# GreatV/oar-ocr

Measured on AMD Instinct MI355X. Metric: images/sec end-to-end PP-OCRv6 det+rec, higher is better.
Workload: dtype f32; 1 GPU; PP-OCRv6-tiny-class det+rec (synthetic-weight graphs: det 447089 params, rec 1135700 params, V=6906), batch=32 synthetic 960x960 pages per GPU, 40 text lines/page; timed region = u8 pages in pageable HOST memory -> oar_ocr_predict -> oar_ocr_decode -> sorted boxes + texts + scores on the host; image_batch_size=32, region_batch_size=256, parallelism=image-parallel x1

## Files before the change

### include/oar_mi355x.h

```cpp
#ifndef OAR_MI355X_H
#define OAR_MI355X_H

#include <stddef.h>
#include <stdint.h>

#ifdef __cplusplus
extern "C" {
#endif

typedef enum {
    OAR_OK = 0,
    OAR_INVALID_INPUT = 1,
    OAR_MODEL_LOAD = 2,
    OAR_UNSUPPORTED_OP = 3,
    OAR_SHAPE_MISMATCH = 4,
    OAR_DEVICE = 5,
    OAR_OOM = 6,
    OAR_INTERNAL = 7
} oar_status;

size_t oar_last_error(char* buf, size_t cap);
size_t oar_version(char* buf, size_t cap);
int oar_device_count(void);

// ... 170 lines not shown
    float* ctc_probs;
    float* page_angle;
    uint8_t* page_rectified;
    float* line_angle;
    uint32_t n_points;
    uint32_t* point_offsets;
} oar_ocr_result;

oar_status oar_ocr_create(const uint8_t* det_onnx, size_t det_len, const uint8_t* rec_onnx, size_t rec_len,
                          const oar_ocr_cfg* cfg, oar_ocr** out);
void oar_ocr_destroy(oar_ocr* o);
oar_status oar_ocr_predict(oar_ocr* o, const uint8_t* const* rgb, const uint32_t* widths, const uint32_t* heights,
                           uint32_t n_images, oar_ocr_result* out);
oar_status oar_ocr_predict_device(oar_ocr* o, const uint8_t* const* d_rgb, const uint32_t* widths,
                                  const uint32_t* heights, uint32_t n_images, oar_ocr_result* out);
void oar_ocr_result_free(oar_ocr_result* r);
oar_status oar_ocr_predict_async(oar_ocr* o, const uint8_t* const* rgb, const uint32_t* widths, const uint32_t* heights, uint32_t n_images,
                                 int32_t device_pages, uint64_t* ticket);
oar_status oar_ocr_wait(oar_ocr* o, uint64_t ticket, oar_ocr_result* out);
oar_status oar_ocr_decode(const oar_ctc_dict* dict, const oar_ocr_result* res, float score_threshold, oar_text_result* out);

oar_status oar_ctc_word_boxes(const float* line_pts_xy, uint32_t n_points, const char* text_utf8, size_t text_len, const uint32_t* col_indices,
                              uint32_t n_cols, uint32_t seq_len, float wh_ratio, float max_wh_ratio, float* boxes, uint32_t cap_boxes, uint32_t* n_boxes);
oar_status oar_char_positions_to_word_boxes(const float* line_pts_xy, uint32_t n_points, const float* char_positions, uint32_t n_positions,
                                            uint32_t char_count, float* boxes, uint32_t cap_boxes, uint32_t* n_boxes);
typedef struct {
    uint32_t n_regions;
    uint64_t* box_offsets;
    float* boxes;
} oar_word_boxes;
oar_status oar_ocr_word_boxes(const oar_ocr_result* res, const oar_text_result* txt, oar_word_boxes* out);
void oar_word_boxes_free(oar_word_boxes* w);

typedef struct {
    uint32_t n_images, n_regions;
    uint32_t* region_offsets;
    float* points;
    float* scores;
    uint64_t* text_offsets;
    char* utf8;
} oar_packed_pages;
oar_status oar_shard_range(uint64_t n_items, uint32_t world_size, uint32_t rank, uint64_t* begin, uint64_t* end);
oar_status oar_ocr_pack(const oar_ocr_result* res, const oar_text_result* txt, uint8_t** blob, size_t* len);
void oar_blob_free(uint8_t* blob);
oar_status oar_packed_merge(const uint8_t* const* blobs, const size_t* lens, uint32_t n_blobs, oar_packed_pages* out);
void oar_packed_pages_free(oar_packed_pages* p);

typedef struct oar_cls oar_cls;
typedef struct {
    int32_t device_id;
    uint32_t input_h, input_w;
    uint32_t resize_short;
    uint32_t topk;
    uint32_t batch;
} oar_cls_cfg;
typedef struct {
    uint32_t n_images, topk, n_classes;
    int32_t* class_ids;
    float* scores;
} oar_cls_result;
oar_status oar_cls_create(const uint8_t* onnx, size_t onnx_len, const oar_cls_cfg* cfg, oar_cls** out);
void oar_cls_destroy(oar_cls* c);
oar_status oar_cls_run(oar_cls* c, const uint8_t* const* rgb, const uint32_t* widths, const uint32_t* heights, uint32_t n_images,
                       oar_cls_result* out);
void oar_cls_result_free(oar_cls_result* r);
oar_status oar_cls_preprocess(oar_cls* c, const uint8_t* const* rgb, const uint32_t* widths, const uint32_t* heights, uint32_t n_images,
                              float* out_nchw);

typedef struct oar_rect oar_rect;
#define OAR_RECT_NATIVE_SIZE 0xFFFFFFFFu
typedef struct { int32_t device_id; uint32_t target_h, target_w; } oar_rect_cfg;
oar_status oar_rect_create(const uint8_t* onnx, size_t onnx_len, const oar_rect_cfg* cfg, oar_rect** out);
void oar_rect_destroy(oar_rect* r);
oar_status oar_rect_run(oar_rect* r, const uint8_t* rgb, uint32_t width, uint32_t height, uint8_t* out_rgb);

oar_status oar_ocr_attach(oar_ocr* o, oar_cls* doc_orientation, oar_rect* rectifier, oar_cls* line_orientation);

oar_status oar_k_rotate_rgb(const uint8_t* rgb, uint32_t w, uint32_t h, int32_t quarter, uint8_t* out);
oar_status oar_k_bgr_planes_to_rgb(const float* planes, uint64_t plane, float scale, uint8_t* out);
oar_status oar_host_rotate_back_points(float* pts, uint32_t n_points, float angle, uint32_t rotated_w, uint32_t rotated_h);

typedef struct oar_layout oar_layout;
typedef struct {
    int32_t device_id;
    uint32_t input_h, input_w;
    int32_t resize_filter;
    int32_t color_bgr;
    float scale;
    float mean[3], std[3];
    uint32_t num_classes;
    int32_t model_type;
    float score_threshold;
    float nms_threshold;
    uint32_t max_detections;
} oar_layout_cfg;
typedef struct {
    uint32_t n_images, n_boxes;
    uint32_t* box_offsets;
    float* boxes;
    int32_t* classes;
    float* scores;
    uint32_t feature_dim;
} oar_layout_result;
oar_status oar_layout_create(const uint8_t* onnx, size_t onnx_len, const oar_layout_cfg* cfg, oar_layout** out);
void oar_layout_destroy(oar_layout* l);
oar_status oar_layout_run(oar_layout* l, const uint8_t* const* rgb, const uint32_t* widths, const uint32_t* heights, uint32_t n_images, oar_layout_result* out);
void oar_layout_result_free(oar_layout_result* r);
oar_status oar_layout_preprocess(oar_layout* l, const uint8_t* rgb, uint32_t width, uint32_t height, float* out_chw);
oar_status oar_k_resize_filter(const uint8_t* rgb, uint32_t w, uint32_t h, uint32_t nw, uint32_t nh, int32_t filter, uint8_t* out);
oar_status oar_k_layout_postprocess(const float* pred, uint32_t n_images, uint32_t rows, uint32_t feat, const float* src_wh, uint32_t num_classes, int32_t model_type,
                                    float score_threshold, float nms_threshold, uint32_t max_detections, oar_layout_result* out);
typedef struct {
    float score_threshold;
    const float* class_thresholds;
    int32_t layout_nms;
    int32_t image_class_id;
    int32_t formula_class_id;
    const int32_t* class_merge_modes;
} oar_ppdoc_cfg;
oar_status oar_layout_run_ppdoc(oar_layout* l, const uint8_t* const* rgb, const uint32_t* widths, const uint32_t* heights, uint32_t n_images, const oar_ppdoc_cfg* cfg,
                                oar_layout_result* out);
oar_status oar_k_ppdoc_postprocess(const float* pred, uint32_t n_images, uint32_t rows, uint32_t feat, const float* src_wh, uint32_t num_classes, const oar_ppdoc_cfg* cfg,
                                   oar_layout_result* out);
int32_t oar_host_nms_with_merge(const float* boxes, const int32_t* classes, const float* scores, uint32_t n, const int32_t* mode_of_class, uint32_t num_classes,
                                float nms_threshold, uint32_t max_detections, float* out_boxes, int32_t* out_classes, float* out_scores);

oar_status oar_dev_alloc(int32_t device_id, size_t bytes, void** out);
oar_status oar_dev_upload(void* dst, const void* src, size_t bytes);
oar_status oar_dev_download(void* dst, const void* src, size_t bytes);
void oar_dev_free(void* p);
oar_status oar_dev_synchronize(int32_t device_id);

oar_status oar_k_normalize(const uint8_t* rgb, uint32_t w, uint32_t h, const int32_t src_channels[3],
                           const float alpha[3], const float beta[3], int32_t hwc_layout, float* out);
oar_status oar_k_rec_preprocess(const uint8_t* const* rgb, const uint32_t* widths, const uint32_t* heights,
                                uint32_t n, uint32_t img_h, uint32_t img_w, uint32_t max_img_w,
                                float* out_nchw, uint32_t* tensor_width);
oar_status oar_k_rec_preprocess_flip(const uint8_t* const* rgb, const uint32_t* widths, const uint32_t* heights, const uint8_t* flips,
                                     uint32_t n, uint32_t img_h, uint32_t img_w, uint32_t max_img_w,
                                     float* out_nchw, uint32_t* tensor_width);
oar_status oar_k_resize_triangle(const uint8_t* rgb, uint32_t w, uint32_t h, uint32_t nw, uint32_t nh, uint8_t* out);
oar_status oar_k_threshold(const float* pred, size_t n, float thresh, uint8_t* mask);
oar_status oar_k_dilate(const uint8_t* mask, uint32_t height, uint32_t width, uint8_t* out);
oar_status oar_k_poly_scores(const float* pred, uint32_t height, uint32_t width, const float* pts_xy, const uint32_t* counts,
                             uint32_t n_polys, float* scores);
oar_status oar_k_contours(const uint8_t* mask, uint32_t width, uint32_t height, uint32_t max_contours, int32_t* n_contours,
                          int64_t* offsets, int32_t* pts_xy, int32_t* types, int64_t cap_points);
oar_status oar_k_ctc_argmax(const float* probs, size_t rows, size_t vocab, int64_t* idx, float* prob);
oar_status oar_k_unclip(const float* boxes, uint32_t n_boxes, float ratio, int32_t* counts, float* pts_xy, uint32_t cap_points);
oar_status oar_k_box_scores(const float* pred, uint32_t height, uint32_t width, const float* boxes,
                            uint32_t n_boxes, float* scores);
oar_status oar_k_rotate_crop(const uint8_t* rgb, uint32_t w, uint32_t h, const float box[8], uint8_t* out,
                             size_t cap, uint32_t* out_w, uint32_t* out_h);

oar_status oar_image_decode(const uint8_t* bytes, size_t len, uint8_t** rgb, uint32_t* width, uint32_t* height);
void oar_image_free(uint8_t* rgb);
oar_status oar_image_decode_device(const uint8_t* bytes, size_t len, int32_t device_id, void** dev_rgb, uint32_t* width, uint32_t* height);

int32_t oar_host_candidates(const uint8_t* mask, uint32_t width, uint32_t height, uint32_t max_candidates, int32_t max_bands,
                            float* boxes8, int32_t cap);
int32_t oar_host_contours(const uint8_t* mask, uint32_t width, uint32_t height, uint32_t max_contours, int32_t max_bands,
                          int64_t* offsets, int32_t* pts_xy, int32_t* types, int64_t cap_points);
int32_t oar_host_contours_bits(const uint8_t* mask, uint32_t width, uint32_t height, uint32_t max_contours, int32_t max_bands,
                               int64_t* offsets, int32_t* pts_xy, int32_t* types, int64_t cap_points);
int32_t oar_host_unclip(const float box8[8], float ratio, float* out_xy, int32_t cap_points);
int32_t oar_host_approx_poly_dp(const float* xy, int32_t n_points, float epsilon, float* out_xy, int32_t cap_points);
float oar_host_perimeter(const float* xy, int32_t n_points);
int32_t oar_host_unclip_poly(const float* xy, int32_t n_points, float ratio, float* out_xy, int32_t cap_points);
int32_t oar_host_offset_ring(const int64_t* xy, int32_t n_points, double radius, int64_t* out_xy, int32_t cap_points);
int32_t oar_host_ring_outline(const int64_t* xy, int32_t n_points, int32_t negative, int64_t* out_xy, int32_t cap_points);
void oar_host_sort_poly_boxes(const float* pts_xy, const uint32_t* offsets, int32_t n, int32_t* order);
int32_t oar_host_mini_box(const float* xy, int32_t n_points, float box8[8], float* min_side);
int32_t oar_host_convex_hull(const float* xy, int32_t n_points, float* out_xy, int32_t cap_points);
void oar_host_sort_quad_boxes(const float* boxes8, int32_t n, int32_t* order);
int32_t oar_host_pool_selftest(int32_t threads, int32_t jobs);
void oar_host_plan_crop(uint32_t img_w, uint32_t img_h, const float box8[8], int32_t plan[8], float inv[9]);

oar_status oar_debug_inject_failure(const char* site, int32_t count);

typedef struct {
    char name[48];
    uint64_t launches;
    double total_ms;
    double alg_bytes;
    double alg_flops;
} oar_prof_entry;
void oar_prof_reset(void);
void oar_prof_enable(int32_t on);
void oar_prof_filter(const char* class_name);
void oar_prof_sampling(int32_t stride, int32_t phase);
int32_t oar_prof_snapshot(oar_prof_entry* entries, int32_t cap);

#ifdef __cplusplus
}
#endif
#endif
```

### oar_ocr_amd/api.py

```python
from __future__ import annotations

import ctypes as C
import os
from dataclasses import dataclass, field
from pathlib import Path
from typing import List, Optional, Sequence

import numpy as np

_HERE = Path(__file__).resolve().parent
LIB_PATH = _HERE / "lib" / "libOarMi355x.so"
_lib = None

OAR_OK, OAR_INVALID_INPUT, OAR_MODEL_LOAD, OAR_UNSUPPORTED_OP, OAR_SHAPE_MISMATCH, OAR_DEVICE, OAR_OOM, OAR_INTERNAL = range(8)


class OCRError(RuntimeError):

    def __init__(self, code: int, message: str):
        super().__init__(f"[oar_status {code}] {message}")
        self.code = code
        self.message = message


class EngineCfg(C.Structure):
    _fields_ = [("device_id", C.c_int32), ("use_hip_graph", C.c_int32), ("profile", C.c_int32), ("precision", C.c_int32), ("stream", C.c_void_p)]


PRECISION_F32 = 0


class Tensor(C.Structure):
    _fields_ = [("rank", C.c_int32), ("dims", C.c_int64 * 8), ("data", C.POINTER(C.c_float)), ("name", C.c_char * 64),
                ("dtype", C.c_int32), ("reserved", C.c_int32), ("data_i64", C.POINTER(C.c_int64))]


class Input(C.Structure):
    _fields_ = [("name", C.c_char_p), ("data", C.POINTER(C.c_float)), ("dims", C.POINTER(C.c_int64)), ("rank", C.c_int32),
                ("reserved", C.c_int32)]


class IoInfo(C.Structure):
    _fields_ = [("name", C.c_char * 64), ("dtype", C.c_int32), ("rank", C.c_int32), ("dims", C.c_int64 * 8)]


OUTPUT_VIEW_FN = C.CFUNCTYPE(C.c_int32, C.c_void_p, C.POINTER(C.c_int64), C.c_int32, C.POINTER(C.c_float))


class DetCfg(C.Structure):
    _fields_ = [("device_id", C.c_int32), ("limit_side_len", C.c_uint32), ("limit_type", C.c_int32), ("max_side_limit", C.c_uint32),
                ("max_candidates", C.c_uint32), ("use_hip_graph", C.c_int32), ("profile", C.c_int32), ("host_threads", C.c_int32),
                ("box_type", C.c_int32), ("score_mode", C.c_int32), ("use_dilation", C.c_int32), ("gpu_contours", C.c_int32)]


class DetResult(C.Structure):
    _fields_ = [("n_images", C.c_uint32), ("n_boxes", C.c_uint32), ("box_offsets", C.POINTER(C.c_uint32)),
                ("points", C.POINTER(C.c_float)), ("scores", C.POINTER(C.c_float)), ("n_points", C.c_uint32), ("point_offsets", C.POINTER(C.c_uint32))]


class RecCfg(C.Structure):
    _fields_ = [("device_id", C.c_int32), ("rec_image_shape", C.c_uint32 * 3), ("max_img_w", C.c_uint32), ("use_hip_graph", C.c_int32),
                ("profile", C.c_int32), ("reserved", C.c_int32)]


class RecResult(C.Structure):
    _fields_ = [("batch", C.c_uint32), ("seq_len", C.c_uint32), ("vocab", C.c_uint32), ("tensor_width", C.c_uint32),
                ("indices", C.POINTER(C.c_int64)), ("probs", C.POINTER(C.c_float))]


class OcrCfg(C.Structure):
    _fields_ = [("det", DetCfg), ("rec", RecCfg), ("det_thresh", C.c_float), ("det_box_thresh", C.c_float), ("det_unclip_ratio", C.c_float),
                ("image_batch_size", C.c_uint32), ("region_batch_size", C.c_uint32), ("max_pooled_crops", C.c_uint32), ("box_sort", C.c_int32), ("lanes", C.c_uint32)]


class OcrResult(C.Structure):
    _fields_ = [("n_images", C.c_uint32), ("n_regions", C.c_uint32), ("region_offsets", C.POINTER(C.c_uint32)),
                ("points", C.POINTER(C.c_float)), ("det_scores", C.POINTER(C.c_float)), ("crop_wh", C.POINTER(C.c_uint32)),
                ("seq_len", C.POINTER(C.c_uint32)), ("max_wh_ratio", C.POINTER(C.c_float)), ("ctc_offsets", C.POINTER(C.c_uint64)),
                ("ctc_indices", C.POINTER(C.c_int64)), ("ctc_probs", C.POINTER(C.c_float)),
                ("page_angle", C.POINTER(C.c_float)), ("page_rectified", C.POINTER(C.c_uint8)), ("line_angle", C.POINTER(C.c_float)),
                ("n_points", C.c_uint32), ("point_offsets", C.POINTER(C.c_uint32))]


class ClsCfg(C.Structure):
    _fields_ = [("device_id", C.c_int32), ("input_h", C.c_uint32), ("input_w", C.c_uint32), ("resize_short", C.c_uint32),
                ("topk", C.c_uint32), ("batch", C.c_uint32)]


class ClsResult(C.Structure):
    _fields_ = [("n_images", C.c_uint32), ("topk", C.c_uint32), ("n_classes", C.c_uint32), ("class_ids", C.POINTER(C.c_int32)),
                ("scores", C.POINTER(C.c_float))]


class RectCfg(C.Structure):
    _fields_ = [("device_id", C.c_int32), ("target_h", C.c_uint32), ("target_w", C.c_uint32)]


class TextResult(C.Structure):
    _fields_ = [("n", C.c_uint32), ("text_offsets", C.POINTER(C.c_uint64)), ("utf8", C.POINTER(C.c_char)), ("scores", C.POINTER(C.c_float)),
                ("char_offsets", C.POINTER(C.c_uint64)), ("char_cols", C.POINTER(C.c_uint32)), ("char_positions", C.POINTER(C.c_float)),
                ("seq_len", C.POINTER(C.c_uint32)), ("kept", C.POINTER(C.c_uint8))]


class WordBoxes(C.Structure):
    _fields_ = [("n_regions", C.c_uint32), ("box_offsets", C.POINTER(C.c_uint64)), ("boxes", C.POINTER(C.c_float))]


class LayoutCfg(C.Structure):
    _fields_ = [("device_id", C.c_int32), ("input_h", C.c_uint32), ("input_w", C.c_uint32), ("resize_filter", C.c_int32), ("color_bgr", C.c_int32), ("scale", C.c_float),
                ("mean", C.c_float * 3), ("std", C.c_float * 3), ("num_classes", C.c_uint32), ("model_type", C.c_int32), ("score_threshold", C.c_float),
                ("nms_threshold", C.c_float), ("max_detections", C.c_uint32)]


class LayoutResult(C.Structure):
    _fields_ = [("n_images", C.c_uint32), ("n_boxes", C.c_uint32), ("box_offsets", C.POINTER(C.c_uint32)), ("boxes", C.POINTER(C.c_float)),
                ("classes", C.POINTER(C.c_int32)), ("scores", C.POINTER(C.c_float)), ("feature_dim", C.c_uint32)]


class ProfEntry(C.Structure):
    _fields_ = [("name", C.c_char * 48), ("launches", C.c_uint64), ("total_ms", C.c_double), ("alg_bytes", C.c_double), ("alg_flops", C.c_double)]


class DecodeStats(C.Structure):
    _fields_ = [("steps_limit", C.c_int64), ("steps_enqueued", C.c_int64), ("steps_executed", C.c_int64), ("lookahead", C.c_int64)]

    def __repr__(self):
        return f"DecodeStats(steps_limit={self.steps_limit}, steps_enqueued={self.steps_enqueued}, steps_executed={self.steps_executed}, lookahead={self.lookahead})"


EXPORTS = [
    "oar_last_error", "oar_version", "oar_device_count", "oar_engine_create", "oar_engine_destroy", "oar_engine_input_name",
    "oar_engine_run", "oar_engine_run_named", "oar_engine_run_first_f32", "oar_engine_io", "oar_tensor_free", "oar_engine_cost", "oar_det_create", "oar_det_destroy", "oar_det_run", "oar_det_result_free",
    "oar_db_postprocess", "oar_rec_create", "oar_rec_destroy", "oar_rec_run", "oar_rec_result_free", "oar_ocr_create", "oar_ocr_destroy",
    "oar_ocr_predict", "oar_ocr_predict_device", "oar_ocr_result_free", "oar_dev_alloc", "oar_dev_upload", "oar_dev_download",
    "oar_dev_free", "oar_dev_synchronize", "oar_k_normalize", "oar_k_rec_preprocess", "oar_k_resize_triangle", "oar_k_threshold",
    "oar_k_ctc_argmax", "oar_k_box_scores", "oar_k_rotate_crop", "oar_prof_reset", "oar_prof_enable", "oar_prof_filter", "oar_prof_sampling", "oar_prof_snapshot",
    "oar_host_candidates", "oar_host_unclip", "oar_host_mini_box", "oar_host_convex_hull", "oar_host_sort_quad_boxes", "oar_host_pool_selftest", "oar_host_plan_crop",
    "oar_cls_create", "oar_cls_destroy", "oar_cls_run", "oar_cls_result_free", "oar_cls_preprocess", "oar_rect_create", "oar_rect_destroy",
    "oar_rect_run", "oar_ocr_attach", "oar_k_rotate_rgb", "oar_k_bgr_planes_to_rgb", "oar_host_rotate_back_points",
    "oar_engine_cache_stats", "oar_onnx_inspect", "oar_host_contours", "oar_ctc_dict_create", "oar_ctc_dict_destroy", "oar_ctc_dict_classes",
    "oar_ctc_decode", "oar_ocr_decode", "oar_text_result_free", "oar_db_postprocess_ex", "oar_k_dilate", "oar_k_poly_scores", "oar_debug_inject_failure", "oar_k_contours", "oar_host_contours_bits",
    "oar_k_unclip", "oar_k_rec_preprocess_flip", "oar_layout_create", "oar_layout_destroy", "oar_layout_run", "oar_layout_result_free", "oar_layout_preprocess", "oar_k_resize_filter", "oar_k_layout_postprocess", "oar_layout_run_ppdoc", "oar_k_ppdoc_postprocess", "oar_host_nms_with_merge", "oar_image_decode_device", "oar_ocr_predict_async", "oar_ocr_wait", "oar_ctc_word_boxes", "oar_char_positions_to_word_boxes", "oar_ocr_word_boxes", "oar_word_boxes_free", "oar_image_decode", "oar_image_free", "oar_host_approx_poly_dp", "oar_host_perimeter", "oar_host_unclip_poly", "oar_host_offset_ring", "oar_host_ring_outline", "oar_host_sort_poly_boxes",
    "oar_engine_set_decode_stop", "oar_engine_decode_stats",
]


def lib():
    global _lib
    if _lib is not None:
        return _lib
    if not LIB_PATH.exists():
        raise OCRError(OAR_DEVICE, f"{LIB_PATH} is missing: run `python -c 'import __graft_entry__ as g; g.build()'` "
                                   "(the MI355X path has no CPU fallback)")
    L = C.CDLL(str(LIB_PATH))
    vp, u8pp, u32p, f32p = C.c_void_p, C.POINTER(C.c_void_p), C.POINTER(C.c_uint32), C.POINTER(C.c_float)
    L.oar_last_error.restype = C.c_size_t
    L.oar_last_error.argtypes = [C.c_char_p, C.c_size_t]
    L.oar_version.restype = C.c_size_t
    L.oar_version.argtypes = [C.c_char_p, C.c_size_t]
    L.oar_device_count.restype = C.c_int
    L.oar_engine_create.argtypes = [vp, C.c_size_t, C.POINTER(EngineCfg), C.POINTER(vp)]
    L.oar_engine_destroy.argtypes = [vp]
    L.oar_engine_destroy.restype = None
    L.oar_engine_input_name.argtypes = [vp, C.c_char_p, C.c_size_t]
    L.oar_engine_run.argtypes = [vp, vp, C.POINTER(C.c_int64), C.c_int32, C.POINTER(Tensor), C.c_int32, C.POINTER(C.c_int32)]
    L.oar_engine_run_named.argtypes = [vp, C.POINTER(Input), C.c_int32, C.POINTER(Tensor), C.c_int32, C.POINTER(C.c_int32)]
    L.oar_engine_run_first_f32.argtypes = [vp, C.POINTER(Input), C.c_int32, OUTPUT_VIEW_FN, vp]
    L.oar_engine_io.argtypes = [vp, C.POINTER(IoInfo), C.c_int32, C.POINTER(C.c_int32), C.POINTER(IoInfo), C.c_int32, C.POINTER(C.c_int32)]
    L.oar_tensor_free.argtypes = [C.POINTER(Tensor)]
    L.oar_tensor_free.restype = None
    L.oar_engine_cost.argtypes = [vp, C.POINTER(C.c_int64), C.c_int32, C.POINTER(C.c_double), C.POINTER(C.c_double), C.POINTER(C.c_int32)]
    L.oar_engine_cache_stats.argtypes = [vp, C.POINTER(C.c_uint64), C.POINTER(C.c_uint64)]
    L.oar_engine_set_decode_stop.argtypes = [vp, C.c_int64]
    L.oar_engine_decode_stats.argtypes = [vp, C.POINTER(DecodeStats)]
    L.oar_onnx_inspect.argtypes = [vp, C.c_size_t, C.c_char_p, C.c_size_t]
    L.oar_det_create.argtypes = [vp, C.c_size_t, C.POINTER(DetCfg), C.POINTER(vp)]
    L.oar_det_destroy.argtypes = [vp]
    L.oar_det_destroy.restype = None
    L.oar_det_run.argtypes = [vp, u8pp, u32p, u32p, C.c_uint32, C.c_float, C.c_float, C.c_float, C.POINTER(DetResult)]
    L.oar_det_result_free.argtypes = [C.POINTER(DetResult)]
    L.oar_det_result_free.restype = None
    L.oar_db_postprocess.argtypes = [vp, C.c_uint32, C.c_uint32, C.c_uint32, C.c_uint32, C.c_float, C.c_float, C.c_float, C.c_uint32, C.POINTER(DetResult)]
    L.oar_db_postprocess_ex.argtypes = [vp, C.c_uint32, C.c_uint32, C.c_uint32, C.c_uint32, C.c_float, C.c_float, C.c_float, C.c_uint32, C.c_int32, C.c_int32,
                                        C.c_int32, C.POINTER(DetResult)]
    L.oar_debug_inject_failure.argtypes = [C.c_char_p, C.c_int32]
    L.oar_k_dilate.argtypes = [vp, C.c_uint32, C.c_uint32, vp]
    L.oar_k_poly_scores.argtypes = [vp, C.c_uint32, C.c_uint32, vp, u32p, C.c_uint32, vp]
    L.oar_rec_create.argtypes = [vp, C.c_size_t, C.POINTER(RecCfg), C.POINTER(vp)]
    L.oar_rec_destroy.argtypes = [vp]
    L.oar_rec_destroy.restype = None
    L.oar_rec_run.argtypes = [vp, u8pp, u32p, u32p, C.c_uint32, C.POINTER(RecResult)]
    L.oar_rec_result_free.argtypes = [C.POINTER(RecResult)]
    L.oar_rec_result_free.restype = None
    L.oar_ocr_create.argtypes = [vp, C.c_size_t, vp, C.c_size_t, C.POINTER(OcrCfg), C.POINTER(vp)]
    L.oar_ocr_destroy.argtypes = [vp]
    L.oar_ocr_destroy.restype = None
    L.oar_ocr_predict.argtypes = [vp, u8pp, u32p, u32p, C.c_uint32, C.POINTER(OcrResult)]
    L.oar_ocr_predict_device.argtypes = [vp, u8pp, u32p, u32p, C.c_uint32, C.POINTER(OcrResult)]
    L.oar_ocr_result_free.argtypes = [C.POINTER(OcrResult)]
    L.oar_ocr_result_free.restype = None
    L.oar_dev_alloc.argtypes = [C.c_int32, C.c_size_t, C.POINTER(vp)]
    L.oar_dev_upload.argtypes = [vp, vp, C.c_size_t]
    L.oar_dev_download.argtypes = [vp, vp, C.c_size_t]
    L.oar_dev_free.argtypes = [vp]
    L.oar_dev_free.restype = None
    L.oar_dev_synchronize.argtypes = [C.c_int32]
    L.oar_k_normalize.argtypes = [vp, C.c_uint32, C.c_uint32, C.POINTER(C.c_int32), f32p, f32p, C.c_int32, vp]
    L.oar_k_rec_preprocess.argtypes = [u8pp, u32p, u32p, C.c_uint32, C.c_uint32, C.c_uint32, C.c_uint32, vp, u32p]
    L.oar_ctc_word_boxes.argtypes = [vp, C.c_uint32, C.c_char_p, C.c_size_t, vp, C.c_uint32, C.c_uint32, C.c_float, C.c_float, vp, C.c_uint32, u32p]
    L.oar_char_positions_to_word_boxes.argtypes = [vp, C.c_uint32, vp, C.c_uint32, C.c_uint32, vp, C.c_uint32, u32p]
    L.oar_ocr_word_boxes.argtypes = [vp, vp, vp]
    L.oar_word_boxes_free.argtypes = [vp]
    L.oar_word_boxes_free.restype = None
    L.oar_k_rec_preprocess_flip.argtypes = [u8pp, u32p, u32p, vp, C.c_uint32, C.c_uint32, C.c_uint32, C.c_uint32, vp, u32p]
    L.oar_k_resize_triangle.argtypes = [vp, C.c_uint32, C.c_uint32, C.c_uint32, C.c_uint32, vp]
    L.oar_k_threshold.argtypes = [vp, C.c_size_t, C.c_float, vp]
    L.oar_k_ctc_argmax.argtypes = [vp, C.c_size_t, C.c_size_t, vp, vp]
    L.oar_k_box_scores.argtypes = [vp, C.c_uint32, C.c_uint32, vp, C.c_uint32, vp]
    L.oar_k_unclip.argtypes = [vp, C.c_uint32, C.c_float, vp, vp, C.c_uint32]
    L.oar_image_decode.argtypes = [vp, C.c_size_t, C.POINTER(C.POINTER(C.c_uint8)), C.POINTER(C.c_uint32), C.POINTER(C.c_uint32)]
    L.oar_image_free.argtypes = [C.POINTER(C.c_uint8)]
    L.oar_layout_create.argtypes = [vp, C.c_size_t, vp, C.POINTER(C.c_void_p)]
    L.oar_layout_destroy.argtypes = [vp]
    L.oar_layout_destroy.restype = None
    L.oar_layout_run.argtypes = [vp, u8pp, u32p, u32p, C.c_uint32, vp]
    L.oar_layout_result_free.argtypes = [vp]
    L.oar_layout_result_free.restype = None
    L.oar_layout_preprocess.argtypes = [vp, vp, C.c_uint32, C.c_uint32, vp]
    L.oar_k_resize_filter.argtypes = [vp, C.c_uint32, C.c_uint32, C.c_uint32, C.c_uint32, C.c_int32, vp]
    L.oar_k_layout_postprocess.argtypes = [vp, C.c_uint32, C.c_uint32, C.c_uint32, vp, C.c_uint32, C.c_int32, C.c_float, C.c_float, C.c_uint32, vp]
    L.oar_ocr_predict_async.argtypes = [vp, u8pp, u32p, u32p, C.c_uint32, C.c_int32, C.POINTER(C.c_uint64)]
    L.oar_ocr_wait.argtypes = [vp, C.c_uint64, vp]
    L.oar_image_decode_device.argtypes = [vp, C.c_size_t, C.c_int32, C.POINTER(C.c_void_p), C.POINTER(C.c_uint32), C.POINTER(C.c_uint32)]
    L.oar_image_free.restype = None
    L.oar_k_rotate_crop.argtypes = [vp, C.c_uint32, C.c_uint32, f32p, vp, C.c_size_t, u32p, u32p]
    L.oar_host_candidates.argtypes = [vp, C.c_uint32, C.c_uint32, C.c_uint32, C.c_int32, vp, C.c_int32]
    L.oar_host_candidates.restype = C.c_int32
    L.oar_host_contours.argtypes = [vp, C.c_uint32, C.c_uint32, C.c_uint32, C.c_int32, vp, vp, vp, C.c_int64]
    L.oar_host_contours.restype = C.c_int32
    L.oar_host_unclip.argtypes = [vp, C.c_float, vp, C.c_int32]
    L.oar_host_unclip.restype = C.c_int32
    L.oar_host_approx_poly_dp.argtypes = [vp, C.c_int32, C.c_float, vp, C.c_int32]
    L.oar_host_approx_poly_dp.restype = C.c_int32
    L.oar_host_perimeter.argtypes = [vp, C.c_int32]
    L.oar_host_perimeter.restype = C.c_float
    L.oar_host_unclip_poly.argtypes = [vp, C.c_int32, C.c_float, vp, C.c_int32]
    L.oar_host_unclip_poly.restype = C.c_int32
    L.oar_host_offset_ring.argtypes = [vp, C.c_int32, C.c_double, vp, C.c_int32]
    L.oar_host_offset_ring.restype = C.c_int32
    L.oar_host_ring_outline.argtypes = [vp, C.c_int32, C.c_int32, vp, C.c_int32]
    L.oar_host_ring_outline.restype = C.c_int32
    L.oar_host_sort_poly_boxes.argtypes = [vp, vp, C.c_int32, vp]
    L.oar_host_sort_poly_boxes.restype = None
    L.oar_host_mini_box.argtypes = [vp, C.c_int32, vp, f32p]
    L.oar_host_mini_box.restype = C.c_int32
    L.oar_host_convex_hull.argtypes = [vp, C.c_int32, vp, C.c_int32]
    L.oar_host_convex_hull.restype = C.c_int32
    L.oar_host_sort_quad_boxes.argtypes = [vp, C.c_int32, vp]
    L.oar_host_sort_quad_boxes.restype = None
    L.oar_host_plan_crop.argtypes = [C.c_uint32, C.c_uint32, vp, vp, vp]
    L.oar_host_plan_crop.restype = None
    L.oar_cls_create.argtypes = [vp, C.c_size_t, C.POINTER(ClsCfg), C.POINTER(vp)]
    L.oar_cls_destroy.argtypes = [vp]
    L.oar_cls_destroy.restype = None
    L.oar_cls_run.argtypes = [vp, u8pp, u32p, u32p, C.c_uint32, C.POINTER(ClsResult)]
    L.oar_cls_result_free.argtypes = [C.POINTER(ClsResult)]
    L.oar_cls_result_free.restype = None
    L.oar_cls_preprocess.argtypes = [vp, u8pp, u32p, u32p, C.c_uint32, vp]
    L.oar_rect_create.argtypes = [vp, C.c_size_t, C.POINTER(RectCfg), C.POINTER(vp)]
    L.oar_rect_destroy.argtypes = [vp]
    L.oar_rect_destroy.restype = None
    L.oar_rect_run.argtypes = [vp, vp, C.c_uint32, C.c_uint32, vp]
    L.oar_ocr_attach.argtypes = [vp, vp, vp, vp]
    L.oar_k_rotate_rgb.argtypes = [vp, C.c_uint32, C.c_uint32, C.c_int32, vp]
    L.oar_k_bgr_planes_to_rgb.argtypes = [vp, C.c_uint64, C.c_float, vp]
    L.oar_host_rotate_back_points.argtypes = [vp, C.c_uint32, C.c_float, C.c_uint32, C.c_uint32]
    L.oar_ctc_dict_create.argtypes = [C.c_char_p, C.c_size_t, C.c_int32, C.POINTER(vp)]
    L.oar_ctc_dict_destroy.argtypes = [vp]
    L.oar_ctc_dict_destroy.restype = None
    L.oar_ctc_dict_classes.argtypes = [vp]
    L.oar_ctc_dict_classes.restype = C.c_uint32
    L.oar_ctc_decode.argtypes = [vp, vp, vp, C.c_uint32, C.c_uint32, C.c_float, C.POINTER(TextResult)]
    L.oar_ocr_decode.argtypes = [vp, C.POINTER(OcrResult), C.c_float, C.POINTER(TextResult)]
    L.oar_text_result_free.argtypes = [C.POINTER(TextResult)]
    L.oar_text_result_free.restype = None
    L.oar_prof_reset.restype = None
    L.oar_prof_enable.argtypes = [C.c_int32]
    L.oar_prof_enable.restype = None
    L.oar_prof_filter.argtypes = [C.c_char_p]
    L.oar_prof_filter.restype = None
    L.oar_prof_sampling.argtypes = [C.c_int32, C.c_int32]
    L.oar_prof_sampling.restype = None
    L.oar_prof_snapshot.argtypes = [C.POINTER(ProfEntry), C.c_int32]
    L.oar_prof_snapshot.restype = C.c_int32
    _lib = L
    return L


def _check(st: int):
    if st != OAR_OK:
        buf = C.create_string_buffer(4096)
        lib().oar_last_error(buf, 4096)
        raise OCRError(st, buf.value.decode(errors="replace"))


DEFAULT_PARALLEL_THRESHOLD = 4


def load_image_from_memory(data: bytes) -> np.ndarray:
    buf = (C.c_char * len(data)).from_buffer_copy(data) if len(data) else (C.c_char * 1)()
    out = C.POINTER(C.c_uint8)()
    w, h = C.c_uint32(0), C.c_uint32(0)
    _check(lib().oar_image_decode(C.cast(buf, C.c_void_p), len(data), C.byref(out), C.byref(w), C.byref(h)))
    try:
        return np.ctypeslib.as_array(out, shape=(h.value, w.value, 3)).copy()
    finally:
        lib().oar_image_free(out)


def load_image_to_device(data: bytes, device_id: int = 0):
    buf = (C.c_char * len(data)).from_buffer_copy(data) if len(data) else (C.c_char * 1)()
    ptr = C.c_void_p()
    w, h = C.c_uint32(0), C.c_uint32(0)
    _check(lib().oar_image_decode_device(C.cast(buf, C.c_void_p), len(data), device_id, C.byref(ptr), C.byref(w), C.byref(h)))
    holder = DeviceBuffer.__new__(DeviceBuffer)
    holder.ptr, holder.nbytes = ptr, w.value * h.value * 3
    return holder, w.value, h.value


def load_image(path) -> np.ndarray:
    with open(path, "rb") as f:
        return load_image_from_memory(f.read())


def load_images(paths, parallel_threshold: Optional[int] = None) -> List[np.ndarray]:
    paths = list(paths)
    thr = DEFAULT_PARALLEL_THRESHOLD if parallel_threshold is None else parallel_threshold
    if len(paths) > thr:
        from concurrent.futures import ThreadPoolExecutor
        with ThreadPoolExecutor(max_workers=min(len(paths), os.cpu_count() or 4)) as ex:
            return list(ex.map(load_image, paths))
    return [load_image(p) for p in paths]


def version() -> str:
    buf = C.create_string_buffer(256)
    lib().oar_version(buf, 256)
    return buf.value.decode()


def onnx_inspect(model: bytes) -> str:
    buf = C.create_string_buffer(8192)
    b = (C.c_char * max(len(model), 1)).from_buffer_copy(model or b"\0")
    st = lib().oar_onnx_inspect(C.cast(b, C.c_void_p), len(model), buf, 8192)
    _check(st)
    return buf.value.decode()


def debug_inject_failure(site: str, count: int):
    _check(lib().oar_debug_inject_failure(site.encode(), count))


def device_count() -> int:
    return int(lib().oar_device_count())


def _p(a: np.ndarray):
    return a.ctypes.data_as(C.c_void_p)


def _img_arrays(images: Sequence[np.ndarray]):
    imgs = [np.ascontiguousarray(im, dtype=np.uint8) for im in images]
    for im in imgs:
        if im.ndim != 3 or im.shape[2] != 3:
            raise OCRError(OAR_INVALID_INPUT, "images must be HxWx3 uint8 (RgbImage)")
    ptrs = (C.c_void_p * max(len(imgs), 1))(*[im.ctypes.data for im in imgs])
    ws = (C.c_uint32 * max(len(imgs), 1))(*[im.shape[1] for im in imgs])
    hs = (C.c_uint32 * max(len(imgs), 1))(*[im.shape[0] for im in imgs])
    return imgs, ptrs, ws, hs


class OrtInfer:

    def __init__(self, model: bytes, device_id: int = 0, profile: bool = False, precision: int = PRECISION_F32, stream: Optional[int] = None):
        self._h = C.c_void_p()
        cfg = EngineCfg(device_id, 0, int(profile), int(precision), C.c_void_p(stream) if stream else None)
        buf = (C.c_char * len(model)).from_buffer_copy(model)
        _check(lib().oar_engine_create(C.cast(buf, C.c_void_p), len(model), C.byref(cfg), C.byref(self._h)))
# ... 1027 lines not shown
        raise OCRError(OAR_INVALID_INPUT, "oar_host_nms_with_merge failed")
    return ob[:k].copy(), oc[:k].copy(), os_[:k].copy()


def k_resize_filter(rgb, nw, nh, filter="lanczos3"):
    rgb = np.ascontiguousarray(rgb, np.uint8)
    h, w, _ = rgb.shape
    out = np.empty((nh, nw, 3), np.uint8)
    _check(lib().oar_k_resize_filter(_p(rgb), w, h, nw, nh, LAYOUT_FILTERS[filter], _p(out)))
    return out


def k_layout_postprocess(pred, src_wh, num_classes, score_threshold=0.5, nms_threshold=0.5, max_detections=100, model_type="picodet"):
    pred = np.ascontiguousarray(pred, np.float32)
    n, rows, feat = pred.shape
    wh = np.ascontiguousarray(src_wh, np.float32).reshape(n, 2)
    res = LayoutResult()
    _check(lib().oar_k_layout_postprocess(_p(pred) if pred.size else None, n, rows, feat, _p(wh), num_classes, LAYOUT_MODEL_TYPES.get(model_type, 0), C.c_float(score_threshold),
                                          C.c_float(nms_threshold), max_detections, C.byref(res)))
    try:
        return _unpack_layout(res)
    finally:
        lib().oar_layout_result_free(C.byref(res))


class DeviceBuffer:
    def __init__(self, data: np.ndarray, device_id: int = 0):
        data = np.ascontiguousarray(data)
        self.nbytes = data.nbytes
        self.ptr = C.c_void_p()
        _check(lib().oar_dev_alloc(device_id, self.nbytes, C.byref(self.ptr)))
        _check(lib().oar_dev_upload(self.ptr, _p(data), self.nbytes))

    def free(self):
        if self.ptr:
            lib().oar_dev_free(self.ptr)
            self.ptr = C.c_void_p()

    def __del__(self):
        try:
            self.free()
        except Exception:
            pass


def prof_enable(on: bool = True):
    lib().oar_prof_enable(int(on))


def prof_filter(name: str = ""):
    lib().oar_prof_filter(name.encode() if name else None)


def prof_sampling(stride: int = 1, phase: int = 0):
    lib().oar_prof_sampling(stride, phase)


def prof_reset():
    lib().oar_prof_reset()


def prof_snapshot(max_entries: int = 512):
    arr = (ProfEntry * max_entries)()
    n = lib().oar_prof_snapshot(arr, max_entries)
    return [{"name": arr[i].name.decode(), "launches": int(arr[i].launches), "total_ms": arr[i].total_ms,
             "alg_bytes": arr[i].alg_bytes, "alg_flops": arr[i].alg_flops} for i in range(min(n, max_entries))]


def k_normalize(rgb, alpha, beta, src=(0, 1, 2), layout="chw"):
    rgb = np.ascontiguousarray(rgb, np.uint8)
    h, w, _ = rgb.shape
    out = np.empty((3, h, w) if layout == "chw" else (h, w, 3), np.float32)
    a, b = np.ascontiguousarray(alpha, np.float32), np.ascontiguousarray(beta, np.float32)
    s = (C.c_int32 * 3)(*src)
    _check(lib().oar_k_normalize(_p(rgb), w, h, s, a.ctypes.data_as(C.POINTER(C.c_float)), b.ctypes.data_as(C.POINTER(C.c_float)),
                                 0 if layout == "chw" else 1, _p(out)))
    return out


def k_rec_preprocess(crops, img_h=48, img_w=320, max_img_w=3200, flips=None):
    imgs, ptrs, ws, hs = _img_arrays(crops)
    tw = C.c_uint32(0)
    fl = None if flips is None else np.ascontiguousarray(np.asarray(flips, bool).astype(np.uint8))
    _check(lib().oar_k_rec_preprocess_flip(ptrs, ws, hs, None if fl is None else _p(fl), len(imgs), img_h, img_w, max_img_w, None, C.byref(tw)))
    out = np.empty((len(imgs), 3, img_h, tw.value), np.float32)
    _check(lib().oar_k_rec_preprocess_flip(ptrs, ws, hs, None if fl is None else _p(fl), len(imgs), img_h, img_w, max_img_w, _p(out), C.byref(tw)))
    return out


def k_resize_triangle(rgb, nw, nh):
    rgb = np.ascontiguousarray(rgb, np.uint8)
    h, w, _ = rgb.shape
    out = np.empty((nh, nw, 3), np.uint8)
    _check(lib().oar_k_resize_triangle(_p(rgb), w, h, nw, nh, _p(out)))
    return out


def k_threshold(pred, thresh):
    pred = np.ascontiguousarray(pred, np.float32)
    out = np.empty(pred.shape, np.uint8)
    _check(lib().oar_k_threshold(_p(pred), pred.size, thresh, _p(out)))
    return out


def k_dilate(mask):
    mask = np.ascontiguousarray(mask, np.uint8)
    out = np.empty_like(mask)
    _check(lib().oar_k_dilate(_p(mask), mask.shape[0], mask.shape[1], _p(out)))
    return out


def k_poly_scores(pred, polys):
    pred = np.ascontiguousarray(pred, np.float32)
    h, w = pred.shape
    pts = np.ascontiguousarray(np.concatenate([np.asarray(p, np.float32).reshape(-1, 2) for p in polys]) if polys else np.zeros((0, 2), np.float32))
    counts = (C.c_uint32 * max(len(polys), 1))(*[len(p) for p in polys])
    out = np.zeros(len(polys), np.float32)
    _check(lib().oar_k_poly_scores(_p(pred), h, w, _p(pts), counts, len(polys), _p(out)))
    return out


def k_ctc_argmax(probs):
    probs = np.ascontiguousarray(probs, np.float32)
    v = probs.shape[-1]
    rows = probs.size // v if v else 0
    idx = np.zeros(rows, np.int64)
    p = np.zeros(rows, np.float32)
    _check(lib().oar_k_ctc_argmax(_p(probs), rows, v, _p(idx), _p(p)))
    return idx, p


def k_box_scores(pred, boxes):
    pred = np.ascontiguousarray(pred, np.float32)
    boxes = np.ascontiguousarray(boxes, np.float32).reshape(-1, 8)
    h, w = pred.shape
    out = np.zeros(boxes.shape[0], np.float32)
    _check(lib().oar_k_box_scores(_p(pred), h, w, _p(boxes), boxes.shape[0], _p(out)))
    return out


def k_rotate_crop(img, box):
    img = np.ascontiguousarray(img, np.uint8)
    h, w, _ = img.shape
    box = np.ascontiguousarray(box, np.float32).reshape(8)
    cap = 3 * (w + h + 8) ** 2
    out = np.empty(cap, np.uint8)
    ow, oh = C.c_uint32(0), C.c_uint32(0)
    _check(lib().oar_k_rotate_crop(_p(img), w, h, box.ctypes.data_as(C.POINTER(C.c_float)), _p(out), cap, C.byref(ow), C.byref(oh)))
    if ow.value == 0:
        return None
    return out[:ow.value * oh.value * 3].reshape(oh.value, ow.value, 3).copy()


def host_candidates(mask, max_candidates=1000, max_bands=1):
    mask = np.ascontiguousarray(mask, np.uint8)
    h, w = mask.shape
    out = np.zeros((max_candidates, 4, 2), np.float32)
    n = lib().oar_host_candidates(_p(mask), w, h, max_candidates, max_bands, _p(out), max_candidates)
    if n < 0:
        raise OCRError(OAR_INTERNAL, "oar_host_candidates failed")
    return out[:n].copy()


def host_contours(mask, max_contours=100000, max_bands=1, bits=False):
    mask = np.ascontiguousarray(mask, np.uint8)
    h, w = mask.shape
    cap = 4 * h * w + 16
    offs = np.zeros(max_contours + 1, np.int64)
    pts = np.zeros((cap, 2), np.int32)
    types = np.zeros(max_contours, np.int32)
    fn = lib().oar_host_contours_bits if bits else lib().oar_host_contours
    n = fn(_p(mask), w, h, max_contours, max_bands, _p(offs), _p(pts), _p(types), cap)
    if n < 0:
        raise OCRError(OAR_INTERNAL, "oar_host_contours failed")
    return [(pts[offs[i]:offs[i + 1]].copy(), int(types[i])) for i in range(n)]


def k_contours(mask, max_contours=100000):
    mask = np.ascontiguousarray(mask, np.uint8)
    h, w = mask.shape
    cap = 4 * h * w + 16
    offs = np.zeros(max_contours + 1, np.int64)
    pts = np.zeros((cap, 2), np.int32)
    types = np.zeros(max_contours, np.int32)
    n = C.c_int32(0)
    _check(lib().oar_k_contours(_p(mask), w, h, max_contours, C.byref(n), _p(offs), _p(pts), _p(types), cap))
    return [(pts[offs[i]:offs[i + 1]].copy(), int(types[i])) for i in range(n.value)]


def k_unclip(boxes, ratio, cap_points=96):
    b = np.ascontiguousarray(boxes, np.float32).reshape(-1, 8)
    n = len(b)
    counts = np.zeros(max(n, 1), np.int32)
    pts = np.zeros((max(n, 1), cap_points, 2), np.float32)
    _check(lib().oar_k_unclip(_p(b), n, C.c_float(ratio), _p(counts), _p(pts), cap_points))
    return [None if counts[i] < 0 else pts[i, :counts[i]].copy() for i in range(n)]


def host_unclip(box, ratio):
    box = np.ascontiguousarray(box, np.float32).reshape(8)
    out = np.zeros((1024, 2), np.float32)
    n = lib().oar_host_unclip(_p(box), ratio, _p(out), 1024)
    return out[:max(n, 0)].copy()


def host_approx_poly_dp(points, epsilon):
    pts = np.ascontiguousarray(points, np.float32).reshape(-1, 2)
    out = np.zeros((max(len(pts), 1), 2), np.float32)
    n = lib().oar_host_approx_poly_dp(_p(pts), pts.shape[0], C.c_float(epsilon), _p(out), out.shape[0])
    return out[:max(n, 0)].copy()


def host_perimeter(points) -> float:
    pts = np.ascontiguousarray(points, np.float32).reshape(-1, 2)
    return float(lib().oar_host_perimeter(_p(pts), pts.shape[0]))


def host_unclip_poly(points, ratio):
    pts = np.ascontiguousarray(points, np.float32).reshape(-1, 2)
    cap = 64 * len(pts) + 1024
    out = np.zeros((cap, 2), np.float32)
    n = lib().oar_host_unclip_poly(_p(pts), pts.shape[0], C.c_float(ratio), _p(out), cap)
    if n < 0:
        raise RuntimeError("oar_host_unclip_poly failed")
    return out[:n].copy()


def host_offset_ring(ring, radius):
    r = np.ascontiguousarray(ring, np.int64).reshape(-1, 2)
    cap = 64 * len(r) + 1024
    out = np.zeros((cap, 2), np.int64)
    n = lib().oar_host_offset_ring(_p(r), r.shape[0], C.c_double(radius), _p(out), cap)
    return out[:max(n, 0)].copy()


def host_ring_outline(raw, negative=False):
    r = np.ascontiguousarray(raw, np.int64).reshape(-1, 2)
    cap = 4 * len(r) + 64
    out = np.zeros((cap, 2), np.int64)
    n = lib().oar_host_ring_outline(_p(r), r.shape[0], 1 if negative else 0, _p(out), cap)
    return out[:n].copy() if n > 0 else None


def host_sort_poly_boxes(polys):
    if not polys:
        return np.zeros(0, np.int32)
    offs = np.zeros(len(polys) + 1, np.uint32)
    offs[1:] = np.cumsum([len(p) for p in polys])
    pts = np.ascontiguousarray(np.concatenate([np.asarray(p, np.float32).reshape(-1, 2) for p in polys] + [np.zeros((0, 2), np.float32)]), np.float32)
    if len(pts) == 0:
        pts = np.zeros((1, 2), np.float32)
    order = np.zeros(len(polys), np.int32)
    lib().oar_host_sort_poly_boxes(_p(pts), _p(offs), len(polys), _p(order))
    return order


def host_mini_box(points):
    pts = np.ascontiguousarray(points, np.float32).reshape(-1, 2)
    out = np.zeros((4, 2), np.float32)
    ms = C.c_float(0)
    ok = lib().oar_host_mini_box(_p(pts), pts.shape[0], _p(out), C.byref(ms))
    return (out, float(ms.value)) if ok == 1 else None


def host_convex_hull(points):
    pts = np.ascontiguousarray(points, np.float32).reshape(-1, 2)
    out = np.zeros((max(pts.shape[0], 1), 2), np.float32)
    n = lib().oar_host_convex_hull(_p(pts), pts.shape[0], _p(out), out.shape[0])
    if n < 0:
        raise OCRError(1, "oar_host_convex_hull failed")
    return out[:n].copy()


def host_sort_quad_boxes(boxes):
    b = np.ascontiguousarray(boxes, np.float32).reshape(-1, 8)
    order = np.zeros(b.shape[0], np.int32)
    if b.shape[0]:
        lib().oar_host_sort_quad_boxes(_p(b), b.shape[0], _p(order))
    return order


def host_plan_crop(img_w, img_h, box):
    b = np.ascontiguousarray(box, np.float32).reshape(8)
    plan = np.zeros(8, np.int32)
    inv = np.zeros(9, np.float32)
    lib().oar_host_plan_crop(img_w, img_h, _p(b), _p(plan), _p(inv))
    return plan, inv


@dataclass
class Classification:
    class_id: int
    score: float


class ImageClassifier:

    def __init__(self, model: bytes, input_hw=(224, 224), resize_short: int = 256, topk: int = 1, device_id: int = 0, batch: int = 0):
        self._h = C.c_void_p()
        self.input_hw = tuple(input_hw)
        cfg = ClsCfg(device_id, input_hw[0], input_hw[1], resize_short or 0, topk, batch)
        buf = (C.c_char * len(model)).from_buffer_copy(model)
        _check(lib().oar_cls_create(C.cast(buf, C.c_void_p), len(model), C.byref(cfg), C.byref(self._h)))

    def predict(self, images: Sequence[np.ndarray]) -> List[List[Classification]]:
        if len(images) == 0:
# ... 376 lines not shown
```

### oar_ocr_amd/csrc/c_api.cc

```cpp
#include <condition_variable>
#include <cstdlib>
#include <cmath>
#include <cstring>
#include <deque>
#include <map>
#include <mutex>
#include <thread>

#include "engine.h"
#include "layout.h"
#include "pipeline.h"

namespace oar {
const std::string& last_error();
extern std::atomic<int> g_inject_batched_det_failures;
}
using namespace oar;

struct oar_engine { std::unique_ptr<Engine> e; PinBuf view; };
struct oar_det { std::unique_ptr<Detector> d; };
struct oar_rec { std::unique_ptr<Recognizer> r; };
struct OcrLane {
    std::unique_ptr<Ocr> o;
    std::thread worker;
// ... 990 lines not shown
oar_status oar_k_rec_preprocess(const uint8_t* const* rgb, const uint32_t* widths, const uint32_t* heights, uint32_t n, uint32_t img_h,
                                uint32_t img_w, uint32_t max_img_w, float* out_nchw, uint32_t* tensor_width) {
    return oar_k_rec_preprocess_flip(rgb, widths, heights, nullptr, n, img_h, img_w, max_img_w, out_nchw, tensor_width);
}

oar_status oar_k_rec_preprocess_flip(const uint8_t* const* rgb, const uint32_t* widths, const uint32_t* heights, const uint8_t* flips, uint32_t n,
                                     uint32_t img_h, uint32_t img_w, uint32_t max_img_w, float* out_nchw, uint32_t* tensor_width) {
    return guard([&] {
        OAR_CHECK(tensor_width && (n == 0 || (rgb && widths && heights)), OAR_INVALID_INPUT, "oar_k_rec_preprocess: bad arguments");
        require_device();
        std::vector<uint32_t> ws(widths, widths + n), hs(heights, heights + n);
        std::vector<int32_t> rws;
        int Wt = host::rec_tensor_width(ws, hs, (int)img_h, (int)img_w, (int)max_img_w, rws);
        *tensor_width = (uint32_t)Wt;
        if (!out_nchw || n == 0) return;
        size_t stage = 0;
        for (uint32_t i = 0; i < n; ++i) stage += ((size_t)ws[i] * hs[i] * 3 + 63) & ~(size_t)63;
        DevBuf dc, dd, dout;
        dc.reserve(stage); dd.reserve(n * sizeof(pp::CropDesc)); dout.reserve((size_t)n * 3 * img_h * Wt * 4);
        std::vector<pp::CropDesc> descs(n);
        size_t off = 0;
        for (uint32_t i = 0; i < n; ++i) {
            size_t bytes = (size_t)ws[i] * hs[i] * 3;
            OAR_HIP(hipMemcpy(dc.as<uint8_t>() + off, rgb[i], bytes, hipMemcpyHostToDevice));
            descs[i].src = dc.as<uint8_t>() + off; descs[i].w = (int)ws[i]; descs[i].h = (int)hs[i]; descs[i].rw = rws[i]; descs[i].flip = flips && flips[i] ? 1 : 0;
            off += (bytes + 63) & ~(size_t)63;
        }
        OAR_HIP(hipMemcpy(dd.p, descs.data(), n * sizeof(pp::CropDesc), hipMemcpyHostToDevice));
        pp::rec_pack(nullptr, dd.as<pp::CropDesc>(), (int)n, (int)img_h, Wt, dout.as<float>(), 1);
        OAR_HIP(hipMemcpy(out_nchw, dout.p, (size_t)n * 3 * img_h * Wt * 4, hipMemcpyDeviceToHost));
    });
}

oar_status oar_k_resize_triangle(const uint8_t* rgb, uint32_t w, uint32_t h, uint32_t nw, uint32_t nh, uint8_t* out) {
    return guard([&] {
        OAR_CHECK(rgb && out && w && h && nw && nh, OAR_INVALID_INPUT, "oar_k_resize_triangle: bad arguments");
        require_device();
        DevBuf din, dout;
        din.reserve((size_t)w * h * 3); dout.reserve((size_t)nw * nh * 3);
        OAR_HIP(hipMemcpy(din.p, rgb, (size_t)w * h * 3, hipMemcpyHostToDevice));
        pp::resize_triangle(nullptr, din.as<uint8_t>(), (int)w, (int)h, dout.as<uint8_t>(), (int)nw, (int)nh);
        OAR_HIP(hipMemcpy(out, dout.p, (size_t)nw * nh * 3, hipMemcpyDeviceToHost));
    });
}

oar_status oar_k_threshold(const float* pred, size_t n, float thresh, uint8_t* mask) {
    return guard([&] {
        OAR_CHECK((pred && mask) || n == 0, OAR_INVALID_INPUT, "oar_k_threshold: bad arguments");
        require_device();
        if (n == 0) return;
        DevBuf din, dout;
        din.reserve(n * 4); dout.reserve(n + 4);
        OAR_HIP(hipMemcpy(din.p, pred, n * 4, hipMemcpyHostToDevice));
        pp::threshold(nullptr, din.as<float>(), dout.as<uint8_t>(), (int64_t)n, thresh);
        OAR_HIP(hipMemcpy(mask, dout.p, n, hipMemcpyDeviceToHost));
    });
}

oar_status oar_k_dilate(const uint8_t* mask, uint32_t height, uint32_t width, uint8_t* out) {
    return guard([&] {
        OAR_CHECK(mask && out && height && width, OAR_INVALID_INPUT, "oar_k_dilate: bad arguments");
        require_device();
        const size_t n = (size_t)height * width;
        DevBuf din, dout;
        din.reserve(n); dout.reserve(n);
        OAR_HIP(hipMemcpy(din.p, mask, n, hipMemcpyHostToDevice));
        pp::dilate3x3(nullptr, din.as<uint8_t>(), dout.as<uint8_t>(), 1, (int)height, (int)width);
        OAR_HIP(hipMemcpy(out, dout.p, n, hipMemcpyDeviceToHost));
    });
}

oar_status oar_k_poly_scores(const float* pred, uint32_t height, uint32_t width, const float* pts_xy, const uint32_t* counts, uint32_t n_polys,
                             float* scores) {
    return guard([&] {
        OAR_CHECK(pred && height && width && (n_polys == 0 || (pts_xy && counts && scores)), OAR_INVALID_INPUT, "oar_k_poly_scores: bad arguments");
        require_device();
        if (n_polys == 0) return;
        std::vector<pp::PolyDesc> pd(n_polys);
        size_t at = 0;
        for (uint32_t i = 0; i < n_polys; ++i) { pd[i] = pp::PolyDesc{(int32_t)at, (int32_t)counts[i], 0, 0}; at += counts[i]; }
        const size_t hw = (size_t)height * width;
        DevBuf dpred, dpts, dpd, dsc;
        dpred.reserve(hw * 4); dpts.reserve(at * 8 + 8); dpd.reserve(pd.size() * sizeof(pp::PolyDesc)); dsc.reserve((size_t)n_polys * 4);
        OAR_HIP(hipMemcpy(dpred.p, pred, hw * 4, hipMemcpyHostToDevice));
        if (at) OAR_HIP(hipMemcpy(dpts.p, pts_xy, at * 8, hipMemcpyHostToDevice));
        OAR_HIP(hipMemcpy(dpd.p, pd.data(), pd.size() * sizeof(pp::PolyDesc), hipMemcpyHostToDevice));
        pp::poly_scores(nullptr, dpred.as<float>(), (int)height, (int)width, dpts.as<float>(), dpd.as<pp::PolyDesc>(), (int)n_polys, dsc.as<float>());
        OAR_HIP(hipMemcpy(scores, dsc.p, (size_t)n_polys * 4, hipMemcpyDeviceToHost));
    });
}

oar_status oar_k_ctc_argmax(const float* probs, size_t rows, size_t vocab, int64_t* idx, float* prob) {
    return guard([&] {
        require_device();
        if (rows == 0 || vocab == 0) return;
        OAR_CHECK(probs && idx && prob, OAR_INVALID_INPUT, "oar_k_ctc_argmax: bad arguments");
        DevBuf din, di, dp;
        din.reserve(rows * vocab * 4); di.reserve(rows * 8); dp.reserve(rows * 4);
        OAR_HIP(hipMemcpy(din.p, probs, rows * vocab * 4, hipMemcpyHostToDevice));
        pp::ctc_argmax(nullptr, din.as<float>(), (int64_t)rows, (int)vocab, di.as<int64_t>(), dp.as<float>());
        OAR_HIP(hipMemcpy(idx, di.p, rows * 8, hipMemcpyDeviceToHost));
        OAR_HIP(hipMemcpy(prob, dp.p, rows * 4, hipMemcpyDeviceToHost));
    });
}

oar_status oar_k_unclip(const float* boxes, uint32_t n_boxes, float ratio, int32_t* counts, float* pts_xy, uint32_t cap_points) {
    return guard([&] {
        require_device();
        OAR_CHECK(n_boxes == 0 || (boxes && counts && pts_xy), OAR_INVALID_INPUT, "oar_k_unclip: bad arguments");
        if (n_boxes == 0) return;
        std::vector<pp::ScoreBox> sb(n_boxes);
        for (uint32_t i = 0; i < n_boxes; ++i) { std::memcpy(sb[i].pts, boxes + (size_t)i * 8, 32); sb[i].image = 0; sb[i].pad = 0; }
        DevBuf db, dout;
        db.reserve(n_boxes * sizeof(pp::ScoreBox)); dout.reserve(n_boxes * sizeof(pp::UnclipOut));
        OAR_HIP(hipMemcpy(db.p, sb.data(), n_boxes * sizeof(pp::ScoreBox), hipMemcpyHostToDevice));
        pp::unclip_quads(nullptr, db.as<pp::ScoreBox>(), (int)n_boxes, ratio, dout.as<pp::UnclipOut>());
        std::vector<pp::UnclipOut> ho(n_boxes);
        OAR_HIP(hipMemcpy(ho.data(), dout.p, n_boxes * sizeof(pp::UnclipOut), hipMemcpyDeviceToHost));
        for (uint32_t i = 0; i < n_boxes; ++i) {
            counts[i] = ho[i].n_pts;
            const int m = std::min<int>(std::max(ho[i].n_pts, 0), (int)cap_points);
            std::memcpy(pts_xy + (size_t)i * cap_points * 2, ho[i].pts, (size_t)m * 2 * sizeof(float));
        }
    });
}
oar_status oar_k_box_scores(const float* pred, uint32_t height, uint32_t width, const float* boxes, uint32_t n_boxes, float* scores) {
    return guard([&] {
        require_device();
        if (n_boxes == 0) return;
        OAR_CHECK(pred && boxes && scores && height && width, OAR_INVALID_INPUT, "oar_k_box_scores: bad arguments");
        size_t hw = (size_t)height * width;
        DevBuf dpred, db, ds;
        dpred.reserve(hw * 4); db.reserve(n_boxes * sizeof(pp::ScoreBox)); ds.reserve(n_boxes * 4);
        std::vector<pp::ScoreBox> sb(n_boxes);
        for (uint32_t i = 0; i < n_boxes; ++i) { std::memcpy(sb[i].pts, boxes + (size_t)i * 8, 32); sb[i].image = 0; sb[i].pad = 0; }
        OAR_HIP(hipMemcpy(dpred.p, pred, hw * 4, hipMemcpyHostToDevice));
        OAR_HIP(hipMemcpy(db.p, sb.data(), n_boxes * sizeof(pp::ScoreBox), hipMemcpyHostToDevice));
        pp::box_scores(nullptr, dpred.as<float>(), (int)height, (int)width, db.as<pp::ScoreBox>(), (int)n_boxes, ds.as<float>());
        OAR_HIP(hipMemcpy(scores, ds.p, n_boxes * 4, hipMemcpyDeviceToHost));
    });
}

oar_status oar_k_rotate_crop(const uint8_t* rgb, uint32_t w, uint32_t h, const float box[8], uint8_t* out, size_t cap, uint32_t* out_w,
                             uint32_t* out_h) {
    return guard([&] {
        OAR_CHECK(rgb && box && out_w && out_h && w && h, OAR_INVALID_INPUT, "oar_k_rotate_crop: bad arguments");
        require_device();
        host::CropPlan pl = host::plan_crop((int)w, (int)h, box);
        *out_w = *out_h = 0;
        if (pl.mode == 0) return;
        *out_w = (uint32_t)pl.out_w(); *out_h = (uint32_t)pl.out_h();
        size_t bytes = (size_t)pl.out_w() * pl.out_h() * 3;
        OAR_CHECK(out && cap >= bytes, OAR_INVALID_INPUT, "oar_k_rotate_crop: output buffer too small");
        DevBuf dpage, dd, dout;
        dpage.reserve((size_t)w * h * 3); dd.reserve(sizeof(pp::WarpDesc)); dout.reserve(bytes);
        OAR_HIP(hipMemcpy(dpage.p, rgb, (size_t)w * h * 3, hipMemcpyHostToDevice));
        pp::WarpDesc d;
        std::memset(&d, 0, sizeof d);
        d.page = dpage.as<uint8_t>(); d.page_w = (int)w; d.page_h = (int)h;
        d.left = pl.left; d.top = pl.top; d.cw = pl.cw; d.ch = pl.ch; d.ow = pl.ow; d.oh = pl.oh; d.rot = pl.rot; d.mode = pl.mode;
        std::memcpy(d.inv, pl.inv, sizeof d.inv);
        d.out_off = 0;
        OAR_HIP(hipMemcpy(dd.p, &d, sizeof d, hipMemcpyHostToDevice));
        pp::rotate_crops(nullptr, dd.as<pp::WarpDesc>(), 1, dout.as<uint8_t>(), pl.out_w() * pl.out_h());
        OAR_HIP(hipMemcpy(out, dout.p, bytes, hipMemcpyDeviceToHost));
    });
}

int32_t oar_host_candidates(const uint8_t* mask, uint32_t width, uint32_t height, uint32_t max_candidates, int32_t max_bands,
                            float* boxes8, int32_t cap) {
    try {
        const int row_bytes = ((int)width + 7) / 8;
        std::vector<uint8_t> bits((size_t)row_bytes * height, 0);
        for (uint32_t y = 0; y < height; ++y)
            for (uint32_t x = 0; x < width; ++x)
                if (mask[(size_t)y * width + x]) bits[(size_t)y * row_bytes + (x >> 3)] |= (uint8_t)(1u << (x & 7));
        std::vector<int> cuts = host::blank_row_bands_bits(bits.data(), row_bytes, (int)height, max_bands < 1 ? 1 : max_bands);
        std::vector<host::Contour> cs;
        for (size_t i = 0; i + 1 < cuts.size(); ++i) {
            auto part = host::find_contours_band_bits(bits.data(), row_bytes, (int)width, cuts[i], cuts[i + 1], max_candidates, true);
            for (auto& c : part) { if (cs.size() >= max_candidates) break; cs.push_back(std::move(c)); }
        }
        int32_t n = 0;
        for (auto& c : cs) {
            host::Pt mb[4];
            float ms = 0.f;
            if (!host::contour_mini_box(c, mb, ms) || ms < 3.0f) continue;
            if (n < cap) for (int k = 0; k < 4; ++k) { boxes8[n * 8 + k * 2] = mb[k].x; boxes8[n * 8 + k * 2 + 1] = mb[k].y; }
            ++n;
        }
        return n;
    } catch (...) { return -1; }
}
int32_t oar_host_contours_bits(const uint8_t* mask, uint32_t width, uint32_t height, uint32_t max_contours, int32_t max_bands, int64_t* offsets,
                               int32_t* pts_xy, int32_t* types, int64_t cap_points) {
    try {
        const int row_bytes = ((int)width + 7) / 8;
        std::vector<uint8_t> bits((size_t)row_bytes * height, 0);
        for (uint32_t y = 0; y < height; ++y)
            for (uint32_t x = 0; x < width; ++x)
                if (mask[(size_t)y * width + x]) bits[(size_t)y * row_bytes + (x >> 3)] |= (uint8_t)(1u << (x & 7));
        std::vector<int> cuts = host::blank_row_bands_bits(bits.data(), row_bytes, (int)height, max_bands < 1 ? 1 : max_bands);
        int32_t n = 0;
        int64_t np = 0;
        if (offsets) offsets[0] = 0;
        for (size_t i = 0; i + 1 < cuts.size(); ++i) {
            auto part = host::find_contours_band_bits(bits.data(), row_bytes, (int)width, cuts[i], cuts[i + 1], max_contours);
            for (auto& c : part) {
                if ((uint32_t)n >= max_contours) break;
                for (auto& q : c.pts) {
                    if (pts_xy && np < cap_points) { pts_xy[np * 2] = (int32_t)q.x; pts_xy[np * 2 + 1] = (int32_t)q.y; }
                    ++np;
                }
                if (types) types[n] = c.hole ? 1 : 0;
                ++n;
                if (offsets) offsets[n] = np;
            }
        }
        return n;
    } catch (...) { return -1; }
}
int32_t oar_host_contours(const uint8_t* mask, uint32_t width, uint32_t height, uint32_t max_contours, int32_t max_bands, int64_t* offsets,
                          int32_t* pts_xy, int32_t* types, int64_t cap_points) {
    try {
        std::vector<int32_t> scratch((size_t)width * height);
        std::vector<int> cuts = host::blank_row_bands(mask, (int)width, (int)height, max_bands < 1 ? 1 : max_bands);
        int32_t n = 0;
        int64_t np = 0;
        if (offsets) offsets[0] = 0;
        for (size_t i = 0; i + 1 < cuts.size(); ++i) {
            auto part = host::find_contours_band(mask, (int)width, (int)height, cuts[i], cuts[i + 1], max_contours, scratch.data());
            for (auto& c : part) {
                if ((uint32_t)n >= max_contours) break;
                for (auto& q : c.pts) {
                    if (pts_xy && np < cap_points) { pts_xy[np * 2] = (int32_t)q.x; pts_xy[np * 2 + 1] = (int32_t)q.y; }
                    ++np;
                }
                if (types) types[n] = c.hole ? 1 : 0;
                ++n;
                if (offsets) offsets[n] = np;
            }
        }
        return n;
    } catch (...) { return -1; }
}

oar_status oar_k_contours(const uint8_t* mask, uint32_t width, uint32_t height, uint32_t max_contours, int32_t* n_contours, int64_t* offsets,
                          int32_t* pts_xy, int32_t* types, int64_t cap_points) {
    return guard([&] {
        OAR_CHECK(mask && width > 0 && height > 0 && n_contours, OAR_INVALID_INPUT, "oar_k_contours: bad arguments");
        int ndev = 0;
        if (hipGetDeviceCount(&ndev) != hipSuccess || ndev <= 0) fail(OAR_DEVICE, "no HIP device visible: libOarMi355x has no CPU fallback");
        DevBuf dm;
        const size_t hw = (size_t)width * height;
        dm.reserve(hw);
        OAR_HIP(hipMemcpy(dm.p, mask, hw, hipMemcpyHostToDevice));
        std::vector<host::Contour> cs = Detector::trace_device_mask(dm.as<uint8_t>(), (int)height, (int)width, max_contours);
        int64_t np = 0;
        if (offsets) offsets[0] = 0;
        int32_t n = 0;
        for (auto& c : cs) {
            for (auto& q : c.pts) {
                if (pts_xy && np < cap_points) { pts_xy[np * 2] = (int32_t)q.x; pts_xy[np * 2 + 1] = (int32_t)q.y; }
                ++np;
            }
            if (types) types[n] = c.hole ? 1 : 0;
            ++n;
            if (offsets) offsets[n] = np;
        }
        *n_contours = n;
    });
}
int32_t oar_host_unclip(const float box8[8], float ratio, float* out_xy, int32_t cap_points) {
    try {
        host::Pt b[4];
        for (int k = 0; k < 4; ++k) b[k] = {box8[k * 2], box8[k * 2 + 1]};
        std::vector<host::Pt> r = host::unclip(b, ratio);
        for (size_t i = 0; i < r.size() && (int32_t)i < cap_points; ++i) { out_xy[i * 2] = r[i].x; out_xy[i * 2 + 1] = r[i].y; }
        return (int32_t)r.size();
    } catch (...) { return -1; }
}
oar_status oar_image_decode(const uint8_t* bytes, size_t len, uint8_t** rgb, uint32_t* width, uint32_t* height) {
    return guard([&] {
        OAR_CHECK(bytes && rgb && width && height, OAR_INVALID_INPUT, "oar_image_decode: bad arguments");
        *rgb = nullptr; *width = *height = 0;
        if (img::is_jpeg(bytes, len)) {
            img::JpegImage ji;
            img::jpeg_entropy_decode(bytes, len, ji);
            std::vector<uint8_t> px;
            img::jpeg_render_host(ji, px);
            uint8_t* out = cmalloc<uint8_t>(px.size());
            std::memcpy(out, px.data(), px.size());
            *rgb = out; *width = ji.w; *height = ji.h;
            return;
        }
        std::vector<uint8_t> px;
        uint32_t w = 0, h = 0;
        if (!img::is_png(bytes, len)) {
            if (!img::decode_misc(bytes, len, px, w, h)) {
                const char* what = img::sniff(bytes, len);
                if (what) fail(OAR_UNSUPPORTED_OP, std::string("image load: ") + what + " is not decoded by this library (PNG, JPEG, BMP, PNM, TIFF and GIF are); use the reference's loader for it");
                fail(OAR_INVALID_INPUT, "image load: unrecognised image format");
            }
        } else {
            img::decode_png(bytes, len, px, w, h);
        }
        uint8_t* out = cmalloc<uint8_t>(px.size());
        std::memcpy(out, px.data(), px.size());
        *rgb = out; *width = w; *height = h;
    });
}
void oar_image_free(uint8_t* rgb) { std::free(rgb); }

oar_status oar_image_decode_device(const uint8_t* bytes, size_t len, int32_t device_id, void** dev_rgb, uint32_t* width, uint32_t* height) {
    return guard([&] {
        OAR_CHECK(bytes && dev_rgb && width && height, OAR_INVALID_INPUT, "oar_image_decode_device: bad arguments");
        *dev_rgb = nullptr; *width = *height = 0;
        require_device();
// ... 282 lines not shown
```

### oar_ocr_amd/csrc/pipeline.cc

```cpp
#include "pipeline.h"

#include <algorithm>
#include <map>
#include <string>
#include <cmath>
#include <chrono>
#include <cstdlib>
#include <cstring>
#include <sched.h>

namespace oar {

namespace {
struct PhaseTimer {
    bool on;
    std::chrono::steady_clock::time_point t0;
    std::vector<std::pair<const char*, double>> marks;
    PhaseTimer() {
        static const bool en = [] { const char* e = getenv("OAR_TIMING"); return e && (e[0] == '1' || e[0] == '2'); }();
        on = en;
        t0 = std::chrono::steady_clock::now();
    }
    void mark(const char* name) {
        if (!on) return;
// ... 876 lines not shown
            OAR_HIP(hipMemcpyAsync(sl.scores_host.p, sl.scores_dev.p, total * sizeof(float), hipMemcpyDeviceToHost, score_stream_));
            OAR_HIP(hipEventRecord(score_done_[sb], score_stream_));
        } else if (total) {
            sl.boxes_host.reserve(total * sizeof(pp::ScoreBox)); sl.scores_host.reserve(total * sizeof(float));
            sl.boxes_dev.reserve(total * sizeof(pp::ScoreBox)); sl.scores_dev.reserve(total * sizeof(float));
            pp::ScoreBox* sbx = sl.boxes_host.as<pp::ScoreBox>();
            for (int k = 0; k < nb; ++k)
                for (size_t i = 0; i < cands[b0 + k].size(); ++i) {
                    pp::ScoreBox& x = sbx[sl.base[k] + i];
                    std::memcpy(x.pts, cands[b0 + k][i].pts, sizeof x.pts);
                    x.image = b0 + k; x.pad = 0;
                }
            OAR_HIP(hipMemcpyAsync(sl.boxes_dev.p, sbx, total * sizeof(pp::ScoreBox), hipMemcpyHostToDevice, score_stream_));
            pp::box_scores(score_stream_, probs, H, W, sl.boxes_dev.as<pp::ScoreBox>(), (int)total, sl.scores_dev.as<float>());
            OAR_HIP(hipMemcpyAsync(sl.scores_host.p, sl.scores_dev.p, total * sizeof(float), hipMemcpyDeviceToHost, score_stream_));
            static const int gpu_unclip_env = [] { const char* e = getenv("OAR_GPU_UNCLIP"); return e && (e[0] == '0' || e[0] == '1') ? e[0] - '0' : -1; }();
            const bool gpu_unclip = gpu_unclip_env >= 0 ? gpu_unclip_env == 1 : gpu_contours;
            sl.unclipped = gpu_unclip;
            if (gpu_unclip) {
                sl.unclip_dev.reserve(total * sizeof(pp::UnclipOut)); sl.unclip_host.reserve(total * sizeof(pp::UnclipOut));
                pp::unclip_quads(score_stream_, sl.boxes_dev.as<pp::ScoreBox>(), (int)total, unclip, sl.unclip_dev.as<pp::UnclipOut>());
                OAR_HIP(hipMemcpyAsync(sl.unclip_host.p, sl.unclip_dev.p, total * sizeof(pp::UnclipOut), hipMemcpyDeviceToHost, score_stream_));
            }
            OAR_HIP(hipEventRecord(score_done_[sb], score_stream_));
        }
        tmark("box_scores_enqueue");
        if (sb > 0 && !finished_prev) finish(sb - 1);
    };
    static const int depth = [] { const char* e = getenv("OAR_DET_DEPTH"); int v = e ? atoi(e) : 1; return v < 1 ? 1 : v > 8 ? 8 : v; }();
    if (helper_enqueues) {
        struct Enqueuer {
            std::thread th;
            std::atomic<int> done{0};
            std::atomic<bool> failed{false};
            std::exception_ptr err;
            ~Enqueuer() { if (th.joinable()) th.join(); }
        } enq;
        const int device = eng_->device();
        enq.th = std::thread([&, device] {
            try {
                OAR_HIP(hipSetDevice(device));
                for (int q = 0; q < nsub; ++q) { enqueue(q); enq.done.store(q + 1, std::memory_order_release); }
            } catch (...) {
                enq.err = std::current_exception();
                enq.failed.store(true, std::memory_order_release);
            }
        });
        for (int sb = 0; sb < nsub; ++sb) {
            wait_for_thread([&] { return enq.done.load(std::memory_order_acquire) > sb || enq.failed.load(std::memory_order_acquire); });
            if (enq.failed.load(std::memory_order_acquire)) { enq.th.join(); std::rethrow_exception(enq.err); }
            host_stage(sb);
        }
        finish(nsub - 1);
        enq.th.join();
        if (enq.failed.load(std::memory_order_acquire)) std::rethrow_exception(enq.err);
    } else {
        int queued = 0;
        for (; queued < std::min(depth, nsub); ++queued) enqueue(queued);
        for (int sb = 0; sb < nsub; ++sb) {
            if (queued < nsub) enqueue(queued++);
            host_stage(sb);
        }
        finish(nsub - 1);
    }
    if (Profiler::get().enabled) Profiler::get().flush();
}

std::vector<host::Contour> Detector::trace_device_mask(const uint8_t* d_mask, int H, int W, uint32_t max_contours, bool gpu_contours) {
    const size_t hw = (size_t)H * W;
    std::vector<uint8_t> mask;
    auto fetch = [&]() -> const uint8_t* {
        if (mask.empty()) { mask.resize(hw); OAR_HIP(hipMemcpy(mask.data(), d_mask, hw, hipMemcpyDeviceToHost)); }
        return mask.data();
    };
    if (!gpu_contours) return host::find_contours(fetch(), W, H, max_contours);
    ContourBufs tb;
    tb.reserve(1, 1, H, W, 1);
    pp::trace_contours(nullptr, d_mask, 1, H, W, tb.rows.as<uint8_t>(), tb.band_y.as<int32_t>(), tb.n_bands.as<int32_t>(), tb.lists.as<uint32_t>(),
                       ContourBufs::kSegsPerPage, tb.scratch.as<uint32_t>(), tb.packed.as<uint32_t>(), (uint32_t)std::min<size_t>(tb.packed_words_per_page, 0xffffffffu),
                       tb.ctrl.as<uint32_t>(), tb.ctrl_host.as<uint32_t>(), tb.table_dev.as<pp::SegRec>(), tb.table.as<pp::SegRec>(), ContourBufs::kSegsPerPage);
    OAR_HIP(hipStreamSynchronize(nullptr));
    const uint32_t* ctrl = tb.ctrl_host.as<uint32_t>();
    const uint32_t n_rec = ctrl[pp::kTraceCtlSegments];
    if (ctrl[pp::kTraceCtlOverflow] || n_rec > ContourBufs::kSegsPerPage) return host::find_contours(fetch(), W, H, max_contours);
    std::vector<std::pair<uint32_t, host::Contour>> items;
    for (uint32_t i = 0; i < n_rec; ++i) {
        const pp::SegRec& r = tb.table.as<pp::SegRec>()[i];
        OAR_CHECK(r.page == 0 && r.y0 >= 0 && r.y0 < r.y1 && r.y1 <= H && r.x0 >= 0 && r.x0 < r.x1 && r.x1 <= W, OAR_INTERNAL, "contour tracer: corrupt segment record");
        if (r.flags) trace_record_on_host(r, fetch(), H, W, max_contours, items);
        else parse_traced_record(r, tb.packed.as<uint32_t>(), items);
    }
    std::vector<host::Contour> out;
    merge_traced_page(items, max_contours, out);
    return out;
}

void Detector::postprocess_host(const float* pred, int H, int W, uint32_t src_w, uint32_t src_h, float thresh, float box_thresh,
                                float unclip, uint32_t max_candidates, DetBoxes& out, int score_mode, int use_dilation, int box_type) {
    int ndev = 0;
    if (hipGetDeviceCount(&ndev) != hipSuccess || ndev <= 0) fail(OAR_DEVICE, "no HIP device visible: libOarMi355x has no CPU fallback");
    const size_t hw = (size_t)H * W;
    DevBuf dpred, dmask, dmask2, dboxes, dscores, dpts;
    dpred.reserve(hw * 4); dmask.reserve(hw);
    OAR_HIP(hipMemcpy(dpred.p, pred, hw * 4, hipMemcpyHostToDevice));
    pp::threshold(nullptr, dpred.as<float>(), dmask.as<uint8_t>(), (int64_t)hw, thresh);
    const uint8_t* traced = dmask.as<uint8_t>();
    if (use_dilation) { dmask2.reserve(hw); pp::dilate3x3(nullptr, traced, dmask2.as<uint8_t>(), 1, H, W); traced = dmask2.as<uint8_t>(); }
    std::vector<Candidate> cands;
    const int kind = box_type == 1 ? kCandPoly : score_mode == 1 ? kCandSlow : kCandFast;
    {
        std::vector<host::Contour> cs = Detector::trace_device_mask(traced, H, W, max_candidates ? max_candidates : 1000);
        for (auto& c : cs) {
            Candidate cd;
            if (contour_candidate(c, cd, kind)) cands.push_back(std::move(cd));
        }
    }
    std::vector<float> scores(cands.size(), 0.f);
    if (!cands.empty() && kind != kCandFast) {
        std::vector<float> pts;
        std::vector<pp::PolyDesc> pd;
        for (auto& c : cands) {
            pd.push_back(pp::PolyDesc{(int32_t)(pts.size() / 2), (int32_t)c.contour.size(), 0, 0});
            for (auto& p : c.contour) { pts.push_back(p.x); pts.push_back(p.y); }
        }
        dpts.reserve(pts.size() * 4 + 8); dboxes.reserve(pd.size() * sizeof(pp::PolyDesc)); dscores.reserve(pd.size() * 4);
        OAR_HIP(hipMemcpy(dpts.p, pts.data(), pts.size() * 4, hipMemcpyHostToDevice));
        OAR_HIP(hipMemcpy(dboxes.p, pd.data(), pd.size() * sizeof(pp::PolyDesc), hipMemcpyHostToDevice));
        pp::poly_scores(nullptr, dpred.as<float>(), H, W, dpts.as<float>(), dboxes.as<pp::PolyDesc>(), (int)pd.size(), dscores.as<float>());
        OAR_HIP(hipMemcpy(scores.data(), dscores.p, pd.size() * 4, hipMemcpyDeviceToHost));
    } else if (!cands.empty()) {
        std::vector<pp::ScoreBox> sb(cands.size());
        for (size_t i = 0; i < cands.size(); ++i) { std::memcpy(sb[i].pts, cands[i].pts, sizeof sb[i].pts); sb[i].image = 0; sb[i].pad = 0; }
        dboxes.reserve(sb.size() * sizeof(pp::ScoreBox)); dscores.reserve(sb.size() * 4);
        OAR_HIP(hipMemcpy(dboxes.p, sb.data(), sb.size() * sizeof(pp::ScoreBox), hipMemcpyHostToDevice));
        pp::box_scores(nullptr, dpred.as<float>(), H, W, dboxes.as<pp::ScoreBox>(), (int)sb.size(), dscores.as<float>());
        OAR_HIP(hipMemcpy(scores.data(), dscores.p, sb.size() * 4, hipMemcpyDeviceToHost));
    }
    if (box_type == 1) finish_polys(cands, scores.data(), H, W, src_w, src_h, box_thresh, unclip, out);
    else finish_boxes(cands, scores.data(), H, W, src_w, src_h, box_thresh, unclip, out);
}

Recognizer::Recognizer(const uint8_t* onnx, size_t len, const oar_rec_cfg& cfg, const std::vector<hipStream_t>& lane_streams) : cfg_(cfg) {
    if (cfg_.rec_image_shape[0] == 0) { cfg_.rec_image_shape[0] = 3; cfg_.rec_image_shape[1] = 48; cfg_.rec_image_shape[2] = 320; }
    if (cfg_.max_img_w == 0) cfg_.max_img_w = 3200;
    eng_.reset(new Engine(onnx, len, cfg_.device_id, lane_streams.empty() ? nullptr : lane_streams[0]));
    const int n_lanes = [] { const char* e = getenv("OAR_REC_LANES"); int v = e ? atoi(e) : 2; return v < 1 ? 1 : v > 4 ? 4 : v; }();
    for (int i = 1; i < n_lanes; ++i) {
        lanes_.emplace_back(new Engine(onnx, len, cfg_.device_id, i < (int)lane_streams.size() ? lane_streams[i] : nullptr));
        lane_in_.emplace_back(new DevBuf());
        hipEvent_t ev;
        OAR_HIP(hipEventCreateWithFlags(&ev, hipEventDisableTiming));
        lane_done_.push_back(ev);
    }
    if (n_lanes > 1) {
        std::vector<hipStream_t> ls{eng_->stream()};
        for (auto& l : lanes_) ls.push_back(l->stream());
        Profiler::get().add_lanes(this, ls);
    }
}
Recognizer::~Recognizer() {
    if (!lanes_.empty()) Profiler::get().remove_lanes(this);
    for (auto& l : lanes_) (void)hipStreamSynchronize(l->stream());
    for (hipEvent_t e : lane_done_) (void)hipEventDestroy(e);
}

const float* Recognizer::pack(const std::vector<Crop>& crops, int& Wt, bool nchw, size_t desc_slot, size_t stage_slot, int lane) {
    hipStream_t s = lane_engine(lane).stream();
    DevBuf& in_buf = lane == 0 ? input_f32_ : *lane_in_[lane - 1];
    const int n = (int)crops.size();
    const int img_h = (int)cfg_.rec_image_shape[1], img_w = (int)cfg_.rec_image_shape[2];
    std::vector<uint32_t> ws(n), hs(n);
    size_t stage = 0;
    for (int i = 0; i < n; ++i) {
        OAR_CHECK(crops[i].w > 0 && crops[i].h > 0 && (crops[i].host || crops[i].dev), OAR_INVALID_INPUT, "recognizer: empty crop");
        ws[i] = crops[i].w; hs[i] = crops[i].h;
        if (!crops[i].dev) stage += ((size_t)crops[i].w * crops[i].h * 3 + 63) & ~(size_t)63;
    }
    std::vector<int32_t> rws;
    Wt = host::rec_tensor_width(ws, hs, img_h, img_w, (int)cfg_.max_img_w, rws);
    size_t need_in = (size_t)n * 3 * img_h * Wt * sizeof(float);
    size_t need_desc = (desc_slot + n) * sizeof(pp::CropDesc), need_stage = stage_slot + stage;
    if (need_stage > crops_dev_.cap || need_in > in_buf.cap || need_desc > descs_dev_.cap) {
        OAR_HIP(hipStreamSynchronize(s));
        OAR_CHECK(desc_slot == 0 && stage_slot == 0, OAR_INTERNAL, "recognizer staging buffers must be pre-sized for multi-batch runs");
        crops_dev_.reserve(need_stage); in_buf.reserve(need_in); descs_dev_.reserve(need_desc);
    }
    if (need_desc > descs_host_.cap || need_stage > stage_host_.cap) {
        OAR_CHECK(desc_slot == 0 && stage_slot == 0, OAR_INTERNAL, "recognizer pinned buffers must be pre-sized for multi-batch runs");
        descs_host_.reserve(need_desc); stage_host_.reserve(need_stage);
    }
    pp::CropDesc* dh = descs_host_.as<pp::CropDesc>() + desc_slot;
    pp::CropDesc* dd = descs_dev_.as<pp::CropDesc>() + desc_slot;
    size_t off = stage_slot;
    for (int i = 0; i < n; ++i) {
        const uint8_t* d = crops[i].dev;
        if (!d) {
            size_t bytes = (size_t)crops[i].w * crops[i].h * 3;
            std::memcpy(stage_host_.as<uint8_t>() + off, crops[i].host, bytes);
            d = crops_dev_.as<uint8_t>() + off;
            off += (bytes + 63) & ~(size_t)63;
        }
        dh[i].src = d; dh[i].w = (int)crops[i].w; dh[i].h = (int)crops[i].h; dh[i].rw = rws[i]; dh[i].flip = crops[i].flip ? 1 : 0;
    }
    if (stage) OAR_HIP(hipMemcpyAsync(crops_dev_.as<uint8_t>() + stage_slot, stage_host_.as<uint8_t>() + stage_slot, stage, hipMemcpyHostToDevice, s));
    OAR_HIP(hipMemcpyAsync(dd, dh, (size_t)n * sizeof(pp::CropDesc), hipMemcpyHostToDevice, s));
    pp::rec_pack(s, dd, n, img_h, Wt, in_buf.as<float>(), nchw ? 1 : 0);
    return in_buf.as<float>();
}

static_assert(sizeof(pp::ResizedImg) == sizeof(k::StemImg) && sizeof(pp::ResizedImg) == 16, "one table for pp::rec_resize_u8 and k::conv_smallcin_u8");

const pp::ResizedImg* Recognizer::pack_u8(const std::vector<Crop>& crops, int& Wt, size_t desc_slot, size_t stage_slot, int lane) {
    hipStream_t s = lane_engine(lane).stream();
    DevBuf& in_buf = lane == 0 ? input_f32_ : *lane_in_[lane - 1];
    const int n = (int)crops.size();
    const int img_h = (int)cfg_.rec_image_shape[1], img_w = (int)cfg_.rec_image_shape[2];
    std::vector<uint32_t> ws(n), hs(n);
    size_t stage = 0;
    for (int i = 0; i < n; ++i) {
        OAR_CHECK(crops[i].w > 0 && crops[i].h > 0 && (crops[i].host || crops[i].dev), OAR_INVALID_INPUT, "recognizer: empty crop");
        ws[i] = crops[i].w; hs[i] = crops[i].h;
        if (!crops[i].dev) stage += ((size_t)crops[i].w * crops[i].h * 3 + 63) & ~(size_t)63;
    }
    std::vector<int32_t> rws;
    Wt = host::rec_tensor_width(ws, hs, img_h, img_w, (int)cfg_.max_img_w, rws);
    size_t need_in = 0;
    int max_rw = 0;
    for (int i = 0; i < n; ++i) { need_in += ((size_t)img_h * rws[i] * 3 + 63) & ~(size_t)63; max_rw = std::max(max_rw, (int)rws[i]); }
    const size_t need_desc = (desc_slot + n) * sizeof(pp::CropDesc), need_stage = stage_slot + stage, need_imgs = (desc_slot + n) * sizeof(pp::ResizedImg);
    OAR_CHECK(need_stage <= crops_dev_.cap && need_in <= in_buf.cap && need_desc <= descs_dev_.cap && need_imgs <= imgs_dev_.cap && need_desc <= descs_host_.cap &&
                  need_stage <= stage_host_.cap && need_imgs <= imgs_host_.cap, OAR_INTERNAL, "recognizer staging buffers must be pre-sized (run_batches)");
    pp::CropDesc* dh = descs_host_.as<pp::CropDesc>() + desc_slot;
    pp::CropDesc* dd = descs_dev_.as<pp::CropDesc>() + desc_slot;
    pp::ResizedImg* ih = imgs_host_.as<pp::ResizedImg>() + desc_slot;
    pp::ResizedImg* id = imgs_dev_.as<pp::ResizedImg>() + desc_slot;
    size_t off = stage_slot, roff = 0;
    for (int i = 0; i < n; ++i) {
        const uint8_t* d = crops[i].dev;
        if (!d) {
            const size_t bytes = (size_t)crops[i].w * crops[i].h * 3;
            std::memcpy(stage_host_.as<uint8_t>() + off, crops[i].host, bytes);
            d = crops_dev_.as<uint8_t>() + off;
            off += (bytes + 63) & ~(size_t)63;
        }
        dh[i].src = d; dh[i].w = (int)crops[i].w; dh[i].h = (int)crops[i].h; dh[i].rw = rws[i]; dh[i].flip = crops[i].flip ? 1 : 0;
        ih[i].ptr = in_buf.as<uint8_t>() + roff; ih[i].w = rws[i]; ih[i].pad = 0;
        roff += ((size_t)img_h * rws[i] * 3 + 63) & ~(size_t)63;
    }
    if (stage) OAR_HIP(hipMemcpyAsync(crops_dev_.as<uint8_t>() + stage_slot, stage_host_.as<uint8_t>() + stage_slot, stage, hipMemcpyHostToDevice, s));
    OAR_HIP(hipMemcpyAsync(dd, dh, (size_t)n * sizeof(pp::CropDesc), hipMemcpyHostToDevice, s));
    OAR_HIP(hipMemcpyAsync(id, ih, (size_t)n * sizeof(pp::ResizedImg), hipMemcpyHostToDevice, s));
    pp::rec_resize_u8(s, dd, id, n, img_h, max_rw);
    return id;
}

void Recognizer::pack_only(const std::vector<Crop>& crops, std::vector<float>& nchw, uint32_t& Wt_out) {
    std::lock_guard<std::mutex> lk(mu_);
    OAR_HIP(hipSetDevice(eng_->device()));
    nchw.clear(); Wt_out = 0;
    if (crops.empty()) return;
    int Wt = 0;
    const float* d = pack(crops, Wt, true);
    size_t cnt = crops.size() * 3 * (size_t)cfg_.rec_image_shape[1] * Wt;
    nchw.resize(cnt);
    OAR_HIP(hipMemcpyAsync(nchw.data(), d, cnt * 4, hipMemcpyDeviceToHost, eng_->stream()));
    OAR_HIP(hipStreamSynchronize(eng_->stream()));
    Wt_out = (uint32_t)Wt;
}

void Recognizer::run(const std::vector<Crop>& crops, RecOut& out) {
    std::vector<std::vector<Crop>> b(1, crops);
    std::vector<RecOut> o;
    run_batches(b, o);
    out = std::move(o[0]);
}

void Recognizer::run_batches(const std::vector<std::vector<Crop>>& batches, std::vector<RecOut>& outs) {
    std::lock_guard<std::mutex> lk(mu_);
    outs.assign(batches.size(), RecOut());
    OAR_HIP(hipSetDevice(eng_->device()));
    hipStream_t s = eng_->stream();
    const int img_h = (int)cfg_.rec_image_shape[1], img_w = (int)cfg_.rec_image_shape[2];
    size_t total_crops = 0, total_stage = 0, max_in = 0;
    for (auto& b : batches) {
        std::vector<uint32_t> ws, hs;
        for (auto& c : b) {
            ws.push_back(c.w); hs.push_back(c.h);
            OAR_CHECK(c.w > 0 && c.h > 0 && (c.host || c.dev), OAR_INVALID_INPUT, "recognizer: empty crop");
            if (!c.dev) total_stage += ((size_t)c.w * c.h * 3 + 63) & ~(size_t)63;
        }
        if (b.empty()) continue;
        std::vector<int32_t> rws;
        int Wt = host::rec_tensor_width(ws, hs, img_h, img_w, (int)cfg_.max_img_w, rws);
        max_in = std::max(max_in, (size_t)b.size() * 3 * img_h * Wt * sizeof(float));
        total_crops += b.size();
    }
    if (total_crops == 0) return;
    if (total_stage > crops_dev_.cap || max_in > input_f32_.cap || total_crops * sizeof(pp::CropDesc) > descs_dev_.cap) {
        OAR_HIP(hipStreamSynchronize(s));
        crops_dev_.reserve(total_stage); input_f32_.reserve(max_in); descs_dev_.reserve(total_crops * sizeof(pp::CropDesc));
    }
    for (auto& lb : lane_in_)
        if (max_in > lb->cap) { for (auto& le : lanes_) OAR_HIP(hipStreamSynchronize(le->stream())); lb->reserve(max_in); }
    descs_host_.reserve(total_crops * sizeof(pp::CropDesc));
    stage_host_.reserve(total_stage);
    const char* fuse_env = getenv("OAR_REC_FUSE_STEM");
    const bool fuse_stem = !(fuse_env && fuse_env[0] == '0') && eng_->stem_fusable();
    if (fuse_stem) {
        if (total_crops * sizeof(pp::ResizedImg) > imgs_dev_.cap) { OAR_HIP(hipStreamSynchronize(s)); for (auto& le : lanes_) OAR_HIP(hipStreamSynchronize(le->stream())); imgs_dev_.reserve(total_crops * sizeof(pp::ResizedImg)); }
        imgs_host_.reserve(total_crops * sizeof(pp::ResizedImg));
    }

    struct Pending { size_t row0, rows; };
    std::vector<Pending> pend(batches.size(), Pending{0, 0});
    size_t desc_slot = 0, stage_slot = 0, row_total = 0;
    std::vector<int> Wts(batches.size(), 0);
    std::vector<char> fuse_tail(batches.size(), 0);
    for (size_t bi = 0; bi < batches.size(); ++bi) {
        const auto& b = batches[bi];
        if (b.empty()) continue;
        std::vector<uint32_t> ws, hs;
        for (auto& c : b) { ws.push_back(c.w); hs.push_back(c.h); }
        std::vector<int32_t> rws;
        Wts[bi] = host::rec_tensor_width(ws, hs, img_h, img_w, (int)cfg_.max_img_w, rws);
        const Plan& probe = eng_->plan_for({(int64_t)b.size(), 3, img_h, Wts[bi]}, true, false, nullptr, fuse_stem);
        OAR_CHECK(!probe.outputs.empty(), OAR_INTERNAL, "CRNN: no output returned from inference");
        fuse_tail[bi] = probe.outputs[0].dims.size() == 3 && probe.outputs[0].dims[2] > 1024;
        const Plan& plan = fuse_tail[bi] ? eng_->plan_for({(int64_t)b.size(), 3, img_h, Wts[bi]}, true, true, nullptr, fuse_stem) : probe;
        const PlanOutput& po = plan.outputs[0];
        OAR_CHECK(po.dims.size() == 3, OAR_SHAPE_MISMATCH, "CRNN: expected 3D output (batch, time, vocab)");
        OAR_CHECK(po.dims[0] == (int64_t)b.size(), OAR_SHAPE_MISMATCH, "CRNN: output batch differs from input batch");
        outs[bi].T = (uint32_t)po.dims[1]; outs[bi].V = (uint32_t)po.dims[2]; outs[bi].Wt = (uint32_t)Wts[bi];
        pend[bi].row0 = row_total; pend[bi].rows = (size_t)b.size() * po.dims[1];
        if (po.dims[2] == 0) pend[bi].rows = 0;
        row_total += pend[bi].rows;
    }
    if (row_total * 8 > idx_dev_.cap || row_total * 4 > prob_dev_.cap) {
        OAR_HIP(hipStreamSynchronize(s));
        idx_dev_.reserve(row_total * 8); prob_dev_.reserve(row_total * 4);
    }
    idx_host_.reserve(row_total * 8); prob_host_.reserve(row_total * 4);
    const int n_lanes = 1 + (int)lanes_.size();
    std::vector<char> lane_used(n_lanes, 0);
    int next_lane = 0;
    for (size_t bi = 0; bi < batches.size(); ++bi) {
        const auto& b = batches[bi];
        if (b.empty()) continue;
        const int lane = next_lane;
        next_lane = (next_lane + 1) % n_lanes;
        lane_used[lane] = 1;
        Engine& eng = lane_engine(lane);
        hipStream_t sl = eng.stream();
        int Wt = 0;
        const float* in = nullptr;
        const pp::ResizedImg* imgs = nullptr;
        if (fuse_stem) imgs = pack_u8(b, Wt, desc_slot, stage_slot, lane);
        else in = pack(b, Wt, false, desc_slot, stage_slot, lane);
        desc_slot += b.size();
        for (auto& c : b) if (!c.dev) stage_slot += ((size_t)c.w * c.h * 3 + 63) & ~(size_t)63;
        k::StemU8 st{};
        if (fuse_stem) {
            st.src[0] = 2; st.src[1] = 1; st.src[2] = 0;
            st.dev = reinterpret_cast<const k::StemImg*>(imgs);
        }
        const Plan& plan = fuse_stem ? eng.run_stem(st, {(int64_t)b.size(), 3, img_h, Wt}, fuse_tail[bi] != 0)
                                     : eng.run(in, {(int64_t)b.size(), 3, img_h, Wt}, true, fuse_tail[bi] != 0);
        if (pend[bi].rows == 0) continue;
        const PlanOutput& po = plan.outputs[0];
        if (plan.skipped_softmax && plan.ctc_part.kind != Loc::NONE)
            k::ctc_combine(sl, eng.out_ptr(plan.ctc_part), (int64_t)pend[bi].rows, plan.ctc_tiles, idx_dev_.as<int64_t>() + pend[bi].row0,
                           prob_dev_.as<float>() + pend[bi].row0);
        else if (plan.skipped_softmax)
            k::softmax_argmax(sl, eng.out_ptr(po.loc), (int64_t)pend[bi].rows, plan.logits_valid > 0 ? plan.logits_valid : (int)po.dims[2], (int)po.dims[2],
                              idx_dev_.as<int64_t>() + pend[bi].row0, prob_dev_.as<float>() + pend[bi].row0);
        else
            pp::ctc_argmax(sl, eng.out_ptr(po.loc), (int64_t)pend[bi].rows, (int)po.dims[2], idx_dev_.as<int64_t>() + pend[bi].row0,
                           prob_dev_.as<float>() + pend[bi].row0);
    }
    for (int lane = 1; lane < n_lanes; ++lane) {
        if (!lane_used[lane]) continue;
        OAR_HIP(hipEventRecord(lane_done_[lane - 1], lanes_[lane - 1]->stream()));
        OAR_HIP(hipStreamWaitEvent(s, lane_done_[lane - 1], 0));
    }
    if (row_total) {
        OAR_HIP(hipMemcpyAsync(idx_host_.p, idx_dev_.p, row_total * 8, hipMemcpyDeviceToHost, s));
        OAR_HIP(hipMemcpyAsync(prob_host_.p, prob_dev_.p, row_total * 4, hipMemcpyDeviceToHost, s));
    }
    OAR_HIP(hipStreamSynchronize(s));
    for (size_t bi = 0; bi < batches.size(); ++bi) {
        if (pend[bi].rows == 0) continue;
        outs[bi].idx.assign(idx_host_.as<int64_t>() + pend[bi].row0, idx_host_.as<int64_t>() + pend[bi].row0 + pend[bi].rows);
        outs[bi].prob.assign(prob_host_.as<float>() + pend[bi].row0, prob_host_.as<float>() + pend[bi].row0 + pend[bi].rows);
    }
    if (Profiler::get().enabled) Profiler::get().flush();
}

Classifier::Classifier(const uint8_t* onnx, size_t len, const ClsCfg& cfg) : cfg_(cfg) {
    if (cfg_.input_h == 0 || cfg_.input_w == 0) { cfg_.input_h = 224; cfg_.input_w = 224; }
    if (cfg_.topk == 0) cfg_.topk = 1;
    if (cfg_.batch == 0) cfg_.batch = 64;
    eng_.reset(new Engine(onnx, len, cfg_.device_id));
}

const float* Classifier::pack(const std::vector<Image>& images, size_t i0, size_t n, bool nchw) {
    hipStream_t s = eng_->stream();
    const int ch = (int)cfg_.input_h, cw = (int)cfg_.input_w;
    size_t stage = 0;
    for (size_t i = 0; i < n; ++i) {
        const Image& im = images[i0 + i];
        OAR_CHECK(im.w > 0 && im.h > 0 && (im.host || im.dev), OAR_INVALID_INPUT, "classifier: empty image");
        if (!im.dev) stage += ((size_t)im.w * im.h * 3 + 255) & ~(size_t)255;
    }
    const size_t need_in = n * 3 * (size_t)ch * cw * sizeof(float), need_desc = n * sizeof(pp::ClsDesc);
    if (stage > stage_dev_.cap || need_in > input_f32_.cap || need_desc > descs_dev_.cap) {
        OAR_HIP(hipStreamSynchronize(s));
        stage_dev_.reserve(stage); input_f32_.reserve(need_in); descs_dev_.reserve(need_desc);
    } else {
        OAR_HIP(hipStreamSynchronize(s));
    }
    stage_host_.reserve(stage); descs_host_.reserve(need_desc);
    pp::ClsDesc* dh = descs_host_.as<pp::ClsDesc>();
    size_t off = 0;
    for (size_t i = 0; i < n; ++i) {
        const Image& im = images[i0 + i];
        const uint8_t* d = im.dev;
        if (!d) {
            const size_t bytes = (size_t)im.w * im.h * 3;
            std::memcpy(stage_host_.as<uint8_t>() + off, im.host, bytes);
            d = stage_dev_.as<uint8_t>() + off;
            off += (bytes + 255) & ~(size_t)255;
        }
        pp::ClsDesc& c = dh[i];
        c.src = d; c.w = (int)im.w; c.h = (int)im.h; c.pad = 0;
        if (cfg_.resize_short == 0) {
            c.nw = cw; c.nh = ch; c.x1 = 0; c.y1 = 0;
        } else {
            const float shortf = (float)std::min(im.w, im.h);
            const float scale = (float)cfg_.resize_short / shortf;
            const uint32_t nw = (uint32_t)std::max(std::round((float)im.w * scale), (float)cw);
            const uint32_t nh = (uint32_t)std::max(std::round((float)im.h * scale), (float)ch);
            c.nw = (int)nw; c.nh = (int)nh;
            c.x1 = (int)((nw > (uint32_t)cw ? nw - (uint32_t)cw : 0u) / 2);
            c.y1 = (int)((nh > (uint32_t)ch ? nh - (uint32_t)ch : 0u) / 2);
        }
    }
    if (stage) OAR_HIP(hipMemcpyAsync(stage_dev_.p, stage_host_.p, stage, hipMemcpyHostToDevice, s));
    OAR_HIP(hipMemcpyAsync(descs_dev_.p, descs_host_.p, need_desc, hipMemcpyHostToDevice, s));
    const float scale = 1.0f / 255.0f;
    const float mean[3] = {0.485f, 0.456f, 0.406f}, stdv[3] = {0.229f, 0.224f, 0.225f};
    float alpha[3], beta[3];
    for (int c = 0; c < 3; ++c) { alpha[c] = scale / stdv[c]; beta[c] = -mean[c] / stdv[c]; }
    pp::cls_pack(s, descs_dev_.as<pp::ClsDesc>(), (int)n, ch, cw, alpha, beta, input_f32_.as<float>(), nchw ? 1 : 0);
    return input_f32_.as<float>();
}

void Classifier::pack_only(const std::vector<Image>& images, std::vector<float>& nchw) {
    std::lock_guard<std::mutex> lk(mu_);
    OAR_HIP(hipSetDevice(eng_->device()));
    nchw.clear();
    if (images.empty()) return;
    const float* d = pack(images, 0, images.size(), true);
    nchw.resize(images.size() * 3 * (size_t)cfg_.input_h * cfg_.input_w);
    OAR_HIP(hipMemcpyAsync(nchw.data(), d, nchw.size() * 4, hipMemcpyDeviceToHost, eng_->stream()));
    OAR_HIP(hipStreamSynchronize(eng_->stream()));
}

void Classifier::run(const std::vector<Image>& images, ClsOut& out) {
    std::lock_guard<std::mutex> lk(mu_);
    OAR_HIP(hipSetDevice(eng_->device()));
    hipStream_t s = eng_->stream();
    out = ClsOut();
    out.topk = cfg_.topk;
    for (size_t i0 = 0; i0 < images.size(); i0 += cfg_.batch) {
        const size_t n = std::min<size_t>(cfg_.batch, images.size() - i0);
        const float* in = pack(images, i0, n, false);
        const Plan& plan = eng_->run(in, {(int64_t)n, 3, (int64_t)cfg_.input_h, (int64_t)cfg_.input_w}, true);
        OAR_CHECK(!plan.outputs.empty(), OAR_INTERNAL, "PP-LCNet: no output returned from inference");
        const PlanOutput& po = plan.outputs[0];
        OAR_CHECK(po.dims.size() == 2 && po.dims[0] == (int64_t)n, OAR_SHAPE_MISMATCH, "PP-LCNet: failed to convert output to 2D array");
        const int nc = (int)po.dims[1];
        out.n_classes = (uint32_t)nc;
        probs_host_.reserve(n * nc * sizeof(float));
        OAR_HIP(hipMemcpyAsync(probs_host_.p, eng_->out_ptr(po.loc), n * nc * sizeof(float), hipMemcpyDeviceToHost, s));
        OAR_HIP(hipStreamSynchronize(s));
        const float* pr = probs_host_.as<float>();
        const int k = std::min<int>((int)cfg_.topk, nc);
        for (size_t i = 0; i < n; ++i) {
            std::vector<int> order(nc);
            for (int c = 0; c < nc; ++c) order[c] = c;
            const float* row = pr + i * nc;
            std::stable_sort(order.begin(), order.end(), [&](int a, int b) { return row[a] > row[b]; });
            for (int t = 0; t < (int)cfg_.topk; ++t) {
                out.ids.push_back(t < k ? order[t] : -1);
                out.scores.push_back(t < k ? row[order[t]] : 0.0f);
            }
        }
    }
    if (Profiler::get().enabled) Profiler::get().flush();
}

Rectifier::Rectifier(const uint8_t* onnx, size_t len, const RectCfg& cfg) : cfg_(cfg) {
    eng_.reset(new Engine(onnx, len, cfg_.device_id));
}

void Rectifier::run_device(const uint8_t* src, uint32_t w, uint32_t h, uint8_t* dst) {
    std::lock_guard<std::mutex> lk(mu_);
    run_device_locked(src, w, h, dst);
}

void Rectifier::run_device_locked(const uint8_t* src, uint32_t w, uint32_t h, uint8_t* dst) {
// ... 179 lines not shown
                const float x = q[2 * k], y = q[2 * k + 1];
                if (a == 90) { q[2 * k] = (float)m.rotated_h - y; q[2 * k + 1] = x; }
                else if (a == 180) { q[2 * k] = (float)m.rotated_w - x; q[2 * k + 1] = (float)m.rotated_h - y; }
                else if (a == 270) { q[2 * k] = y; q[2 * k + 1] = (float)m.rotated_w - x; }
            }
        };
        for (auto& r : out[i]) {
            back(r.pts, 4);
            if (!r.poly.empty()) back(r.poly.data(), r.poly.size() / 2);
        }
    }
}

void Ocr::predict_core(const std::vector<PageRef>& pages, std::vector<std::vector<OcrRegion>>& out) {
    const int n = (int)pages.size();
    OAR_HIP(hipSetDevice(det_->engine().device()));
    hipStream_t s = det_->engine().stream();
    PhaseTimer timer;
    g_timer = &timer;
    struct TimerReset { ~TimerReset() { g_timer = nullptr; } } timer_reset;
    struct PoolItem { int img; int det_index; uint32_t w, h; float wh_ratio; size_t off; bool flip = false; };
    struct Slot { bool filled = false; OcrRegion r; };
    std::vector<std::vector<Slot>> per_image(n);
    std::vector<PoolItem> pool;
    size_t pool_bytes = 0;
    const float base_ratio = (float)cfg_.rec.rec_image_shape[2] > 0 ? (float)cfg_.rec.rec_image_shape[2] / (float)cfg_.rec.rec_image_shape[1] : 320.0f / 48.0f;

    auto flush = [&]() {
        if (pool.empty()) return;
        OAR_HIP(hipStreamSynchronize(s));
        std::vector<float> line_angle(pool.size(), -1.0f);
        if (line_cls_) {
            std::vector<Classifier::Image> imgs(pool.size());
            for (size_t i = 0; i < pool.size(); ++i) { imgs[i].dev = crop_pool_.as<uint8_t>() + pool[i].off; imgs[i].w = pool[i].w; imgs[i].h = pool[i].h; }
            ClsOut co;
            line_cls_->run(imgs, co);
            for (size_t i = 0; i < pool.size(); ++i) {
                const int c = co.ids[i * co.topk];
                if (c < 0) continue;
                line_angle[i] = (float)c * 180.0f;
                per_image[pool[i].img][pool[i].det_index].r.line_angle = line_angle[i];
                pool[i].flip = c == 1;
            }
        }
        std::vector<PoolItem> sorted = pool;
        std::stable_sort(sorted.begin(), sorted.end(), [](const PoolItem& a, const PoolItem& b) { return a.wh_ratio < b.wh_ratio; });
        const size_t bs = cfg_.region_batch_size;
        std::vector<std::vector<Recognizer::Crop>> batches;
        std::vector<float> chunk_max;
        for (size_t c0 = 0; c0 < sorted.size(); c0 += bs) {
            size_t c1 = std::min(sorted.size(), c0 + bs);
            std::vector<Recognizer::Crop> crops;
            float cm = base_ratio;
            for (size_t i = c0; i < c1; ++i) {
                Recognizer::Crop c;
                c.dev = crop_pool_.as<uint8_t>() + sorted[i].off; c.w = sorted[i].w; c.h = sorted[i].h; c.flip = sorted[i].flip;
                crops.push_back(c);
                if (sorted[i].wh_ratio > cm) cm = sorted[i].wh_ratio;
            }
            batches.push_back(std::move(crops));
            chunk_max.push_back(cm);
        }
        std::vector<RecOut> ros;
        tmark("rec_sort_batching");
        rec_->run_batches(batches, ros);
        tmark("rec_all_batches");
        for (size_t bi = 0; bi < batches.size(); ++bi) {
            const RecOut& ro = ros[bi];
            const size_t c0 = bi * bs;
            for (size_t k = 0; k < batches[bi].size(); ++k) {
                Slot& sl = per_image[sorted[c0 + k].img][sorted[c0 + k].det_index];
                sl.filled = true;
                sl.r.T = ro.T; sl.r.max_wh_ratio = chunk_max[bi];
                if (!ro.idx.empty()) {
                    sl.r.idx.assign(ro.idx.begin() + k * ro.T, ro.idx.begin() + (k + 1) * ro.T);
                    sl.r.prob.assign(ro.prob.begin() + k * ro.T, ro.prob.begin() + (k + 1) * ro.T);
                }
            }
        }
        pool.clear();
        pool_bytes = 0;
    };

    int flush_count = 0;
    bool planning_failed = false;
    auto run_chunk = [&](int start, int end) {
        std::vector<PageRef> chunk(pages.begin() + start, pages.begin() + end);
        std::vector<DetBoxes> boxes;
        std::vector<const uint8_t*> dev_pages;
        size_t desc_used = 0;
        auto plan_pages = [&](int first, int count) {
            struct Planned { int img; int det_index; host::CropPlan plan; };
            std::vector<Planned> planned;
            for (int li = first; li < first + count; ++li) {
                const int img = start + li;
                const bool poly = cfg_.det.box_type == 1;
                const bool poly_sort = cfg_.box_sort == 2 || (cfg_.box_sort == 0 && poly);
                std::vector<uint32_t> poly_off;
                std::vector<int> order;
                if (poly) {
                    poly_off.assign(boxes[li].counts.size() + 1, 0);
                    for (size_t b = 0; b < boxes[li].counts.size(); ++b) poly_off[b + 1] = poly_off[b] + boxes[li].counts[b];
                } else if (poly_sort) {
                    const size_t nb = boxes[li].pts.size() / 8;
                    poly_off.resize(nb + 1);
                    for (size_t b = 0; b <= nb; ++b) poly_off[b] = (uint32_t)(4 * b);
                }
                if (poly_sort) {
                    order = host::sort_poly_boxes(boxes[li].pts, poly_off);
                } else if (!poly) {
                    order = host::sort_quad_boxes(boxes[li].pts);
                } else {
                    std::vector<float> aabb(boxes[li].counts.size() * 8);
                    for (size_t b = 0; b < boxes[li].counts.size(); ++b) {
                        float x0 = 3.4e38f, y0 = 3.4e38f, x1 = -3.4e38f, y1 = -3.4e38f;
                        for (uint32_t q = poly_off[b]; q < poly_off[b + 1]; ++q) {
                            const float x = boxes[li].pts[2 * q], y = boxes[li].pts[2 * q + 1];
                            x0 = std::min(x0, x); x1 = std::max(x1, x); y0 = std::min(y0, y); y1 = std::max(y1, y);
                        }
                        const float q8[8] = {x0, y0, x1, y0, x1, y1, x0, y1};
                        std::memcpy(aabb.data() + b * 8, q8, sizeof q8);
                    }
                    order = host::sort_quad_boxes(aabb);
                }
                per_image[img].resize(order.size());
                for (size_t k = 0; k < order.size(); ++k) {
                    Slot& sl = per_image[img][k];
                    sl.r.det_score = boxes[li].scores[order[k]];
                    host::CropPlan pl;
                    if (poly) {
                        const float* pp_ = boxes[li].pts.data() + (size_t)poly_off[order[k]] * 2;
                        const uint32_t np_ = boxes[li].counts[order[k]];
                        sl.r.poly.assign(pp_, pp_ + (size_t)np_ * 2);
                        std::memset(sl.r.pts, 0, sizeof sl.r.pts);
                        if (np_ == 4) {
                            std::memcpy(sl.r.pts, pp_, sizeof sl.r.pts);
                            pl = host::plan_crop((int)pages[img].w, (int)pages[img].h, sl.r.pts);
                        } else {
                            pl = host::plan_bbox_crop((int)pages[img].w, (int)pages[img].h, pp_, (int)np_);
                        }
                    } else {
                        std::memcpy(sl.r.pts, boxes[li].pts.data() + (size_t)order[k] * 8, sizeof sl.r.pts);
                        pl = host::plan_crop((int)pages[img].w, (int)pages[img].h, sl.r.pts);
                    }
                    if (pl.mode == 0) continue;
                    sl.r.crop_w = (uint32_t)pl.out_w(); sl.r.crop_h = (uint32_t)pl.out_h();
                    planned.push_back({img, (int)k, pl});
                }
            }
            size_t pi = 0;
            while (pi < planned.size()) {
                size_t room = cfg_.max_pooled_crops - pool.size();
                size_t take = std::min(room, planned.size() - pi);
                size_t add_bytes = 0;
                int max_px = 0;
                for (size_t q = pi; q < pi + take; ++q) {
                    const host::CropPlan& pl = planned[q].plan;
                    add_bytes += ((size_t)pl.out_w() * pl.out_h() * 3 + 63) & ~(size_t)63;
                    max_px = std::max(max_px, pl.out_w() * pl.out_h());
                }
                if (pool_bytes + add_bytes > crop_pool_.cap) {
                    OAR_HIP(hipStreamSynchronize(s));
                    DevBuf bigger;
                    bigger.reserve((pool_bytes + add_bytes) * 2);
                    if (pool_bytes) OAR_HIP(hipMemcpy(bigger.p, crop_pool_.p, pool_bytes, hipMemcpyDeviceToDevice));
                    std::swap(bigger.p, crop_pool_.p); std::swap(bigger.cap, crop_pool_.cap);
                }
                const size_t need_desc = (desc_used + take) * sizeof(pp::WarpDesc);
                if (need_desc > warp_descs_dev_.cap || need_desc > warp_descs_host_.cap) {
                    OAR_HIP(hipStreamSynchronize(s));
                    const size_t want = std::max<size_t>(2 * take * sizeof(pp::WarpDesc), 8192 * sizeof(pp::WarpDesc));
                    warp_descs_host_.reserve(want); warp_descs_dev_.reserve(want);
                    desc_used = 0;
                }
                pp::WarpDesc* wd = warp_descs_host_.as<pp::WarpDesc>() + desc_used;
                pp::WarpDesc* wd_dev = warp_descs_dev_.as<pp::WarpDesc>() + desc_used;
                for (size_t q = 0; q < take; ++q) {
                    const Planned& P = planned[pi + q];
                    const host::CropPlan& pl = P.plan;
                    pp::WarpDesc& d = wd[q];
                    d.page = dev_pages[P.img - start]; d.page_w = (int)pages[P.img].w; d.page_h = (int)pages[P.img].h;
                    d.left = pl.left; d.top = pl.top; d.cw = pl.cw; d.ch = pl.ch; d.ow = pl.ow; d.oh = pl.oh; d.rot = pl.rot; d.mode = pl.mode;
                    std::memcpy(d.inv, pl.inv, sizeof d.inv);
                    d.out_off = (int64_t)pool_bytes;
                    PoolItem it;
                    it.img = P.img; it.det_index = P.det_index; it.w = (uint32_t)pl.out_w(); it.h = (uint32_t)pl.out_h();
                    it.wh_ratio = (float)it.w / (float)std::max<uint32_t>(it.h, 1);
                    it.off = pool_bytes;
                    pool.push_back(it);
                    pool_bytes += ((size_t)it.w * it.h * 3 + 63) & ~(size_t)63;
                }
                OAR_HIP(hipMemcpyAsync(wd_dev, wd, take * sizeof(pp::WarpDesc), hipMemcpyHostToDevice, s));
                pp::rotate_crops(s, wd_dev, (int)take, crop_pool_.as<uint8_t>(), max_px);
                desc_used += take;
                pi += take;
                if (pool.size() >= cfg_.max_pooled_crops) { flush(); ++flush_count; desc_used = 0; }
            }
        };
        auto guarded_plan = [&](int first, int count) {
            try { plan_pages(first, count); } catch (...) { planning_failed = true; throw; }
        };
        det_->run(chunk, cfg_.det_thresh, cfg_.det_box_thresh, cfg_.det_unclip_ratio, boxes, &dev_pages, guarded_plan);
        OAR_HIP(hipStreamSynchronize(s));
        tmark("crop_sync");
    };
    for (int start = 0; start < n; start += (int)cfg_.image_batch_size) {
        const int end = std::min(n, start + (int)cfg_.image_batch_size);
        const size_t pool_mark = pool.size(), bytes_mark = pool_bytes;
        const int flush_mark = flush_count;
        try {
            run_chunk(start, end);
        } catch (const Error& err) {
            if (end - start <= 1 || planning_failed) throw;
            fprintf(stderr, "[oar] batched text detection failed (%s); falling back to per-image detection for pages %d..%d\n", err.what(), start, end);
            (void)hipStreamSynchronize(s);
            (void)hipGetLastError();
            if (flush_count == flush_mark) { pool.resize(pool_mark); pool_bytes = bytes_mark; }
            else {
                pool.erase(std::remove_if(pool.begin(), pool.end(), [&](const PoolItem& it) { return it.img >= start; }), pool.end());
                pool_bytes = pool.empty() ? 0 : pool.back().off + ((((size_t)pool.back().w * pool.back().h * 3) + 63) & ~(size_t)63);
            }
            for (int i = start; i < end; ++i) per_image[i].clear();
            for (int i = start; i < end; ++i) run_chunk(i, i + 1);
        }
    }
    flush();
    out.assign(n, {});
    for (int i = 0; i < n; ++i)
        for (auto& sl : per_image[i])
            if (sl.filled) out[i].push_back(std::move(sl.r));
    tmark("assemble");
    timer.dump("ocr.predict");
    if (Profiler::get().enabled) Profiler::get().flush();
}

}
```

### oar_ocr_amd/csrc/pipeline.h

```cpp
#pragma once
#include <atomic>
#include <condition_variable>
#include <functional>
#include <memory>
#include <mutex>
#include <thread>
#include <vector>

#include "db_host.h"
#include "engine.h"
#include "prepost.h"

namespace oar {

class ThreadPool {
   public:
    explicit ThreadPool(int n);
    ~ThreadPool();
    void parallel_for(int count, const std::function<void(int)>& fn);
    int size() const { return (int)workers_.size(); }
    void set_active(bool on);
    struct ActiveScope { ThreadPool& p; explicit ActiveScope(ThreadPool& pool) : p(pool) { p.set_active(true); } ~ActiveScope() { p.set_active(false); } };
    static int available_cpus();
    std::function<void()> selftest_worker_delay_, selftest_publish_delay_;

   private:
    void loop();
    std::vector<std::thread> workers_;
    std::mutex mu_;
    std::condition_variable cv_;
    std::atomic<const std::function<void(int)>*> fn_{nullptr};
    std::atomic<int> gen_{0}, done_{0}, count_{0};
    std::atomic<uint64_t> state_{0};
    bool claim(int gen, int count, int& index);
    std::atomic<bool> stop_{false};
    std::atomic<int> active_{0};
    std::mutex err_mu_;
    std::exception_ptr err_;
};

struct PageRef {
    const uint8_t* host = nullptr;
    const uint8_t* dev = nullptr;
    uint32_t w = 0, h = 0;
};

struct DetBoxes {
    std::vector<float> pts;
    std::vector<float> scores;
    std::vector<uint32_t> counts;
};

struct ContourBufs {
    DevBuf rows, band_y, n_bands, lists, scratch, ctrl, table_dev;
    PinBuf ctrl_host, table, packed;
    static constexpr uint32_t kSegsPerPage = 4096;
    size_t packed_words_per_page = 0;
    void reserve(int pages, int sub_pages, int H, int W, int n_sub);
    bool fits(int pages, int sub_pages, int H, int W, int n_sub) const;
};

class Detector {
   public:
    Detector(const uint8_t* onnx, size_t len, const oar_det_cfg& cfg);
    ~Detector();
    using ReadyFn = std::function<void(int first, int count)>;
    void run(const std::vector<PageRef>& pages, float thresh, float box_thresh, float unclip, std::vector<DetBoxes>& out,
             std::vector<const uint8_t*>* dev_pages_out = nullptr, const ReadyFn& on_ready = nullptr);
    Engine& engine() { return *eng_; }
    int lanes() const { return 1 + (int)lanes_.size(); }
    hipStream_t lane_stream(int lane) const { return lane == 0 ? eng_->stream() : lanes_[lane - 1]->stream(); }
    static void postprocess_host(const float* pred, int H, int W, uint32_t src_w, uint32_t src_h, float thresh, float box_thresh,
                                 float unclip, uint32_t max_candidates, DetBoxes& out, int score_mode = 0, int use_dilation = 0, int box_type = 0);
    ThreadPool& pool() { return *pool_; }
    static std::vector<host::Contour> trace_device_mask(const uint8_t* d_mask, int H, int W, uint32_t max_contours, bool gpu_contours = true);

   private:
    void run_group(const std::vector<int>& idx, const std::vector<PageRef>& pages, uint32_t rh, uint32_t rw, float thresh,
                   float box_thresh, float unclip, std::vector<DetBoxes>& out, const ReadyFn& on_ready);
    std::unique_ptr<Engine> eng_;
    std::vector<std::unique_ptr<Engine>> lanes_;
    std::vector<std::unique_ptr<DevBuf>> lane_in_;
    hipEvent_t lanes_start_ = nullptr;
    Engine& lane_engine(int lane) { return lane == 0 ? *eng_ : *lanes_[lane - 1]; }
    void sync_lanes();
    std::unique_ptr<ThreadPool> pool_;
    oar_det_cfg cfg_;
    DevBuf pages_dev_, resized_dev_, input_f32_, mask_dev_, probs_keep_;
    DevBuf mask_dil_;
    DevBuf mask_bits_;
    DevBuf padded_dev_;
    std::vector<const uint8_t*> det_src_;
    std::vector<uint32_t> det_w_, det_h_;
    std::vector<hipEvent_t> sub_events_, mask_ready_, score_done_;
    struct ScoreSlot {
        PinBuf boxes_host, scores_host; DevBuf boxes_dev, scores_dev; std::vector<size_t> base; size_t total = 0;
        PinBuf poly_pts_host, poly_desc_host; DevBuf poly_pts_dev, poly_desc_dev;
        PinBuf unclip_host; DevBuf unclip_dev; bool unclipped = false;
    };
    std::vector<std::unique_ptr<ScoreSlot>> score_slots_;
    std::vector<float> finish_pts_;
    std::vector<uint8_t> finish_ok_;
    hipStream_t copy_stream_ = nullptr;
    hipStream_t upload_stream2_ = nullptr;
    hipStream_t upload_stream_ = nullptr;
    hipEvent_t stage_free_ = nullptr;
    std::vector<hipEvent_t> upload_done_, upload_done2_;
    std::vector<const uint8_t*> upload_src_;
    hipStream_t score_stream_ = nullptr;
    PinBuf mask_host_;
    ContourBufs trace_;
    std::vector<const uint8_t*> page_ptrs_;
    std::mutex mu_;
};

struct RecOut {
    uint32_t T = 0, V = 0, Wt = 0;
    std::vector<int64_t> idx;
    std::vector<float> prob;
};

class Recognizer {
   public:
    Recognizer(const uint8_t* onnx, size_t len, const oar_rec_cfg& cfg, const std::vector<hipStream_t>& lane_streams = {});
    ~Recognizer();
    struct Crop { const uint8_t* host = nullptr; const uint8_t* dev = nullptr; uint32_t w = 0, h = 0; bool flip = false; };
    void run(const std::vector<Crop>& crops, RecOut& out);
    void run_batches(const std::vector<std::vector<Crop>>& batches, std::vector<RecOut>& outs);
    void pack_only(const std::vector<Crop>& crops, std::vector<float>& nchw, uint32_t& Wt);
    Engine& engine() { return *eng_; }

   private:
    const float* pack(const std::vector<Crop>& crops, int& Wt, bool nchw, size_t desc_slot = 0, size_t stage_slot = 0, int lane = 0);
    const pp::ResizedImg* pack_u8(const std::vector<Crop>& crops, int& Wt, size_t desc_slot, size_t stage_slot, int lane);
    DevBuf imgs_dev_; PinBuf imgs_host_;
    Engine& lane_engine(int lane) { return lane == 0 ? *eng_ : *lanes_[lane - 1]; }
    std::unique_ptr<Engine> eng_;
    std::vector<std::unique_ptr<Engine>> lanes_;
    std::vector<std::unique_ptr<DevBuf>> lane_in_;
    std::vector<hipEvent_t> lane_done_;
    oar_rec_cfg cfg_;
    DevBuf crops_dev_, descs_dev_, input_f32_, idx_dev_, prob_dev_;
    PinBuf descs_host_, idx_host_, prob_host_, stage_host_;
    std::mutex mu_;
};

struct ClsCfg {
    int32_t device_id = 0;
    uint32_t input_h = 224, input_w = 224;
    uint32_t resize_short = 256;
    uint32_t topk = 1;
    uint32_t batch = 64;
};
struct ClsOut { std::vector<int32_t> ids; std::vector<float> scores; uint32_t topk = 0, n_classes = 0; };
class Classifier {
   public:
    Classifier(const uint8_t* onnx, size_t len, const ClsCfg& cfg);
    struct Image { const uint8_t* host = nullptr; const uint8_t* dev = nullptr; uint32_t w = 0, h = 0; };
    void run(const std::vector<Image>& images, ClsOut& out);
    void pack_only(const std::vector<Image>& images, std::vector<float>& nchw);
    Engine& engine() { return *eng_; }
    const ClsCfg& cfg() const { return cfg_; }

   private:
    const float* pack(const std::vector<Image>& images, size_t i0, size_t n, bool nchw);
    std::unique_ptr<Engine> eng_;
    ClsCfg cfg_;
    DevBuf stage_dev_, descs_dev_, input_f32_;
    PinBuf stage_host_, descs_host_, probs_host_;
    std::mutex mu_;
};

struct RectCfg { int32_t device_id = 0; uint32_t target_h = 512, target_w = 512; };
class Rectifier {
   public:
    Rectifier(const uint8_t* onnx, size_t len, const RectCfg& cfg);
    void run_device(const uint8_t* src, uint32_t w, uint32_t h, uint8_t* dst);
    void run_host(const uint8_t* src, uint32_t w, uint32_t h, uint8_t* dst);
    struct Page { const uint8_t* src = nullptr; uint32_t w = 0, h = 0; uint8_t* dst = nullptr; };
    void run_device_batch(const std::vector<Page>& pages);
    Engine& engine() { return *eng_; }

   private:
    void run_device_locked(const uint8_t* src, uint32_t w, uint32_t h, uint8_t* dst);
    std::unique_ptr<Engine> eng_;
    RectCfg cfg_;
    DevBuf resized_dev_, input_f32_, out_u8_, io_dev_;
    std::mutex mu_;
};

struct OcrRegion {
    float pts[8];
    std::vector<float> poly;
    float det_score;
    uint32_t crop_w, crop_h, T;
    float max_wh_ratio;
    std::vector<int64_t> idx;
    std::vector<float> prob;
    float line_angle = -1.0f;
};

class Ocr {
   public:
    Ocr(const uint8_t* det, size_t det_len, const uint8_t* rec, size_t rec_len, const oar_ocr_cfg& cfg);
    struct PageMeta { float angle = -1.0f; bool rectified = false; uint32_t rotated_w = 0, rotated_h = 0; };
    void predict(const std::vector<PageRef>& pages, std::vector<std::vector<OcrRegion>>& out, std::vector<PageMeta>* meta_out = nullptr);
    void attach(Classifier* doc_orientation, Rectifier* rectifier, Classifier* line_orientation) { doc_cls_ = doc_orientation; rect_ = rectifier; line_cls_ = line_orientation; }
    Detector& det() { return *det_; }
    Recognizer& rec() { return *rec_; }

   private:
    void predict_core(const std::vector<PageRef>& pages, std::vector<std::vector<OcrRegion>>& out);
    void preprocess_pages(const std::vector<PageRef>& pages, std::vector<PageRef>& cur);
    std::unique_ptr<Detector> det_;
    std::unique_ptr<Recognizer> rec_;
    oar_ocr_cfg cfg_;
    DevBuf crop_pool_, warp_descs_dev_;
    Classifier* doc_cls_ = nullptr;
    Rectifier* rect_ = nullptr;
    Classifier* line_cls_ = nullptr;
    std::vector<PageMeta> meta_;
    DevBuf pre_pages_;
    DevBuf upload_pages_;
    PinBuf warp_descs_host_;
    std::mutex mu_;
};

}
```

### oar_ocr_amd/csrc/prepost.h

```cpp
#pragma once
#include <hip/hip_runtime.h>

#include <cstdint>

namespace oar {
namespace pp {

void normalize(hipStream_t s, const uint8_t* rgb, float* out, int64_t n_images, int64_t plane, const int src[3],
               const float alpha[3], const float beta[3], int layout);
void normalize_pages(hipStream_t s, const uint8_t* const* d_pages, int n_pages, float* out, int64_t plane, const int src[3], const float alpha[3],
                     const float beta[3], int layout);

struct CropDesc {
    const uint8_t* src;
    int32_t w, h;
    int32_t rw;
    int32_t flip;
};
void rec_pack(hipStream_t s, const CropDesc* d_descs, int n, int img_h, int Wt, float* out, int nchw);
struct ResizedImg { uint8_t* ptr; int32_t w; int32_t pad; };
void rec_resize_u8(hipStream_t s, const CropDesc* d_descs, const ResizedImg* d_dst, int n, int img_h, int max_rw);

void resize_triangle(hipStream_t s, const uint8_t* src, int w, int h, uint8_t* dst, int nw, int nh);

void threshold(hipStream_t s, const float* pred, uint8_t* mask, int64_t n, float thresh);

void pack_mask_bits(hipStream_t s, const uint8_t* mask, uint8_t* bits, int n_images, int height, int width);
void db_keep_and_pack(hipStream_t s, const float* net_out, int64_t img_stride, float* probs, uint8_t* bits, int n_images, int height, int width, float thresh);

void dilate3x3(hipStream_t s, const uint8_t* mask, uint8_t* out, int n_images, int height, int width);

struct SegRec { int32_t page, y0, y1, x0, x1; uint32_t off, used, n_contours, flags; };
enum { kTraceCtlTotal = 0, kTraceCtlNSmall = 1, kTraceCtlNLarge = 2, kTraceCtlCurSmall = 3, kTraceCtlCurLarge = 4, kTraceCtlSegments = 5, kTraceCtlOverflow = 6,
       kTraceCtlWords = 8 };
inline int trace_max_bands(int H) { return H / 2 + 1; }
void trace_contours(hipStream_t s, const uint8_t* masks, int n_pages, int H, int W, uint8_t* rows, int32_t* band_y, int32_t* n_bands, uint32_t* lists,
                    uint32_t list_cap, uint32_t* scratch, uint32_t* packed, uint32_t packed_cap_words, uint32_t* ctrl, uint32_t* ctrl_host, SegRec* table_dev,
                    SegRec* table, uint32_t table_cap);

void ctc_argmax(hipStream_t s, const float* probs, int64_t rows, int vocab, int64_t* idx, float* prob);

struct ScoreBox {
    float pts[8];
    int32_t image;
    int32_t pad;
};
void box_scores(hipStream_t s, const float* pred, int height, int width, const ScoreBox* d_boxes, int n_boxes, float* d_scores);

constexpr int kUnclipMaxPts = 80;
struct UnclipOut { int32_t n_pts; int32_t pad; float pts[kUnclipMaxPts * 2]; };
void unclip_quads(hipStream_t s, const ScoreBox* d_boxes, int n_boxes, float ratio, UnclipOut* d_out);

struct PolyDesc { int32_t first, count, image, pad; };
void poly_scores(hipStream_t s, const float* pred, int height, int width, const float* d_pts_xy, const PolyDesc* d_polys, int n_polys, float* d_scores);

struct WarpDesc {
    const uint8_t* page;
    int32_t page_w, page_h;
    int32_t left, top, cw, ch;
    int32_t ow, oh;
    int32_t rot;
    int32_t mode;
    float inv[9];
    int64_t out_off;
};
void rotate_crops(hipStream_t s, const WarpDesc* d_descs, int n, uint8_t* out_pool, int max_out_pixels);

struct ClsDesc {
    const uint8_t* src;
    int32_t w, h;
    int32_t nw, nh;
    int32_t x1, y1;
    int32_t pad;
};
void cls_pack(hipStream_t s, const ClsDesc* d_descs, int n, int crop_h, int crop_w, const float alpha[3], const float beta[3], float* out, int nchw);
void rotate_rgb(hipStream_t s, const uint8_t* src, int w, int h, int quarter, uint8_t* dst);
void bgr_planes_to_rgb(hipStream_t s, const float* planes, int64_t plane, float scale, uint8_t* out);

}
}
```

### oar_ocr_amd/csrc/prepost.hip

```cpp
#include "prepost.h"

#include <hip/hip_runtime.h>

#include "common.h"

namespace oar {
namespace pp {

static inline unsigned grid_for(long work, int block = 256, long cap = 256L * 32) {
    long g = (work + block - 1) / block;
    if (g < 1) g = 1;
    if (g > cap) g = cap;
    return (unsigned)g;
}

struct NormP {
    int src[3];
    float alpha[3], beta[3];
};
struct NormSrcs { const uint8_t* p[32]; };
__global__ __launch_bounds__(256) void normalize_kernel(const uint8_t* __restrict__ rgb, NormSrcs srcs, int use_srcs, float* __restrict__ out, long n_images,
                                                        long plane, NormP p, int layout) {
    const long quads_per_img = (plane + 3) >> 2;
    const long total = n_images * quads_per_img;
// ... 430 lines not shown
        rx[rn] = gx; ry[rn] = gy; ++rn;
    }
    while (rn > 1 && rx[rn - 1] == rx[0] && ry[rn - 1] == ry[0]) --rn;
    if (rn < 3) { o.n_pts = 0; return; }
    int cnt = 0;
    bool overflow = false;
    auto emit = [&](double gx, double gy) {
        if (cnt < kUnclipMaxPts) {
            o.pts[cnt * 2] = (float)((double)(long long)round(gx) / kGrid);
            o.pts[cnt * 2 + 1] = (float)((double)(long long)round(gy) / kGrid);
        } else overflow = true;
        ++cnt;
    };
    const double grid_delta = delta * kGrid;
    if (fabs(grid_delta) < 0.5) {
        for (int i = 0; i < rn; ++i) emit((double)rx[i], (double)ry[i]);
    } else {
        double twice = 0.0;
        for (int i = 0, p = rn - 1; i < rn; p = i++) twice += (double)(ry[p] + ry[i]) * (double)(rx[p] - rx[i]);
        const double radius = twice * 0.5 < 0 ? -grid_delta : grid_delta;
        const double r = fabs(radius), tol = r * 0.002;
        const double per_turn = fmin(kPi / acos(1.0 - tol / r), r * kPi);
        double sn = sin(2.0 * kPi / per_turn);
        const double cs = cos(2.0 * kPi / per_turn);
        if (radius < 0.0) sn = -sn;
        const double per_rad = per_turn / (2.0 * kPi);
        double ux[4], uy[4];
        for (int e = 0; e < rn; ++e) {
            const int f = e + 1 == rn ? 0 : e + 1;
            double dx = (double)(rx[f] - rx[e]), dy = (double)(ry[f] - ry[e]);
            if (dx == 0.0 && dy == 0.0) { ux[e] = uy[e] = 0.0; continue; }
            const double inv_len = 1.0 / sqrt(dx * dx + dy * dy);
            dx *= inv_len; dy *= inv_len;
            ux[e] = dy; uy[e] = -dx;
        }
        for (int v = 0, in_e = rn - 1; v < rn; in_e = v++) {
            const double cx = (double)rx[v], cy = (double)ry[v];
            double turn_sin = uy[v] * ux[in_e] - uy[in_e] * ux[v];
            const double turn_cos = ux[v] * ux[in_e] + uy[v] * uy[in_e];
            turn_sin = turn_sin > 1.0 ? 1.0 : turn_sin < -1.0 ? -1.0 : turn_sin;
            double sx = ux[in_e] * radius, sy = uy[in_e] * radius;
            const double ex = cx + ux[v] * radius, ey = cy + uy[v] * radius;
            if (turn_cos > -0.999 && turn_sin * radius < 0) { o.n_pts = -1; return; }
            emit(cx + sx, cy + sy);
            const int hops = (int)ceil(per_rad * fabs(atan2(turn_sin, turn_cos)));
            for (int h = 1; h < hops; ++h) {
                const double nx = sx * cs - sn * sy, ny = sx * sn + sy * cs;
                sx = nx; sy = ny;
                emit(cx + sx, cy + sy);
            }
            emit(ex, ey);
        }
    }
    if (overflow) { o.n_pts = -1; return; }
    if (cnt > 1 && fabsf(o.pts[0] - o.pts[(cnt - 1) * 2]) < 1.1920929e-7f && fabsf(o.pts[1] - o.pts[(cnt - 1) * 2 + 1]) < 1.1920929e-7f) --cnt;
    o.n_pts = cnt < 3 ? 0 : cnt;
}
void unclip_quads(hipStream_t s, const ScoreBox* d_boxes, int n_boxes, float ratio, UnclipOut* d_out) {
    if (n_boxes == 0) return;
    ProfScope ps(s, "unclip", 0.0, 0.0);
    hipLaunchKernelGGL(unclip_quads_kernel, dim3((n_boxes + 63) / 64), dim3(64), 0, s, d_boxes, n_boxes, ratio, d_out);
}

__global__ __launch_bounds__(256) void poly_scores_kernel(const float* pred, int height, int width, const float* pts, const PolyDesc* polys, float* scores) {
    __shared__ float rsum[256];
    __shared__ unsigned rcnt[256];
    extern __shared__ float lp_pts[];
    const PolyDesc pd = polys[blockIdx.x];
    const float* map = pred + (long)pd.image * height * width;
    const float* gp = pts + (long)pd.first * 2;
    const int n = pd.count;
    const int cap = 8192;
    const bool staged = n * 2 <= cap;
    if (staged) for (int i = threadIdx.x; i < n * 2; i += 256) lp_pts[i] = gp[i];
    __syncthreads();
    const float* P = staged ? lp_pts : gp;
    float mnx = INFINITY, mny = INFINITY, mxx = -INFINITY, mxy = -INFINITY;
    if (n == 0) { mnx = mny = mxx = mxy = 0.0f; }
    for (int i = 0; i < n; ++i) {
        const float x = P[i * 2], y = P[i * 2 + 1];
        if (x < mnx) mnx = x; if (x > mxx) mxx = x;
        if (y < mny) mny = y; if (y > mxy) mxy = y;
    }
    float fx0 = fminf(fmaxf(floorf(mnx), 0.0f), (float)width - 1.0f), fx1 = fminf(fmaxf(ceilf(mxx), 0.0f), (float)width - 1.0f);
    float fy0 = fminf(fmaxf(floorf(mny), 0.0f), (float)height - 1.0f), fy1 = fminf(fmaxf(ceilf(mxy), 0.0f), (float)height - 1.0f);
    const unsigned start_y = f2u(fy0), end_y = f2u(fy1) + 1, start_x = f2u(fx0), end_x = f2u(fx1) + 1;
    float total = 0.0f;
    unsigned long long pixels = 0;
    for (unsigned y0 = start_y; y0 < end_y; y0 += 256) {
        const unsigned yy = y0 + threadIdx.x;
        float line = 0.0f;
        unsigned lp = 0;
        if (yy < end_y && n > 0) {
            const float y = (float)yy + 0.5f;
            const unsigned yi = f2u(y);
            const float* row = map + (long)yi * width;
            float last_x = -INFINITY;
            int last_e = -1;
            bool have_open = false;
            float open_x = 0.0f;
            for (;;) {
                float bx = INFINITY;
                int be = -1;
                for (int i = 0; i < n; ++i) {
                    const int j = i + 1 == n ? 0 : i + 1;
                    const float p1y = P[i * 2 + 1], p2y = P[j * 2 + 1];
                    if (!(((p1y <= y && y < p2y) || (p2y <= y && y < p1y)) && fabsf(p2y - p1y) > 1.1920929e-7f)) continue;
                    const float p1x = P[i * 2], p2x = P[j * 2];
                    const float x = p1x + (y - p1y) * (p2x - p1x) / (p2y - p1y);
                    const bool after = x > last_x || (x == last_x && i > last_e);
                    if (after && (x < bx || (x == bx && i < be) || be < 0)) { bx = x; be = i; }
                }
                if (be < 0) break;
                last_x = bx; last_e = be;
                if (!have_open) { open_x = bx; have_open = true; continue; }
                have_open = false;
                if (yi < (unsigned)height) {
                    const unsigned x1 = f2u(fmaxf(open_x, (float)start_x)), x2 = f2u(fminf(bx, (float)end_x));
                    if (x1 < x2 && x1 >= start_x && x2 <= end_x) {
                        const unsigned xe = x2 < (unsigned)width ? x2 : (unsigned)width;
                        if (x1 < xe) {
                            line = span_sum(row, x1, xe, line);
                            lp += xe - x1;
                        }
                    }
                }
            }
        }
        rsum[threadIdx.x] = line; rcnt[threadIdx.x] = lp;
        __syncthreads();
        if (threadIdx.x == 0) {
            const unsigned lim = min(256u, end_y - y0);
            for (unsigned i = 0; i < lim; ++i) { total += rsum[i]; pixels += rcnt[i]; }
        }
        __syncthreads();
    }
    if (threadIdx.x == 0) scores[blockIdx.x] = pixels > 0 ? total / (float)pixels : 0.0f;
}
void poly_scores(hipStream_t s, const float* pred, int height, int width, const float* d_pts_xy, const PolyDesc* d_polys, int n_polys, float* d_scores) {
    if (n_polys == 0) return;
    ProfScope ps(s, "poly_scores", 0.0, 0.0);
    hipLaunchKernelGGL(poly_scores_kernel, dim3(n_polys), dim3(256), 8192 * sizeof(float), s, pred, height, width, d_pts_xy, d_polys, d_scores);
}

__device__ __forceinline__ float cubic_kernel(float t) {
    const float A = -0.5f;
    float a = fabsf(t);
    if (a <= 1.0f) return (A + 2.0f) * a * a * a - (A + 3.0f) * a * a + 1.0f;
    else if (a < 2.0f) return A * a * a * a - 5.0f * A * a * a + 8.0f * A * a - 4.0f * A;
    return 0.0f;
}
__device__ __forceinline__ int clampi(int v, int lo, int hi) { return v < lo ? lo : (v > hi ? hi : v); }

__global__ __launch_bounds__(256) void rotate_crops_kernel(const WarpDesc* descs, uint8_t* pool) {
    const WarpDesc d = descs[blockIdx.y];
    const int out_w = d.rot ? d.oh : d.ow, out_h = d.rot ? d.ow : d.oh;
    const long total = (long)out_w * out_h;
    uint8_t* out = pool + d.out_off;
    const uint8_t* crop = d.page + ((long)d.top * d.page_w + d.left) * 3;
    const long stride = (long)d.page_w * 3;
    for (long i = (long)blockIdx.x * blockDim.x + threadIdx.x; i < total; i += (long)gridDim.x * blockDim.x) {
        int xo = (int)(i % out_w), yo = (int)(i / out_w);
        int dx = d.rot ? d.ow - 1 - yo : xo, dy = d.rot ? xo : yo;
        uint8_t r, g, b;
        if (d.mode == 1) {
            const uint8_t* p = crop + (long)dy * stride + (long)dx * 3;
            r = p[0]; g = p[1]; b = p[2];
        } else {
            float fx = (float)dx, fy = (float)dy;
            float px = d.inv[0] * fx; px = d.inv[1] * fy + px; px = d.inv[2] * 1.0f + px;
            float py = d.inv[3] * fx; py = d.inv[4] * fy + py; py = d.inv[5] * 1.0f + py;
            float pz = d.inv[6] * fx; pz = d.inv[7] * fy + pz; pz = d.inv[8] * 1.0f + pz;
            if (fabsf(pz) > 1.1920929e-7f) {
                float x = px / pz, y = py / pz;
                int xi = (int)floorf(x), yi = (int)floorf(y);
                float ddx = x - (float)xi, ddy = y - (float)yi;
                float wx[4] = {cubic_kernel(ddx + 1.0f), cubic_kernel(ddx), cubic_kernel(ddx - 1.0f), cubic_kernel(ddx - 2.0f)};
                float wy[4] = {cubic_kernel(ddy + 1.0f), cubic_kernel(ddy), cubic_kernel(ddy - 1.0f), cubic_kernel(ddy - 2.0f)};
                long cx[4], cy[4];
#pragma unroll
                for (int k = 0; k < 4; ++k) { cx[k] = (long)clampi(xi - 1 + k, 0, d.cw - 1) * 3; cy[k] = (long)clampi(yi - 1 + k, 0, d.ch - 1) * stride; }
                float r0 = 0.0f, r1 = 0.0f, r2 = 0.0f;
#pragma unroll
                for (int j = 0; j < 4; ++j)
#pragma unroll
                    for (int k = 0; k < 4; ++k) {
                        float wt = wx[k] * wy[j];
                        const uint8_t* p = crop + cy[j] + cx[k];
                        r0 += wt * (float)p[0]; r1 += wt * (float)p[1]; r2 += wt * (float)p[2];
                    }
                r = (uint8_t)fminf(fmaxf(roundf(r0), 0.0f), 255.0f);
                g = (uint8_t)fminf(fmaxf(roundf(r1), 0.0f), 255.0f);
                b = (uint8_t)fminf(fmaxf(roundf(r2), 0.0f), 255.0f);
            } else {
                r = crop[0]; g = crop[1]; b = crop[2];
            }
        }
        out[i * 3] = r; out[i * 3 + 1] = g; out[i * 3 + 2] = b;
    }
}
void rotate_crops(hipStream_t s, const WarpDesc* d_descs, int n, uint8_t* out_pool, int max_out_pixels) {
    if (n == 0) return;
    ProfScope ps(s, "rotate_crops", 6.0 * (double)n * max_out_pixels, 0.0);
    hipLaunchKernelGGL(rotate_crops_kernel, dim3(grid_for(max_out_pixels, 256, 64), n), dim3(256), 0, s, d_descs, out_pool);
}

__global__ __launch_bounds__(256) void cls_pack_kernel(const ClsDesc* descs, int crop_h, int crop_w, NormP np_, float* out, int nchw) {
    const int n = blockIdx.y;
    const ClsDesc d = descs[n];
    const long plane = (long)crop_h * crop_w;
    for (long i = (long)blockIdx.x * blockDim.x + threadIdx.x; i < plane; i += (long)gridDim.x * blockDim.x) {
        const int ox = (int)(i % crop_w), oy = (int)(i / crop_w);
        uint8_t px[3];
        resize_pixel(d.src, d.w, d.h, d.nw, d.nh, d.x1 + ox, d.y1 + oy, px);
        float v[3];
#pragma unroll
        for (int c = 0; c < 3; ++c) { float t = (float)px[np_.src[c]] * np_.alpha[c]; v[c] = t + np_.beta[c]; }
        if (nchw) {
            float* o = out + (long)n * 3 * plane + i;
            o[0] = v[0]; o[plane] = v[1]; o[2 * plane] = v[2];
        } else {
            float* o = out + ((long)n * plane + i) * 3;
            o[0] = v[0]; o[1] = v[1]; o[2] = v[2];
        }
    }
}
void cls_pack(hipStream_t s, const ClsDesc* d_descs, int n, int crop_h, int crop_w, const float alpha[3], const float beta[3], float* out, int nchw) {
    if (n == 0 || crop_h * crop_w == 0) return;
    NormP p;
    for (int i = 0; i < 3; ++i) { p.src[i] = i; p.alpha[i] = alpha[i]; p.beta[i] = beta[i]; }
    ProfScope ps(s, "cls_pack", 12.0 * (double)n * crop_h * crop_w, 0.0);
    hipLaunchKernelGGL(cls_pack_kernel, dim3(grid_for((long)crop_h * crop_w, 256, 64), n), dim3(256), 0, s, d_descs, crop_h, crop_w, p, out, nchw);
}

__global__ __launch_bounds__(256) void rotate_rgb_kernel(const uint8_t* __restrict__ src, int w, int h, int quarter, uint8_t* __restrict__ dst) {
    const long total = (long)w * h;
    for (long i = (long)blockIdx.x * blockDim.x + threadIdx.x; i < total; i += (long)gridDim.x * blockDim.x) {
        const int x = (int)(i % w), y = (int)(i / w);
        long o;
        if (quarter == 1) o = (long)x * h + (h - 1 - y);
        else if (quarter == 2) o = (long)(h - 1 - y) * w + (w - 1 - x);
        else if (quarter == 3) o = (long)(w - 1 - x) * h + y;
        else o = i;
        const uint8_t* p = src + i * 3;
        dst[o * 3] = p[0]; dst[o * 3 + 1] = p[1]; dst[o * 3 + 2] = p[2];
    }
}
void rotate_rgb(hipStream_t s, const uint8_t* src, int w, int h, int quarter, uint8_t* dst) {
    if ((long)w * h == 0) return;
    ProfScope ps(s, "rotate_rgb", 6.0 * (double)w * h, 0.0);
    hipLaunchKernelGGL(rotate_rgb_kernel, dim3(grid_for((long)w * h)), dim3(256), 0, s, src, w, h, quarter, dst);
}

__global__ __launch_bounds__(256) void bgr_planes_to_rgb_kernel(const float* __restrict__ planes, long plane, float scale, uint8_t* __restrict__ out) {
    for (long p = (long)blockIdx.x * blockDim.x + threadIdx.x; p < plane; p += (long)gridDim.x * blockDim.x) {
#pragma unroll
        for (int c = 0; c < 3; ++c) {
            float v = planes[(long)(2 - c) * plane + p] * scale;
            v = v < 0.0f ? 0.0f : (v > 255.0f ? 255.0f : v);
            out[p * 3 + c] = (v != v) ? (uint8_t)0 : (uint8_t)v;
        }
    }
}
void bgr_planes_to_rgb(hipStream_t s, const float* planes, int64_t plane, float scale, uint8_t* out) {
    if (plane == 0) return;
    ProfScope ps(s, "bgr_planes_to_rgb", 15.0 * (double)plane, 0.0);
    hipLaunchKernelGGL(bgr_planes_to_rgb_kernel, dim3(grid_for(plane)), dim3(256), 0, s, planes, (long)plane, scale, out);
}

}
}
```

### rust/oar-mi355x-sys/src/lib.rs

```rust
#![allow(non_camel_case_types, non_snake_case, clippy::too_many_arguments)]
#![no_std]

use core::ffi::{c_char, c_int, c_void};

pub type oar_status = c_int;
pub const OAR_OK: oar_status = 0;
pub const OAR_INVALID_INPUT: oar_status = 1;
pub const OAR_MODEL_LOAD: oar_status = 2;
pub const OAR_UNSUPPORTED_OP: oar_status = 3;
pub const OAR_SHAPE_MISMATCH: oar_status = 4;
pub const OAR_DEVICE: oar_status = 5;
pub const OAR_OOM: oar_status = 6;
pub const OAR_INTERNAL: oar_status = 7;

pub type oar_precision = c_int;
pub const OAR_PRECISION_F32: oar_precision = 0;

pub type oar_dtype = c_int;
pub const OAR_DTYPE_F32: oar_dtype = 1;
pub const OAR_DTYPE_I64: oar_dtype = 7;

pub const OAR_RECT_NATIVE_SIZE: u32 = 0xFFFFFFFF;

#[repr(C)]
// ... 236 lines not shown
    pub n_classes: u32,
    pub class_ids: *mut i32,
    pub scores: *mut f32,
}

#[repr(C)]
#[derive(Debug, Clone, Copy)]
pub struct oar_rect_cfg {
    pub device_id: i32,
    pub target_h: u32,
    pub target_w: u32,
}

#[repr(C)]
#[derive(Debug, Clone, Copy)]
pub struct oar_layout_cfg {
    pub device_id: i32,
    pub input_h: u32,
    pub input_w: u32,
    pub resize_filter: i32,
    pub color_bgr: i32,
    pub scale: f32,
    pub mean: [f32; 3],
    pub std: [f32; 3],
    pub num_classes: u32,
    pub model_type: i32,
    pub score_threshold: f32,
    pub nms_threshold: f32,
    pub max_detections: u32,
}

#[repr(C)]
#[derive(Debug, Clone, Copy)]
pub struct oar_layout_result {
    pub n_images: u32,
    pub n_boxes: u32,
    pub box_offsets: *mut u32,
    pub boxes: *mut f32,
    pub classes: *mut i32,
    pub scores: *mut f32,
    pub feature_dim: u32,
}

#[repr(C)]
#[derive(Debug, Clone, Copy)]
pub struct oar_ppdoc_cfg {
    pub score_threshold: f32,
    pub class_thresholds: *const f32,
    pub layout_nms: i32,
    pub image_class_id: i32,
    pub formula_class_id: i32,
    pub class_merge_modes: *const i32,
}

#[repr(C)]
#[derive(Debug, Clone, Copy)]
pub struct oar_prof_entry {
    pub name: [c_char; 48],
    pub launches: u64,
    pub total_ms: f64,
    pub alg_bytes: f64,
    pub alg_flops: f64,
}

#[link(name = "OarMi355x")]
unsafe extern "C" {
    pub fn oar_last_error(buf: *mut c_char, cap: usize) -> usize;
    pub fn oar_version(buf: *mut c_char, cap: usize) -> usize;
    pub fn oar_device_count() -> c_int;
    pub fn oar_engine_create(onnx: *const u8, onnx_len: usize, cfg: *const oar_engine_cfg, out: *mut *mut oar_engine) -> oar_status;
    pub fn oar_engine_destroy(e: *mut oar_engine);
    pub fn oar_engine_input_name(e: *const oar_engine, buf: *mut c_char, cap: usize) -> oar_status;
    pub fn oar_engine_run(e: *mut oar_engine, input: *const f32, dims: *const i64, rank: i32, outs: *mut oar_tensor, max_out: i32, n_out: *mut i32) -> oar_status;
    pub fn oar_tensor_free(t: *mut oar_tensor);
    pub fn oar_engine_run_named(e: *mut oar_engine, inputs: *const oar_input, n_in: i32, outs: *mut oar_tensor, max_out: i32, n_out: *mut i32) -> oar_status;
    pub fn oar_engine_run_first_f32(e: *mut oar_engine, inputs: *const oar_input, n_in: i32, view: oar_output_view_fn, user: *mut c_void) -> oar_status;
    pub fn oar_engine_io(e: *const oar_engine, inputs: *mut oar_io_info, max_in: i32, n_in: *mut i32, outputs: *mut oar_io_info, max_out: i32, n_out: *mut i32) -> oar_status;
    pub fn oar_engine_cost(e: *mut oar_engine, dims: *const i64, rank: i32, flops: *mut f64, bytes: *mut f64, n_kernels: *mut i32) -> oar_status;
    pub fn oar_engine_cache_stats(e: *mut oar_engine, cached_plans: *mut u64, evicted_plans: *mut u64) -> oar_status;
    pub fn oar_engine_set_decode_stop(e: *mut oar_engine, token: i64) -> oar_status;
    pub fn oar_engine_decode_stats(e: *mut oar_engine, out: *mut oar_decode_stats) -> oar_status;
    pub fn oar_onnx_inspect(onnx: *const u8, onnx_len: usize, summary: *mut c_char, cap: usize) -> oar_status;
    pub fn oar_det_create(onnx: *const u8, onnx_len: usize, cfg: *const oar_det_cfg, out: *mut *mut oar_det) -> oar_status;
    pub fn oar_det_destroy(d: *mut oar_det);
    pub fn oar_det_run(d: *mut oar_det, rgb: *const *const u8, widths: *const u32, heights: *const u32, n_images: u32, thresh: f32, box_thresh: f32, unclip_ratio: f32, out: *mut oar_det_result) -> oar_status;
    pub fn oar_det_result_free(r: *mut oar_det_result);
    pub fn oar_db_postprocess(pred: *const f32, height: u32, width: u32, src_w: u32, src_h: u32, thresh: f32, box_thresh: f32, unclip_ratio: f32, max_candidates: u32, out: *mut oar_det_result) -> oar_status;
    pub fn oar_db_postprocess_ex(pred: *const f32, height: u32, width: u32, src_w: u32, src_h: u32, thresh: f32, box_thresh: f32, unclip_ratio: f32, max_candidates: u32, box_type: i32, score_mode: i32, use_dilation: i32, out: *mut oar_det_result) -> oar_status;
    pub fn oar_rec_create(onnx: *const u8, onnx_len: usize, cfg: *const oar_rec_cfg, out: *mut *mut oar_rec) -> oar_status;
    pub fn oar_rec_destroy(r: *mut oar_rec);
    pub fn oar_rec_run(r: *mut oar_rec, rgb: *const *const u8, widths: *const u32, heights: *const u32, n_crops: u32, out: *mut oar_rec_result) -> oar_status;
    pub fn oar_rec_result_free(r: *mut oar_rec_result);
    pub fn oar_ctc_dict_create(dict_utf8: *const c_char, len: usize, use_space_char: i32, out: *mut *mut oar_ctc_dict) -> oar_status;
    pub fn oar_ctc_dict_destroy(d: *mut oar_ctc_dict);
    pub fn oar_ctc_dict_classes(d: *const oar_ctc_dict) -> u32;
    pub fn oar_ctc_decode(dict: *const oar_ctc_dict, indices: *const i64, probs: *const f32, batch: u32, seq_len: u32, score_threshold: f32, out: *mut oar_text_result) -> oar_status;
    pub fn oar_text_result_free(r: *mut oar_text_result);
    pub fn oar_ocr_create(det_onnx: *const u8, det_len: usize, rec_onnx: *const u8, rec_len: usize, cfg: *const oar_ocr_cfg, out: *mut *mut oar_ocr) -> oar_status;
    pub fn oar_ocr_destroy(o: *mut oar_ocr);
    pub fn oar_ocr_predict(o: *mut oar_ocr, rgb: *const *const u8, widths: *const u32, heights: *const u32, n_images: u32, out: *mut oar_ocr_result) -> oar_status;
    pub fn oar_ocr_predict_device(o: *mut oar_ocr, d_rgb: *const *const u8, widths: *const u32, heights: *const u32, n_images: u32, out: *mut oar_ocr_result) -> oar_status;
    pub fn oar_ocr_result_free(r: *mut oar_ocr_result);
    pub fn oar_ocr_predict_async(o: *mut oar_ocr, rgb: *const *const u8, widths: *const u32, heights: *const u32, n_images: u32, device_pages: i32, ticket: *mut u64) -> oar_status;
    pub fn oar_ocr_wait(o: *mut oar_ocr, ticket: u64, out: *mut oar_ocr_result) -> oar_status;
    pub fn oar_ocr_decode(dict: *const oar_ctc_dict, res: *const oar_ocr_result, score_threshold: f32, out: *mut oar_text_result) -> oar_status;
    pub fn oar_ctc_word_boxes(line_pts_xy: *const f32, n_points: u32, text_utf8: *const c_char, text_len: usize, col_indices: *const u32, n_cols: u32, seq_len: u32, wh_ratio: f32, max_wh_ratio: f32, boxes: *mut f32, cap_boxes: u32, n_boxes: *mut u32) -> oar_status;
    pub fn oar_char_positions_to_word_boxes(line_pts_xy: *const f32, n_points: u32, char_positions: *const f32, n_positions: u32, char_count: u32, boxes: *mut f32, cap_boxes: u32, n_boxes: *mut u32) -> oar_status;
    pub fn oar_ocr_word_boxes(res: *const oar_ocr_result, txt: *const oar_text_result, out: *mut oar_word_boxes) -> oar_status;
    pub fn oar_word_boxes_free(w: *mut oar_word_boxes);
    pub fn oar_shard_range(n_items: u64, world_size: u32, rank: u32, begin: *mut u64, end: *mut u64) -> oar_status;
    pub fn oar_ocr_pack(res: *const oar_ocr_result, txt: *const oar_text_result, blob: *mut *mut u8, len: *mut usize) -> oar_status;
    pub fn oar_blob_free(blob: *mut u8);
    pub fn oar_packed_merge(blobs: *const *const u8, lens: *const usize, n_blobs: u32, out: *mut oar_packed_pages) -> oar_status;
    pub fn oar_packed_pages_free(p: *mut oar_packed_pages);
    pub fn oar_cls_create(onnx: *const u8, onnx_len: usize, cfg: *const oar_cls_cfg, out: *mut *mut oar_cls) -> oar_status;
    pub fn oar_cls_destroy(c: *mut oar_cls);
    pub fn oar_cls_run(c: *mut oar_cls, rgb: *const *const u8, widths: *const u32, heights: *const u32, n_images: u32, out: *mut oar_cls_result) -> oar_status;
    pub fn oar_cls_result_free(r: *mut oar_cls_result);
    pub fn oar_cls_preprocess(c: *mut oar_cls, rgb: *const *const u8, widths: *const u32, heights: *const u32, n_images: u32, out_nchw: *mut f32) -> oar_status;
    pub fn oar_rect_create(onnx: *const u8, onnx_len: usize, cfg: *const oar_rect_cfg, out: *mut *mut oar_rect) -> oar_status;
    pub fn oar_rect_destroy(r: *mut oar_rect);
    pub fn oar_rect_run(r: *mut oar_rect, rgb: *const u8, width: u32, height: u32, out_rgb: *mut u8) -> oar_status;
    pub fn oar_ocr_attach(o: *mut oar_ocr, doc_orientation: *mut oar_cls, rectifier: *mut oar_rect, line_orientation: *mut oar_cls) -> oar_status;
    pub fn oar_k_rotate_rgb(rgb: *const u8, w: u32, h: u32, quarter: i32, out: *mut u8) -> oar_status;
    pub fn oar_k_bgr_planes_to_rgb(planes: *const f32, plane: u64, scale: f32, out: *mut u8) -> oar_status;
    pub fn oar_host_rotate_back_points(pts: *mut f32, n_points: u32, angle: f32, rotated_w: u32, rotated_h: u32) -> oar_status;
    pub fn oar_layout_create(onnx: *const u8, onnx_len: usize, cfg: *const oar_layout_cfg, out: *mut *mut oar_layout) -> oar_status;
    pub fn oar_layout_destroy(l: *mut oar_layout);
    pub fn oar_layout_run(l: *mut oar_layout, rgb: *const *const u8, widths: *const u32, heights: *const u32, n_images: u32, out: *mut oar_layout_result) -> oar_status;
    pub fn oar_layout_result_free(r: *mut oar_layout_result);
    pub fn oar_layout_preprocess(l: *mut oar_layout, rgb: *const u8, width: u32, height: u32, out_chw: *mut f32) -> oar_status;
    pub fn oar_k_resize_filter(rgb: *const u8, w: u32, h: u32, nw: u32, nh: u32, filter: i32, out: *mut u8) -> oar_status;
    pub fn oar_k_layout_postprocess(pred: *const f32, n_images: u32, rows: u32, feat: u32, src_wh: *const f32, num_classes: u32, model_type: i32, score_threshold: f32, nms_threshold: f32, max_detections: u32, out: *mut oar_layout_result) -> oar_status;
    pub fn oar_layout_run_ppdoc(l: *mut oar_layout, rgb: *const *const u8, widths: *const u32, heights: *const u32, n_images: u32, cfg: *const oar_ppdoc_cfg, out: *mut oar_layout_result) -> oar_status;
    pub fn oar_k_ppdoc_postprocess(pred: *const f32, n_images: u32, rows: u32, feat: u32, src_wh: *const f32, num_classes: u32, cfg: *const oar_ppdoc_cfg, out: *mut oar_layout_result) -> oar_status;
    pub fn oar_host_nms_with_merge(boxes: *const f32, classes: *const i32, scores: *const f32, n: u32, mode_of_class: *const i32, num_classes: u32, nms_threshold: f32, max_detections: u32, out_boxes: *mut f32, out_classes: *mut i32, out_scores: *mut f32) -> i32;
    pub fn oar_dev_alloc(device_id: i32, bytes: usize, out: *mut *mut c_void) -> oar_status;
    pub fn oar_dev_upload(dst: *mut c_void, src: *const c_void, bytes: usize) -> oar_status;
    pub fn oar_dev_download(dst: *mut c_void, src: *const c_void, bytes: usize) -> oar_status;
    pub fn oar_dev_free(p: *mut c_void);
    pub fn oar_dev_synchronize(device_id: i32) -> oar_status;
    pub fn oar_k_normalize(rgb: *const u8, w: u32, h: u32, src_channels: *const i32, alpha: *const f32, beta: *const f32, hwc_layout: i32, out: *mut f32) -> oar_status;
    pub fn oar_k_rec_preprocess(rgb: *const *const u8, widths: *const u32, heights: *const u32, n: u32, img_h: u32, img_w: u32, max_img_w: u32, out_nchw: *mut f32, tensor_width: *mut u32) -> oar_status;
    pub fn oar_k_rec_preprocess_flip(rgb: *const *const u8, widths: *const u32, heights: *const u32, flips: *const u8, n: u32, img_h: u32, img_w: u32, max_img_w: u32, out_nchw: *mut f32, tensor_width: *mut u32) -> oar_status;
    pub fn oar_k_resize_triangle(rgb: *const u8, w: u32, h: u32, nw: u32, nh: u32, out: *mut u8) -> oar_status;
    pub fn oar_k_threshold(pred: *const f32, n: usize, thresh: f32, mask: *mut u8) -> oar_status;
    pub fn oar_k_dilate(mask: *const u8, height: u32, width: u32, out: *mut u8) -> oar_status;
    pub fn oar_k_poly_scores(pred: *const f32, height: u32, width: u32, pts_xy: *const f32, counts: *const u32, n_polys: u32, scores: *mut f32) -> oar_status;
    pub fn oar_k_contours(mask: *const u8, width: u32, height: u32, max_contours: u32, n_contours: *mut i32, offsets: *mut i64, pts_xy: *mut i32, types: *mut i32, cap_points: i64) -> oar_status;
    pub fn oar_k_ctc_argmax(probs: *const f32, rows: usize, vocab: usize, idx: *mut i64, prob: *mut f32) -> oar_status;
    pub fn oar_k_unclip(boxes: *const f32, n_boxes: u32, ratio: f32, counts: *mut i32, pts_xy: *mut f32, cap_points: u32) -> oar_status;
    pub fn oar_k_box_scores(pred: *const f32, height: u32, width: u32, boxes: *const f32, n_boxes: u32, scores: *mut f32) -> oar_status;
    pub fn oar_k_rotate_crop(rgb: *const u8, w: u32, h: u32, box_: *const f32, out: *mut u8, cap: usize, out_w: *mut u32, out_h: *mut u32) -> oar_status;
    pub fn oar_image_decode(bytes: *const u8, len: usize, rgb: *mut *mut u8, width: *mut u32, height: *mut u32) -> oar_status;
    pub fn oar_image_free(rgb: *mut u8);
    pub fn oar_image_decode_device(bytes: *const u8, len: usize, device_id: i32, dev_rgb: *mut *mut c_void, width: *mut u32, height: *mut u32) -> oar_status;
    pub fn oar_host_candidates(mask: *const u8, width: u32, height: u32, max_candidates: u32, max_bands: i32, boxes8: *mut f32, cap: i32) -> i32;
    pub fn oar_host_contours(mask: *const u8, width: u32, height: u32, max_contours: u32, max_bands: i32, offsets: *mut i64, pts_xy: *mut i32, types: *mut i32, cap_points: i64) -> i32;
    pub fn oar_host_contours_bits(mask: *const u8, width: u32, height: u32, max_contours: u32, max_bands: i32, offsets: *mut i64, pts_xy: *mut i32, types: *mut i32, cap_points: i64) -> i32;
    pub fn oar_host_unclip(box8: *const f32, ratio: f32, out_xy: *mut f32, cap_points: i32) -> i32;
    pub fn oar_host_approx_poly_dp(xy: *const f32, n_points: i32, epsilon: f32, out_xy: *mut f32, cap_points: i32) -> i32;
    pub fn oar_host_perimeter(xy: *const f32, n_points: i32) -> f32;
    pub fn oar_host_unclip_poly(xy: *const f32, n_points: i32, ratio: f32, out_xy: *mut f32, cap_points: i32) -> i32;
    pub fn oar_host_offset_ring(xy: *const i64, n_points: i32, radius: f64, out_xy: *mut i64, cap_points: i32) -> i32;
    pub fn oar_host_ring_outline(xy: *const i64, n_points: i32, negative: i32, out_xy: *mut i64, cap_points: i32) -> i32;
    pub fn oar_host_sort_poly_boxes(pts_xy: *const f32, offsets: *const u32, n: i32, order: *mut i32);
    pub fn oar_host_mini_box(xy: *const f32, n_points: i32, box8: *mut f32, min_side: *mut f32) -> i32;
    pub fn oar_host_convex_hull(xy: *const f32, n_points: i32, out_xy: *mut f32, cap_points: i32) -> i32;
    pub fn oar_host_sort_quad_boxes(boxes8: *const f32, n: i32, order: *mut i32);
    pub fn oar_host_pool_selftest(threads: i32, jobs: i32) -> i32;
    pub fn oar_host_plan_crop(img_w: u32, img_h: u32, box8: *const f32, plan: *mut i32, inv: *mut f32);
    pub fn oar_debug_inject_failure(site: *const c_char, count: i32) -> oar_status;
    pub fn oar_prof_reset();
    pub fn oar_prof_enable(on: i32);
    pub fn oar_prof_filter(class_name: *const c_char);
    pub fn oar_prof_sampling(stride: i32, phase: i32);
    pub fn oar_prof_snapshot(entries: *mut oar_prof_entry, cap: i32) -> i32;
}
```

Before: 2489 images/sec.

## Flatten rotate_crops into per-item tiles and vectorize axis-aligned crop copies

```diff
diff --git a/include/oar_mi355x.h b/include/oar_mi355x.h
--- a/include/oar_mi355x.h
+++ b/include/oar_mi355x.h
@@ -346,6 +346,11 @@
                             uint32_t n_boxes, float* scores);
 oar_status oar_k_rotate_crop(const uint8_t* rgb, uint32_t w, uint32_t h, const float box[8], uint8_t* out,
                              size_t cap, uint32_t* out_w, uint32_t* out_h);
+oar_status oar_k_rotate_crops(const uint8_t* const* pages, const uint32_t* page_ws, const uint32_t* page_hs, uint32_t n_pages, const float* boxes8,
+                              const uint32_t* box_page, uint32_t n_boxes, uint8_t* out, size_t cap, uint32_t* out_ws, uint32_t* out_hs, size_t* out_offs,
+                              size_t* needed);
+oar_status oar_k_rec_resize_u8(const uint8_t* const* rgb, const uint32_t* widths, const uint32_t* heights, const uint8_t* flips, uint32_t n, uint32_t img_h,
+                               uint32_t img_w, uint32_t max_img_w, uint8_t* out, uint32_t* tensor_width, int32_t* resized_widths);
 
 oar_status oar_image_decode(const uint8_t* bytes, size_t len, uint8_t** rgb, uint32_t* width, uint32_t* height);
 void oar_image_free(uint8_t* rgb);
diff --git a/oar_ocr_amd/api.py b/oar_ocr_amd/api.py
--- a/oar_ocr_amd/api.py
+++ b/oar_ocr_amd/api.py
@@ -141,7 +141,7 @@
     "oar_engine_cache_stats", "oar_onnx_inspect", "oar_host_contours", "oar_ctc_dict_create", "oar_ctc_dict_destroy", "oar_ctc_dict_classes",
     "oar_ctc_decode", "oar_ocr_decode", "oar_text_result_free", "oar_db_postprocess_ex", "oar_k_dilate", "oar_k_poly_scores", "oar_debug_inject_failure", "oar_k_contours", "oar_host_contours_bits",
     "oar_k_unclip", "oar_k_rec_preprocess_flip", "oar_layout_create", "oar_layout_destroy", "oar_layout_run", "oar_layout_result_free", "oar_layout_preprocess", "oar_k_resize_filter", "oar_k_layout_postprocess", "oar_layout_run_ppdoc", "oar_k_ppdoc_postprocess", "oar_host_nms_with_merge", "oar_image_decode_device", "oar_ocr_predict_async", "oar_ocr_wait", "oar_ctc_word_boxes", "oar_char_positions_to_word_boxes", "oar_ocr_word_boxes", "oar_word_boxes_free", "oar_image_decode", "oar_image_free", "oar_host_approx_poly_dp", "oar_host_perimeter", "oar_host_unclip_poly", "oar_host_offset_ring", "oar_host_ring_outline", "oar_host_sort_poly_boxes",
-    "oar_engine_set_decode_stop", "oar_engine_decode_stats",
+    "oar_engine_set_decode_stop", "oar_engine_decode_stats", "oar_k_rotate_crops", "oar_k_rec_resize_u8",
 ]
 
 
@@ -234,6 +234,8 @@
     L.oar_image_decode_device.argtypes = [vp, C.c_size_t, C.c_int32, C.POINTER(C.c_void_p), C.POINTER(C.c_uint32), C.POINTER(C.c_uint32)]
     L.oar_image_free.restype = None
     L.oar_k_rotate_crop.argtypes = [vp, C.c_uint32, C.c_uint32, f32p, vp, C.c_size_t, u32p, u32p]
+    L.oar_k_rotate_crops.argtypes = [u8pp, u32p, u32p, C.c_uint32, vp, u32p, C.c_uint32, vp, C.c_size_t, u32p, u32p, C.POINTER(C.c_size_t), C.POINTER(C.c_size_t)]
+    L.oar_k_rec_resize_u8.argtypes = [u8pp, u32p, u32p, vp, C.c_uint32, C.c_uint32, C.c_uint32, C.c_uint32, vp, u32p, vp]
     L.oar_host_candidates.argtypes = [vp, C.c_uint32, C.c_uint32, C.c_uint32, C.c_int32, vp, C.c_int32]
     L.oar_host_candidates.restype = C.c_int32
     L.oar_host_contours.argtypes = [vp, C.c_uint32, C.c_uint32, C.c_uint32, C.c_int32, vp, vp, vp, C.c_int64]
@@ -1567,6 +1569,32 @@
     return out[:ow.value * oh.value * 3].reshape(oh.value, ow.value, 3).copy()
 
 
+def k_rotate_crops(pages_, boxes, box_page):
+    imgs, ptrs, ws, hs = _img_arrays(pages_)
+    boxes = np.ascontiguousarray(boxes, np.float32).reshape(-1, 8)
+    n = boxes.shape[0]
+    bp = (C.c_uint32 * max(n, 1))(*[int(v) for v in box_page])
+    ows, ohs = (C.c_uint32 * max(n, 1))(), (C.c_uint32 * max(n, 1))()
+    offs = (C.c_size_t * max(n, 1))()
+    need = C.c_size_t(0)
+    _check(lib().oar_k_rotate_crops(ptrs, ws, hs, len(imgs), _p(boxes), bp, n, None, 0, ows, ohs, offs, C.byref(need)))
+    out = np.empty(max(need.value, 1), np.uint8)
+    _check(lib().oar_k_rotate_crops(ptrs, ws, hs, len(imgs), _p(boxes), bp, n, _p(out), out.size, ows, ohs, offs, C.byref(need)))
+    return [None if ows[i] == 0 else out[offs[i]:offs[i] + ows[i] * ohs[i] * 3].reshape(ohs[i], ows[i], 3).copy() for i in range(n)]
+
+
+def k_rec_resize_u8(crops, img_h=48, img_w=320, max_img_w=3200, flips=None):
+    imgs, ptrs, ws, hs = _img_arrays(crops)
+    tw = C.c_uint32(0)
+    fl = None if flips is None else np.ascontiguousarray(np.asarray(flips, bool).astype(np.uint8))
+    flp = None if fl is None else _p(fl)
+    _check(lib().oar_k_rec_resize_u8(ptrs, ws, hs, flp, len(imgs), img_h, img_w, max_img_w, None, C.byref(tw), None))
+    out = np.empty((len(imgs), img_h, tw.value, 3), np.uint8)
+    rws = np.zeros(len(imgs), np.int32)
+    _check(lib().oar_k_rec_resize_u8(ptrs, ws, hs, flp, len(imgs), img_h, img_w, max_img_w, _p(out), C.byref(tw), _p(rws)))
+    return out, rws
+
+
 def host_candidates(mask, max_candidates=1000, max_bands=1):
     mask = np.ascontiguousarray(mask, np.uint8)
     h, w = mask.shape
diff --git a/oar_ocr_amd/csrc/c_api.cc b/oar_ocr_amd/csrc/c_api.cc
--- a/oar_ocr_amd/csrc/c_api.cc
+++ b/oar_ocr_amd/csrc/c_api.cc
@@ -1166,18 +1166,114 @@
         *out_w = (uint32_t)pl.out_w(); *out_h = (uint32_t)pl.out_h();
         size_t bytes = (size_t)pl.out_w() * pl.out_h() * 3;
         OAR_CHECK(out && cap >= bytes, OAR_INVALID_INPUT, "oar_k_rotate_crop: output buffer too small");
-        DevBuf dpage, dd, dout;
-        dpage.reserve((size_t)w * h * 3); dd.reserve(sizeof(pp::WarpDesc)); dout.reserve(bytes);
-        OAR_HIP(hipMemcpy(dpage.p, rgb, (size_t)w * h * 3, hipMemcpyHostToDevice));
         pp::WarpDesc d;
         std::memset(&d, 0, sizeof d);
+        d.ow = pl.ow; d.oh = pl.oh; d.rot = pl.rot; d.mode = pl.mode;
+        std::vector<pp::WarpItem> items(pp::rotate_crops_items(&d, 1, nullptr));
+        DevBuf dpage, dd, dout;
+        dpage.reserve((size_t)w * h * 3); dd.reserve(sizeof(pp::WarpDesc) + items.size() * sizeof(pp::WarpItem)); dout.reserve(bytes);
+        OAR_HIP(hipMemcpy(dpage.p, rgb, (size_t)w * h * 3, hipMemcpyHostToDevice));
         d.page = dpage.as<uint8_t>(); d.page_w = (int)w; d.page_h = (int)h;
-        d.left = pl.left; d.top = pl.top; d.cw = pl.cw; d.ch = pl.ch; d.ow = pl.ow; d.oh = pl.oh; d.rot = pl.rot; d.mode = pl.mode;
+        d.left = pl.left; d.top = pl.top; d.cw = pl.cw; d.ch = pl.ch;
         std::memcpy(d.inv, pl.inv, sizeof d.inv);
         d.out_off = 0;
+        pp::rotate_crops_items(&d, 1, items.data());
+        pp::WarpItem* ditems = reinterpret_cast<pp::WarpItem*>(dd.as<pp::WarpDesc>() + 1);
         OAR_HIP(hipMemcpy(dd.p, &d, sizeof d, hipMemcpyHostToDevice));
-        pp::rotate_crops(nullptr, dd.as<pp::WarpDesc>(), 1, dout.as<uint8_t>(), pl.out_w() * pl.out_h());
+        OAR_HIP(hipMemcpy(ditems, items.data(), items.size() * sizeof(pp::WarpItem), hipMemcpyHostToDevice));
+        pp::rotate_crops(nullptr, dd.as<pp::WarpDesc>(), ditems, (int)items.size(), dout.as<uint8_t>());
         OAR_HIP(hipMemcpy(out, dout.p, bytes, hipMemcpyDeviceToHost));
+    });
+}
+
+oar_status oar_k_rotate_crops(const uint8_t* const* pages, const uint32_t* page_ws, const uint32_t* page_hs, uint32_t n_pages, const float* boxes8,
+                              const uint32_t* box_page, uint32_t n_boxes, uint8_t* out, size_t cap, uint32_t* out_ws, uint32_t* out_hs, size_t* out_offs,
+                              size_t* needed) {
+    return guard([&] {
+        OAR_CHECK(pages && page_ws && page_hs && n_pages && needed && (n_boxes == 0 || (boxes8 && box_page && out_ws && out_hs && out_offs)), OAR_INVALID_INPUT,
+                  "oar_k_rotate_crops: bad arguments");
+        require_device();
+        std::vector<pp::WarpDesc> descs;
+        std::vector<uint32_t> desc_page;
+        size_t pool = 0;
+        for (uint32_t i = 0; i < n_boxes; ++i) {
+            OAR_CHECK(box_page[i] < n_pages, OAR_INVALID_INPUT, "oar_k_rotate_crops: box on a page that was not given");
+            const uint32_t pg = box_page[i];
+            host::CropPlan pl = host::plan_crop((int)page_ws[pg], (int)page_hs[pg], boxes8 + (size_t)i * 8);
+            out_ws[i] = out_hs[i] = 0; out_offs[i] = pool;
+            if (pl.mode == 0) continue;
+            out_ws[i] = (uint32_t)pl.out_w(); out_hs[i] = (uint32_t)pl.out_h();
+            pp::WarpDesc d;
+            std::memset(&d, 0, sizeof d);
+            d.page_w = (int)page_ws[pg]; d.page_h = (int)page_hs[pg]; d.mode = pl.mode; d.rot = pl.rot;
+            d.left = pl.left; d.top = pl.top; d.cw = pl.cw; d.ch = pl.ch; d.ow = pl.ow; d.oh = pl.oh;
+            std::memcpy(d.inv, pl.inv, sizeof d.inv);
+            d.out_off = (int64_t)pool;
+            descs.push_back(d); desc_page.push_back(pg);
+            pool += ((size_t)pl.out_w() * pl.out_h() * 3 + 63) & ~(size_t)63;
+        }
+        *needed = pool;
+        if (!out || descs.empty()) return;
+        OAR_CHECK(cap >= pool, OAR_INVALID_INPUT, "oar_k_rotate_crops: output buffer too small");
+        struct Pages { std::vector<void*> p; ~Pages() { for (void* q : p) if (q) (void)hipFree(q); } } dev;
+        dev.p.assign(n_pages, nullptr);
+        for (uint32_t g = 0; g < n_pages; ++g) {
+            const size_t bytes = (size_t)page_ws[g] * page_hs[g] * 3;
+            OAR_CHECK(bytes > 0 && pages[g], OAR_INVALID_INPUT, "oar_k_rotate_crops: empty page");
+            OAR_HIP(hipMalloc(&dev.p[g], bytes));
+            OAR_HIP(hipMemcpy(dev.p[g], pages[g], bytes, hipMemcpyHostToDevice));
+        }
+        for (size_t i = 0; i < descs.size(); ++i) descs[i].page = static_cast<const uint8_t*>(dev.p[desc_page[i]]);
+        std::vector<pp::WarpItem> items(pp::rotate_crops_items(descs.data(), (int)descs.size(), nullptr));
+        pp::rotate_crops_items(descs.data(), (int)descs.size(), items.data());
+        DevBuf dd, dout;
+        dd.reserve(descs.size() * sizeof(pp::WarpDesc) + items.size() * sizeof(pp::WarpItem)); dout.reserve(pool);
+        pp::WarpItem* ditems = reinterpret_cast<pp::WarpItem*>(dd.as<pp::WarpDesc>() + descs.size());
+        OAR_HIP(hipMemcpy(dd.p, descs.data(), descs.size() * sizeof(pp::WarpDesc), hipMemcpyHostToDevice));
+        OAR_HIP(hipMemcpy(ditems, items.data(), items.size() * sizeof(pp::WarpItem), hipMemcpyHostToDevice));
+        pp::rotate_crops(nullptr, dd.as<pp::WarpDesc>(), ditems, (int)items.size(), dout.as<uint8_t>());
+        OAR_HIP(hipMemcpy(out, dout.p, pool, hipMemcpyDeviceToHost));
+    });
+}
+
+oar_status oar_k_rec_resize_u8(const uint8_t* const* rgb, const uint32_t* widths, const uint32_t* heights, const uint8_t* flips, uint32_t n, uint32_t img_h,
+                               uint32_t img_w, uint32_t max_img_w, uint8_t* out, uint32_t* tensor_width, int32_t* resized_widths) {
+    return guard([&] {
+        OAR_CHECK(tensor_width && img_h && (n == 0 || (rgb && widths && heights)), OAR_INVALID_INPUT, "oar_k_rec_resize_u8: bad arguments");
+        require_device();
+        std::vector<uint32_t> ws(widths, widths + n), hs(heights, heights + n);
+        std::vector<int32_t> rws;
+        const int Wt = host::rec_tensor_width(ws, hs, (int)img_h, (int)img_w, (int)max_img_w, rws);
+        *tensor_width = (uint32_t)Wt;
+        if (!out || n == 0) return;
+        size_t stage = 0, resized = 0;
+        for (uint32_t i = 0; i < n; ++i) { stage += ((size_t)ws[i] * hs[i] * 3 + 63) & ~(size_t)63; resized += ((size_t)img_h * rws[i] * 3 + 63) & ~(size_t)63; }
+        int max_rw = 0;
+        for (int32_t rw : rws) max_rw = std::max(max_rw, (int)rw);
+        DevBuf dc, dd, di, dout;
+        dc.reserve(stage); dd.reserve(n * sizeof(pp::CropDesc)); di.reserve(n * sizeof(pp::ResizedImg)); dout.reserve(resized);
+        std::vector<pp::CropDesc> descs(n);
+        std::vector<pp::ResizedImg> imgs(n);
+        size_t off = 0, roff = 0;
+        for (uint32_t i = 0; i < n; ++i) {
+            const size_t bytes = (size_t)ws[i] * hs[i] * 3;
+            OAR_HIP(hipMemcpy(dc.as<uint8_t>() + off, rgb[i], bytes, hipMemcpyHostToDevice));
+            descs[i].src = dc.as<uint8_t>() + off; descs[i].w = (int)ws[i]; descs[i].h = (int)hs[i]; descs[i].rw = rws[i]; descs[i].flip = flips && flips[i] ? 1 : 0;
+            imgs[i].ptr = dout.as<uint8_t>() + roff; imgs[i].w = rws[i]; imgs[i].pad = 0;
+            off += (bytes + 63) & ~(size_t)63;
+            roff += ((size_t)img_h * rws[i] * 3 + 63) & ~(size_t)63;
+        }
+        OAR_HIP(hipMemcpy(dd.p, descs.data(), n * sizeof(pp::CropDesc), hipMemcpyHostToDevice));
+        OAR_HIP(hipMemcpy(di.p, imgs.data(), n * sizeof(pp::ResizedImg), hipMemcpyHostToDevice));
+        pp::rec_resize_u8(nullptr, dd.as<pp::CropDesc>(), di.as<pp::ResizedImg>(), (int)n, (int)img_h, max_rw);
+        std::memset(out, 0, (size_t)n * img_h * Wt * 3);
+        roff = 0;
+        for (uint32_t i = 0; i < n; ++i) {
+            if (rws[i] > 0)
+                OAR_HIP(hipMemcpy2D(out + (size_t)i * img_h * Wt * 3, (size_t)Wt * 3, dout.as<uint8_t>() + roff, (size_t)rws[i] * 3, (size_t)rws[i] * 3, img_h, hipMemcpyDeviceToHost));
+            roff += ((size_t)img_h * rws[i] * 3 + 63) & ~(size_t)63;
+            if (resized_widths) resized_widths[i] = rws[i];
+        }
     });
 }
 
diff --git a/oar_ocr_amd/csrc/pipeline.cc b/oar_ocr_amd/csrc/pipeline.cc
--- a/oar_ocr_amd/csrc/pipeline.cc
+++ b/oar_ocr_amd/csrc/pipeline.cc
@@ -1052,6 +1052,7 @@
         OAR_HIP(hipEventCreateWithFlags(&ev, hipEventDisableTiming));
         lane_done_.push_back(ev);
     }
+    OAR_HIP(hipEventCreateWithFlags(&front_ready_, hipEventDisableTiming));
     if (n_lanes > 1) {
         std::vector<hipStream_t> ls{eng_->stream()};
         for (auto& l : lanes_) ls.push_back(l->stream());
@@ -1062,6 +1063,7 @@
     if (!lanes_.empty()) Profiler::get().remove_lanes(this);
     for (auto& l : lanes_) (void)hipStreamSynchronize(l->stream());
     for (hipEvent_t e : lane_done_) (void)hipEventDestroy(e);
+    if (front_ready_) (void)hipEventDestroy(front_ready_);
 }
 
 const float* Recognizer::pack(const std::vector<Crop>& crops, int& Wt, bool nchw, size_t desc_slot, size_t stage_slot, int lane) {
@@ -1109,50 +1111,7 @@
 }
 
 static_assert(sizeof(pp::ResizedImg) == sizeof(k::StemImg) && sizeof(pp::ResizedImg) == 16, "one table for pp::rec_resize_u8 and k::conv_smallcin_u8");
-
-const pp::ResizedImg* Recognizer::pack_u8(const std::vector<Crop>& crops, int& Wt, size_t desc_slot, size_t stage_slot, int lane) {
-    hipStream_t s = lane_engine(lane).stream();
-    DevBuf& in_buf = lane == 0 ? input_f32_ : *lane_in_[lane - 1];
-    const int n = (int)crops.size();
-    const int img_h = (int)cfg_.rec_image_shape[1], img_w = (int)cfg_.rec_image_shape[2];
-    std::vector<uint32_t> ws(n), hs(n);
-    size_t stage = 0;
-    for (int i = 0; i < n; ++i) {
-        OAR_CHECK(crops[i].w > 0 && crops[i].h > 0 && (crops[i].host || crops[i].dev), OAR_INVALID_INPUT, "recognizer: empty crop");
-        ws[i] = crops[i].w; hs[i] = crops[i].h;
-        if (!crops[i].dev) stage += ((size_t)crops[i].w * crops[i].h * 3 + 63) & ~(size_t)63;
-    }
-    std::vector<int32_t> rws;
-    Wt = host::rec_tensor_width(ws, hs, img_h, img_w, (int)cfg_.max_img_w, rws);
-    size_t need_in = 0;
-    int max_rw = 0;
-    for (int i = 0; i < n; ++i) { need_in += ((size_t)img_h * rws[i] * 3 + 63) & ~(size_t)63; max_rw = std::max(max_rw, (int)rws[i]); }
-    const size_t need_desc = (desc_slot + n) * sizeof(pp::CropDesc), need_stage = stage_slot + stage, need_imgs = (desc_slot + n) * sizeof(pp::ResizedImg);
-    OAR_CHECK(need_stage <= crops_dev_.cap && need_in <= in_buf.cap && need_desc <= descs_dev_.cap && need_imgs <= imgs_dev_.cap && need_desc <= descs_host_.cap &&
-                  need_stage <= stage_host_.cap && need_imgs <= imgs_host_.cap, OAR_INTERNAL, "recognizer staging buffers must be pre-sized (run_batches)");
-    pp::CropDesc* dh = descs_host_.as<pp::CropDesc>() + desc_slot;
-    pp::CropDesc* dd = descs_dev_.as<pp::CropDesc>() + desc_slot;
-    pp::ResizedImg* ih = imgs_host_.as<pp::ResizedImg>() + desc_slot;
-    pp::ResizedImg* id = imgs_dev_.as<pp::ResizedImg>() + desc_slot;
-    size_t off = stage_slot, roff = 0;
-    for (int i = 0; i < n; ++i) {
-        const uint8_t* d = crops[i].dev;
-        if (!d) {
-            const size_t bytes = (size_t)crops[i].w * crops[i].h * 3;
-            std::memcpy(stage_host_.as<uint8_t>() + off, crops[i].host, bytes);
-            d = crops_dev_.as<uint8_t>() + off;
-            off += (bytes + 63) & ~(size_t)63;
-        }
-        dh[i].src = d; dh[i].w = (int)crops[i].w; dh[i].h = (int)crops[i].h; dh[i].rw = rws[i]; dh[i].flip = crops[i].flip ? 1 : 0;
-        ih[i].ptr = in_buf.as<uint8_t>() + roff; ih[i].w = rws[i]; ih[i].pad = 0;
-        roff += ((size_t)img_h * rws[i] * 3 + 63) & ~(size_t)63;
-    }
-    if (stage) OAR_HIP(hipMemcpyAsync(crops_dev_.as<uint8_t>() + stage_slot, stage_host_.as<uint8_t>() + stage_slot, stage, hipMemcpyHostToDevice, s));
-    OAR_HIP(hipMemcpyAsync(dd, dh, (size_t)n * sizeof(pp::CropDesc), hipMemcpyHostToDevice, s));
-    OAR_HIP(hipMemcpyAsync(id, ih, (size_t)n * sizeof(pp::ResizedImg), hipMemcpyHostToDevice, s));
-    pp::rec_resize_u8(s, dd, id, n, img_h, max_rw);
-    return id;
-}
+static_assert(sizeof(pp::CropDesc) % 8 == 0 && sizeof(pp::WarpDesc) % 8 == 0, "the ResizedImg table / the warp's block table follows the descriptors in the same upload");
 
 void Recognizer::pack_only(const std::vector<Crop>& crops, std::vector<float>& nchw, uint32_t& Wt_out) {
     std::lock_guard<std::mutex> lk(mu_);
@@ -1196,19 +1155,18 @@
         total_crops += b.size();
     }
     if (total_crops == 0) return;
-    if (total_stage > crops_dev_.cap || max_in > input_f32_.cap || total_crops * sizeof(pp::CropDesc) > descs_dev_.cap) {
-        OAR_HIP(hipStreamSynchronize(s));
-        crops_dev_.reserve(total_stage); input_f32_.reserve(max_in); descs_dev_.reserve(total_crops * sizeof(pp::CropDesc));
-    }
+    const char* fuse_env = getenv("OAR_REC_FUSE_STEM");
+    const bool fuse_stem = !(fuse_env && fuse_env[0] == '0') && eng_->stem_fusable();
+    if (max_in > input_f32_.cap) { OAR_HIP(hipStreamSynchronize(s)); input_f32_.reserve(max_in); }
     for (auto& lb : lane_in_)
         if (max_in > lb->cap) { for (auto& le : lanes_) OAR_HIP(hipStreamSynchronize(le->stream())); lb->reserve(max_in); }
-    descs_host_.reserve(total_crops * sizeof(pp::CropDesc));
-    stage_host_.reserve(total_stage);
-    const char* fuse_env = getenv("OAR_REC_FUSE_STEM");
-    const bool fuse_stem = !(fuse_env && fuse_env[0] == '0') && eng_->stem_fusable();
-    if (fuse_stem) {
-        if (total_crops * sizeof(pp::ResizedImg) > imgs_dev_.cap) { OAR_HIP(hipStreamSynchronize(s)); for (auto& le : lanes_) OAR_HIP(hipStreamSynchronize(le->stream())); imgs_dev_.reserve(total_crops * sizeof(pp::ResizedImg)); }
-        imgs_host_.reserve(total_crops * sizeof(pp::ResizedImg));
+    if (!fuse_stem) {
+        if (total_stage > crops_dev_.cap || total_crops * sizeof(pp::CropDesc) > descs_dev_.cap) {
+            OAR_HIP(hipStreamSynchronize(s));
+            crops_dev_.reserve(total_stage); descs_dev_.reserve(total_crops * sizeof(pp::CropDesc));
+        }
+        descs_host_.reserve(total_crops * sizeof(pp::CropDesc));
+        stage_host_.reserve(total_stage);
     }
 
     struct Pending { size_t row0, rows; };
@@ -1216,12 +1174,13 @@
     size_t desc_slot = 0, stage_slot = 0, row_total = 0;
     std::vector<int> Wts(batches.size(), 0);
     std::vector<char> fuse_tail(batches.size(), 0);
+    std::vector<std::vector<int32_t>> rws_all(batches.size());
     for (size_t bi = 0; bi < batches.size(); ++bi) {
         const auto& b = batches[bi];
         if (b.empty()) continue;
         std::vector<uint32_t> ws, hs;
         for (auto& c : b) { ws.push_back(c.w); hs.push_back(c.h); }
-        std::vector<int32_t> rws;
+        std::vector<int32_t>& rws = rws_all[bi];
         Wts[bi] = host::rec_tensor_width(ws, hs, img_h, img_w, (int)cfg_.max_img_w, rws);
         const Plan& probe = eng_->plan_for({(int64_t)b.size(), 3, img_h, Wts[bi]}, true, false, nullptr, fuse_stem);
         OAR_CHECK(!probe.outputs.empty(), OAR_INTERNAL, "CRNN: no output returned from inference");
@@ -1243,19 +1202,81 @@
     const int n_lanes = 1 + (int)lanes_.size();
     std::vector<char> lane_used(n_lanes, 0);
     int next_lane = 0;
+    struct FrontSlot { size_t crop0 = 0; int max_rw = 0; };
+    std::vector<FrontSlot> fslot(batches.size());
+    const pp::CropDesc* front_descs = nullptr;
+    const pp::ResizedImg* front_imgs = nullptr;
+    if (fuse_stem) {
+        size_t crop0 = 0;
+        for (size_t bi = 0; bi < batches.size(); ++bi) {
+            if (batches[bi].empty()) continue;
+            fslot[bi].crop0 = crop0;
+            for (int32_t rw : rws_all[bi]) fslot[bi].max_rw = std::max(fslot[bi].max_rw, (int)rw);
+            crop0 += batches[bi].size();
+        }
+        const size_t off_img = total_crops * sizeof(pp::CropDesc);
+        const size_t off_stage = (off_img + total_crops * sizeof(pp::ResizedImg) + 63) & ~(size_t)63;
+        const size_t front_bytes = off_stage + total_stage;
+        if (front_bytes > front_dev_.cap) {
+            OAR_HIP(hipStreamSynchronize(s));
+            for (auto& le : lanes_) OAR_HIP(hipStreamSynchronize(le->stream()));
+            front_dev_.reserve(front_bytes);
+        }
+        front_host_.reserve(front_bytes);
+        uint8_t* hb = front_host_.as<uint8_t>();
+        uint8_t* db = front_dev_.as<uint8_t>();
+        pp::CropDesc* dh = reinterpret_cast<pp::CropDesc*>(hb);
+        pp::ResizedImg* ih = reinterpret_cast<pp::ResizedImg*>(hb + off_img);
+        size_t soff = off_stage;
+        int lane = 0;
+        for (size_t bi = 0; bi < batches.size(); ++bi) {
+            const auto& b = batches[bi];
+            if (b.empty()) continue;
+            DevBuf& in_buf = lane == 0 ? input_f32_ : *lane_in_[lane - 1];
+            lane = (lane + 1) % n_lanes;
+            const std::vector<int32_t>& rws = rws_all[bi];
+            size_t roff = 0;
+            for (size_t i = 0; i < b.size(); ++i) {
+                const uint8_t* d = b[i].dev;
+                if (!d) {
+                    const size_t bytes = (size_t)b[i].w * b[i].h * 3;
+                    std::memcpy(hb + soff, b[i].host, bytes);
+                    d = db + soff;
+                    soff += (bytes + 63) & ~(size_t)63;
+                }
+                pp::CropDesc& cd = dh[fslot[bi].crop0 + i];
+                cd.src = d; cd.w = (int)b[i].w; cd.h = (int)b[i].h; cd.rw = rws[i]; cd.flip = b[i].flip ? 1 : 0;
+                pp::ResizedImg& ri = ih[fslot[bi].crop0 + i];
+                ri.ptr = in_buf.as<uint8_t>() + roff; ri.w = rws[i]; ri.pad = 0;
+                roff += ((size_t)img_h * rws[i] * 3 + 63) & ~(size_t)63;
+            }
+            OAR_CHECK(roff <= in_buf.cap, OAR_INTERNAL, "recognizer input buffer must be pre-sized (run_batches)");
+        }
+        OAR_CHECK(soff == front_bytes, OAR_INTERNAL, "recognizer staging size mismatch");
+        OAR_HIP(hipMemcpyAsync(db, hb, front_bytes, hipMemcpyHostToDevice, s));
+        if (n_lanes > 1) OAR_HIP(hipEventRecord(front_ready_, s));
+        front_descs = reinterpret_cast<const pp::CropDesc*>(db);
+        front_imgs = reinterpret_cast<const pp::ResizedImg*>(db + off_img);
+    }
     for (size_t bi = 0; bi < batches.size(); ++bi) {
         const auto& b = batches[bi];
         if (b.empty()) continue;
         const int lane = next_lane;
         next_lane = (next_lane + 1) % n_lanes;
-        lane_used[lane] = 1;
         Engine& eng = lane_engine(lane);
         hipStream_t sl = eng.stream();
         int Wt = 0;
         const float* in = nullptr;
         const pp::ResizedImg* imgs = nullptr;
-        if (fuse_stem) imgs = pack_u8(b, Wt, desc_slot, stage_slot, lane);
-        else in = pack(b, Wt, false, desc_slot, stage_slot, lane);
+        if (fuse_stem) {
+            if (lane != 0 && !lane_used[lane]) OAR_HIP(hipStreamWaitEvent(sl, front_ready_, 0));
+            Wt = Wts[bi];
+            imgs = front_imgs + fslot[bi].crop0;
+            pp::rec_resize_u8(sl, front_descs + fslot[bi].crop0, imgs, (int)b.size(), img_h, fslot[bi].max_rw);
+        } else {
+            in = pack(b, Wt, false, desc_slot, stage_slot, lane);
+        }
+        lane_used[lane] = 1;
         desc_slot += b.size();
         for (auto& c : b) if (!c.dev) stage_slot += ((size_t)c.w * c.h * 3 + 63) & ~(size_t)63;
         k::StemU8 st{};
@@ -1741,12 +1762,12 @@
             while (pi < planned.size()) {
                 size_t room = cfg_.max_pooled_crops - pool.size();
                 size_t take = std::min(room, planned.size() - pi);
-                size_t add_bytes = 0;
-                int max_px = 0;
+                size_t add_bytes = 0, n_items = 0;
                 for (size_t q = pi; q < pi + take; ++q) {
                     const host::CropPlan& pl = planned[q].plan;
                     add_bytes += ((size_t)pl.out_w() * pl.out_h() * 3 + 63) & ~(size_t)63;
-                    max_px = std::max(max_px, pl.out_w() * pl.out_h());
+                    const size_t step = (size_t)pp::warp_block_pixels(pl.mode, pl.rot);
+                    n_items += ((size_t)pl.out_w() * pl.out_h() + step - 1) / step;
                 }
                 if (pool_bytes + add_bytes > crop_pool_.cap) {
                     OAR_HIP(hipStreamSynchronize(s));
@@ -1755,15 +1776,16 @@
                     if (pool_bytes) OAR_HIP(hipMemcpy(bigger.p, crop_pool_.p, pool_bytes, hipMemcpyDeviceToDevice));
                     std::swap(bigger.p, crop_pool_.p); std::swap(bigger.cap, crop_pool_.cap);
                 }
-                const size_t need_desc = (desc_used + take) * sizeof(pp::WarpDesc);
+                const size_t slot = take * sizeof(pp::WarpDesc) + n_items * sizeof(pp::WarpItem);
+                const size_t need_desc = desc_used + slot;
                 if (need_desc > warp_descs_dev_.cap || need_desc > warp_descs_host_.cap) {
                     OAR_HIP(hipStreamSynchronize(s));
-                    const size_t want = std::max<size_t>(2 * take * sizeof(pp::WarpDesc), 8192 * sizeof(pp::WarpDesc));
+                    const size_t want = std::max<size_t>(2 * slot, 8192 * sizeof(pp::WarpDesc));
                     warp_descs_host_.reserve(want); warp_descs_dev_.reserve(want);
                     desc_used = 0;
                 }
-                pp::WarpDesc* wd = warp_descs_host_.as<pp::WarpDesc>() + desc_used;
-                pp::WarpDesc* wd_dev = warp_descs_dev_.as<pp::WarpDesc>() + desc_used;
+                pp::WarpDesc* wd = reinterpret_cast<pp::WarpDesc*>(warp_descs_host_.as<uint8_t>() + desc_used);
+                pp::WarpDesc* wd_dev = reinterpret_cast<pp::WarpDesc*>(warp_descs_dev_.as<uint8_t>() + desc_used);
                 for (size_t q = 0; q < take; ++q) {
                     const Planned& P = planned[pi + q];
                     const host::CropPlan& pl = P.plan;
@@ -1779,9 +1801,11 @@
                     pool.push_back(it);
                     pool_bytes += ((size_t)it.w * it.h * 3 + 63) & ~(size_t)63;
                 }
-                OAR_HIP(hipMemcpyAsync(wd_dev, wd, take * sizeof(pp::WarpDesc), hipMemcpyHostToDevice, s));
-                pp::rotate_crops(s, wd_dev, (int)take, crop_pool_.as<uint8_t>(), max_px);
-                desc_used += take;
+                const size_t filled = pp::rotate_crops_items(wd, (int)take, reinterpret_cast<pp::WarpItem*>(wd + take));
+                OAR_CHECK(filled == n_items, OAR_INTERNAL, "rotate_crops: block table size mismatch");
+                OAR_HIP(hipMemcpyAsync(wd_dev, wd, slot, hipMemcpyHostToDevice, s));
+                pp::rotate_crops(s, wd_dev, reinterpret_cast<const pp::WarpItem*>(wd_dev + take), (int)n_items, crop_pool_.as<uint8_t>());
+                desc_used += (slot + 15) & ~(size_t)15;
                 pi += take;
                 if (pool.size() >= cfg_.max_pooled_crops) { flush(); ++flush_count; desc_used = 0; }
             }
diff --git a/oar_ocr_amd/csrc/pipeline.h b/oar_ocr_amd/csrc/pipeline.h
--- a/oar_ocr_amd/csrc/pipeline.h
+++ b/oar_ocr_amd/csrc/pipeline.h
@@ -132,8 +132,8 @@
 
    private:
     const float* pack(const std::vector<Crop>& crops, int& Wt, bool nchw, size_t desc_slot = 0, size_t stage_slot = 0, int lane = 0);
-    const pp::ResizedImg* pack_u8(const std::vector<Crop>& crops, int& Wt, size_t desc_slot, size_t stage_slot, int lane);
-    DevBuf imgs_dev_; PinBuf imgs_host_;
+    DevBuf front_dev_; PinBuf front_host_;
+    hipEvent_t front_ready_ = nullptr;
     Engine& lane_engine(int lane) { return lane == 0 ? *eng_ : *lanes_[lane - 1]; }
     std::unique_ptr<Engine> eng_;
     std::vector<std::unique_ptr<Engine>> lanes_;
diff --git a/oar_ocr_amd/csrc/prepost.h b/oar_ocr_amd/csrc/prepost.h
--- a/oar_ocr_amd/csrc/prepost.h
+++ b/oar_ocr_amd/csrc/prepost.h
@@ -64,7 +64,19 @@
     float inv[9];
     int64_t out_off;
 };
-void rotate_crops(hipStream_t s, const WarpDesc* d_descs, int n, uint8_t* out_pool, int max_out_pixels);
+struct WarpItem { int32_t crop, first; };
+inline int warp_block_pixels(int mode, int rot) { return mode == 1 && !rot ? 1024 : 256; }
+inline size_t rotate_crops_items(const WarpDesc* descs, int n, WarpItem* out) {
+    size_t m = 0;
+    for (int i = 0; i < n; ++i) {
+        const long total = (long)descs[i].ow * descs[i].oh;
+        const int step = warp_block_pixels(descs[i].mode, descs[i].rot);
+        for (long p = 0; p < total; p += step, ++m)
+            if (out) out[m] = WarpItem{i, (int32_t)p};
+    }
+    return m;
+}
+void rotate_crops(hipStream_t s, const WarpDesc* d_descs, const WarpItem* d_items, int n_items, uint8_t* out_pool);
 
 struct ClsDesc {
     const uint8_t* src;
diff --git a/oar_ocr_amd/csrc/prepost.hip b/oar_ocr_amd/csrc/prepost.hip
--- a/oar_ocr_amd/csrc/prepost.hip
+++ b/oar_ocr_amd/csrc/prepost.hip
@@ -606,57 +606,93 @@
 }
 __device__ __forceinline__ int clampi(int v, int lo, int hi) { return v < lo ? lo : (v > hi ? hi : v); }
 
-__global__ __launch_bounds__(256) void rotate_crops_kernel(const WarpDesc* descs, uint8_t* pool) {
-    const WarpDesc d = descs[blockIdx.y];
+__device__ __forceinline__ uint32_t shr_bytes(uint32_t hi, uint32_t lo, unsigned n) { return (uint32_t)((((uint64_t)hi << 32) | lo) >> (8u * n)); }
+__device__ __forceinline__ uint32_t load_px(const uint8_t* p) {
+    const unsigned a = (unsigned)(reinterpret_cast<uintptr_t>(p) & 3);
+    const uint32_t* p4 = reinterpret_cast<const uint32_t*>(p - a);
+    const uint32_t lo = p4[0], hi = a >= 2 ? p4[1] : 0u;
+    return shr_bytes(hi, lo, a);
+}
+
+__global__ __launch_bounds__(256) void rotate_crops_kernel(const WarpDesc* descs, const WarpItem* items, uint8_t* pool) {
+    const WarpItem it = items[blockIdx.x];
+    const WarpDesc d = descs[it.crop];
     const int out_w = d.rot ? d.oh : d.ow, out_h = d.rot ? d.ow : d.oh;
     const long total = (long)out_w * out_h;
     uint8_t* out = pool + d.out_off;
     const uint8_t* crop = d.page + ((long)d.top * d.page_w + d.left) * 3;
     const long stride = (long)d.page_w * 3;
-    for (long i = (long)blockIdx.x * blockDim.x + threadIdx.x; i < total; i += (long)gridDim.x * blockDim.x) {
-        int xo = (int)(i % out_w), yo = (int)(i / out_w);
-        int dx = d.rot ? d.ow - 1 - yo : xo, dy = d.rot ? xo : yo;
-        uint8_t r, g, b;
-        if (d.mode == 1) {
-            const uint8_t* p = crop + (long)dy * stride + (long)dx * 3;
-            r = p[0]; g = p[1]; b = p[2];
+    const uint8_t* page_end = d.page + (long)d.page_w * d.page_h * 3;
+    if (d.mode == 1 && !d.rot) {
+        const long i0 = (long)it.first + (long)threadIdx.x * 4;
+        if (i0 >= total) return;
+        const int xo = (int)(i0 % out_w), yo = (int)(i0 / out_w);
+        const uint8_t* p = crop + (long)yo * stride + (long)xo * 3;
+        uint8_t* o = out + i0 * 3;
+        if (i0 + 4 <= total && xo + 4 <= out_w && p + 16 <= page_end && (reinterpret_cast<uintptr_t>(o) & 3) == 0) {
+            const unsigned a = (unsigned)(reinterpret_cast<uintptr_t>(p) & 3);
+            const uint32_t* p4 = reinterpret_cast<const uint32_t*>(p - a);
+            const uint32_t w0 = p4[0], w1 = p4[1], w2 = p4[2], w3 = a ? p4[3] : 0u;
+            uint32_t* o4 = reinterpret_cast<uint32_t*>(o);
+            o4[0] = shr_bytes(w1, w0, a); o4[1] = shr_bytes(w2, w1, a); o4[2] = shr_bytes(w3, w2, a);
         } else {
-            float fx = (float)dx, fy = (float)dy;
-            float px = d.inv[0] * fx; px = d.inv[1] * fy + px; px = d.inv[2] * 1.0f + px;
-            float py = d.inv[3] * fx; py = d.inv[4] * fy + py; py = d.inv[5] * 1.0f + py;
-            float pz = d.inv[6] * fx; pz = d.inv[7] * fy + pz; pz = d.inv[8] * 1.0f + pz;
-            if (fabsf(pz) > 1.1920929e-7f) {
-                float x = px / pz, y = py / pz;
-                int xi = (int)floorf(x), yi = (int)floorf(y);
-                float ddx = x - (float)xi, ddy = y - (float)yi;
-                float wx[4] = {cubic_kernel(ddx + 1.0f), cubic_kernel(ddx), cubic_kernel(ddx - 1.0f), cubic_kernel(ddx - 2.0f)};
-                float wy[4] = {cubic_kernel(ddy + 1.0f), cubic_kernel(ddy), cubic_kernel(ddy - 1.0f), cubic_kernel(ddy - 2.0f)};
-                long cx[4], cy[4];
-#pragma unroll
-                for (int k = 0; k < 4; ++k) { cx[k] = (long)clampi(xi - 1 + k, 0, d.cw - 1) * 3; cy[k] = (long)clampi(yi - 1 + k, 0, d.ch - 1) * stride; }
-                float r0 = 0.0f, r1 = 0.0f, r2 = 0.0f;
-#pragma unroll
-                for (int j = 0; j < 4; ++j)
-#pragma unroll
-                    for (int k = 0; k < 4; ++k) {
-                        float wt = wx[k] * wy[j];
-                        const uint8_t* p = crop + cy[j] + cx[k];
-                        r0 += wt * (float)p[0]; r1 += wt * (float)p[1]; r2 += wt * (float)p[2];
-                    }
-                r = (uint8_t)fminf(fmaxf(roundf(r0), 0.0f), 255.0f);
-                g = (uint8_t)fminf(fmaxf(roundf(r1), 0.0f), 255.0f);
-                b = (uint8_t)fminf(fmaxf(roundf(r2), 0.0f), 255.0f);
-            } else {
-                r = crop[0]; g = crop[1]; b = crop[2];
+            for (int k = 0; k < 4 && i0 + k < total; ++k) {
+                const long i = i0 + k;
+                const uint8_t* q = crop + (i / out_w) * stride + (i % out_w) * 3;
+                out[i * 3] = q[0]; out[i * 3 + 1] = q[1]; out[i * 3 + 2] = q[2];
             }
         }
-        out[i * 3] = r; out[i * 3 + 1] = g; out[i * 3 + 2] = b;
-    }
-}
-void rotate_crops(hipStream_t s, const WarpDesc* d_descs, int n, uint8_t* out_pool, int max_out_pixels) {
-    if (n == 0) return;
-    ProfScope ps(s, "rotate_crops", 6.0 * (double)n * max_out_pixels, 0.0);
-    hipLaunchKernelGGL(rotate_crops_kernel, dim3(grid_for(max_out_pixels, 256, 64), n), dim3(256), 0, s, d_descs, out_pool);
+        return;
+    }
+    const long i = (long)it.first + threadIdx.x;
+    if (i >= total) return;
+    const int xo = (int)(i % out_w), yo = (int)(i / out_w);
+    const int dx = d.rot ? d.ow - 1 - yo : xo, dy = d.rot ? xo : yo;
+    uint8_t r, g, b;
+    if (d.mode == 1) {
+        const uint8_t* p = crop + (long)dy * stride + (long)dx * 3;
+        if (p + 8 <= page_end) { const uint32_t v = load_px(p); r = (uint8_t)v; g = (uint8_t)(v >> 8); b = (uint8_t)(v >> 16); }
+        else { r = p[0]; g = p[1]; b = p[2]; }
+    } else {
+        float fx = (float)dx, fy = (float)dy;
+        float px = d.inv[0] * fx; px = d.inv[1] * fy + px; px = d.inv[2] * 1.0f + px;
+        float py = d.inv[3] * fx; py = d.inv[4] * fy + py; py = d.inv[5] * 1.0f + py;
+        float pz = d.inv[6] * fx; pz = d.inv[7] * fy + pz; pz = d.inv[8] * 1.0f + pz;
+        if (fabsf(pz) > 1.1920929e-7f) {
+            float x = px / pz, y = py / pz;
+            int xi = (int)floorf(x), yi = (int)floorf(y);
+            float ddx = x - (float)xi, ddy = y - (float)yi;
+            float wx[4] = {cubic_kernel(ddx + 1.0f), cubic_kernel(ddx), cubic_kernel(ddx - 1.0f), cubic_kernel(ddx - 2.0f)};
+            float wy[4] = {cubic_kernel(ddy + 1.0f), cubic_kernel(ddy), cubic_kernel(ddy - 1.0f), cubic_kernel(ddy - 2.0f)};
+            long cx[4], cy[4];
+#pragma unroll
+            for (int k = 0; k < 4; ++k) { cx[k] = (long)clampi(xi - 1 + k, 0, d.cw - 1) * 3; cy[k] = (long)clampi(yi - 1 + k, 0, d.ch - 1) * stride; }
+            float r0 = 0.0f, r1 = 0.0f, r2 = 0.0f;
+            const bool packed = crop + cy[3] + cx[3] + 8 <= page_end;
+#pragma unroll
+            for (int j = 0; j < 4; ++j)
+#pragma unroll
+                for (int k = 0; k < 4; ++k) {
+                    const float wt = __fmul_rn(wx[k], wy[j]);
+                    const uint8_t* p = crop + cy[j] + cx[k];
+                    float p0, p1, p2;
+                    if (packed) { const uint32_t v = load_px(p); p0 = (float)(v & 0xFFu); p1 = (float)((v >> 8) & 0xFFu); p2 = (float)((v >> 16) & 0xFFu); }
+                    else { p0 = (float)p[0]; p1 = (float)p[1]; p2 = (float)p[2]; }
+                    r0 = __fadd_rn(r0, __fmul_rn(wt, p0)); r1 = __fadd_rn(r1, __fmul_rn(wt, p1)); r2 = __fadd_rn(r2, __fmul_rn(wt, p2));
+                }
+            r = (uint8_t)fminf(fmaxf(roundf(r0), 0.0f), 255.0f);
+            g = (uint8_t)fminf(fmaxf(roundf(r1), 0.0f), 255.0f);
+            b = (uint8_t)fminf(fmaxf(roundf(r2), 0.0f), 255.0f);
+        } else {
+            r = crop[0]; g = crop[1]; b = crop[2];
+        }
+    }
+    out[i * 3] = r; out[i * 3 + 1] = g; out[i * 3 + 2] = b;
+}
+void rotate_crops(hipStream_t s, const WarpDesc* d_descs, const WarpItem* d_items, int n_items, uint8_t* out_pool) {
+    if (n_items == 0) return;
+    ProfScope ps(s, "rotate_crops", 6.0 * (double)n_items * 256, 0.0);
+    hipLaunchKernelGGL(rotate_crops_kernel, dim3(n_items), dim3(256), 0, s, d_descs, d_items, out_pool);
 }
 
 __global__ __launch_bounds__(256) void cls_pack_kernel(const ClsDesc* descs, int crop_h, int crop_w, NormP np_, float* out, int nchw) {
diff --git a/rust/oar-mi355x-sys/src/lib.rs b/rust/oar-mi355x-sys/src/lib.rs
--- a/rust/oar-mi355x-sys/src/lib.rs
+++ b/rust/oar-mi355x-sys/src/lib.rs
@@ -412,6 +412,8 @@
     pub fn oar_k_unclip(boxes: *const f32, n_boxes: u32, ratio: f32, counts: *mut i32, pts_xy: *mut f32, cap_points: u32) -> oar_status;
     pub fn oar_k_box_scores(pred: *const f32, height: u32, width: u32, boxes: *const f32, n_boxes: u32, scores: *mut f32) -> oar_status;
     pub fn oar_k_rotate_crop(rgb: *const u8, w: u32, h: u32, box_: *const f32, out: *mut u8, cap: usize, out_w: *mut u32, out_h: *mut u32) -> oar_status;
+    pub fn oar_k_rotate_crops(pages: *const *const u8, page_ws: *const u32, page_hs: *const u32, n_pages: u32, boxes8: *const f32, box_page: *const u32, n_boxes: u32, out: *mut u8, cap: usize, out_ws: *mut u32, out_hs: *mut u32, out_offs: *mut usize, needed: *mut usize) -> oar_status;
+    pub fn oar_k_rec_resize_u8(rgb: *const *const u8, widths: *const u32, heights: *const u32, flips: *const u8, n: u32, img_h: u32, img_w: u32, max_img_w: u32, out: *mut u8, tensor_width: *mut u32, resized_widths: *mut i32) -> oar_status;
     pub fn oar_image_decode(bytes: *const u8, len: usize, rgb: *mut *mut u8, width: *mut u32, height: *mut u32) -> oar_status;
     pub fn oar_image_free(rgb: *mut u8);
     pub fn oar_image_decode_device(bytes: *const u8, len: usize, device_id: i32, dev_rgb: *mut *mut c_void, width: *mut u32, height: *mut u32) -> oar_status;
```

Result: slower. 2449 images/sec (-1.6%).
